# cptq/SignNet-BasisNet

Hardware: AMD Instinct MI355X
Metric: graphs/sec SignNet+GINE forward, ZINC batch=128 k=16 (higher is better)
Workload: dtype f32

## Files before the change

include/signnet_hip.h:

```cpp
#ifndef SIGNNET_HIP_H
#define SIGNNET_HIP_H

#include <stdint.h>

#ifdef __cplusplus
extern "C" {
#endif

#define SN_OK 0
#define SN_ERR_ARG (-1)
#define SN_ERR_LAUNCH (-2)
#define SN_ERR_UNSUPPORTED (-3)

#define SN_ABI_VERSION 3

int sn_version(void);
const char* sn_last_error(void);
int sn_device_info(int* cu_count, int* lds_bytes_per_cu, int* clock_khz);
int sn_clock_probe(int64_t cycles, int64_t* out_cycles, void* stream);

typedef struct {
  int32_t* phi_bin_col;
  int64_t phi_max_bins;
  int32_t* phi_col_bin0;
// ... 344 lines not shown
                     const int32_t* rowptr, const int32_t* col, const sn_plan_bins* bins,
                     int kmax , int K ,
                     float* out, void* stream);
int sn_phi_fused_prec_f32(const sn_phi_params* params, const float* eigen_vectors, const int32_t* graph_ptr, const int64_t* evoff,
                          const int32_t* rowptr, const int32_t* col, const sn_plan_bins* bins, int kmax, int K, float* out,
                          int precision, void* stream);

int sn_deepsigns_phi_f32(const sn_phi_params* params, const float* x, int ldx, const int32_t* graph_ptr, const int32_t* rowptr,
                         const int32_t* col, const sn_plan_bins* bins, int K, float* out, void* stream);
int sn_deepsigns_phi_prec_f32(const sn_phi_params* params, const float* x, int ldx, const int32_t* graph_ptr, const int32_t* rowptr,
                              const int32_t* col, const sn_plan_bins* bins, int K, float* out, int precision, void* stream);

#define SN_MLP_MAX_LAYERS 16
int sn_mlp_chain_f32(const float* x, int ldx, int64_t R, int d_in, const int32_t* nvalid, int K, const void* const* weights,
                     int n_layers, int d_pad, float* y, int ldy, int d_out, void* stream);
int sn_mlp_chain_prec_f32(const float* x, int ldx, int64_t R, int d_in, const int32_t* nvalid, int K, const void* const* weights,
                          int n_layers, int d_pad, float* y, int ldy, int d_out, int precision, void* stream);

typedef struct {
  const void *wq, *wk, *wv, *wfc;
  const float *ln1_g, *ln1_b;
  const void *w1, *w2;
  const float *ln2_g, *ln2_b;
} sn_rho_layer;

#define SN_RHO_MAX_LAYERS 8
#define SN_RHO_BIN_ROWS 64
typedef struct {
  int d, n_layers, heads, has_pos;
  float ln_eps;
  int head_pad;
  const float* pe_w1;
  const float* pe_bn0_scale;
  const float* pe_bn0_shift;
  const float* pe_w2;
  const float* pe_bn1_scale;
  const float* pe_bn1_shift;
  sn_rho_layer layers[SN_RHO_MAX_LAYERS];
} sn_rho_params;

int sn_rho_fused_f32(const sn_rho_params* params, const float* x, const float* eigen_values,
                     const int32_t* graph_ptr, int64_t B, int64_t N, const sn_plan_bins* bins, int kmax, int K,
                     float* out_sum, void* stream);
int sn_rho_fused_prec_f32(const sn_rho_params* params, const float* x, const float* eigen_values, const int32_t* graph_ptr, int64_t B,
                          int64_t N, const sn_plan_bins* bins, int kmax, int K, float* out_sum, int precision, void* stream);

typedef struct {
  const float* etab[10];
  const float* ew;
  const float* e_scale;
  const float* e_shift;
  const void* w1s;
  const void* w2s;
  const float* eps;
} sn_gnn_layer;

#define SN_GNN_MAX_LAYERS 16
#define SN_GNN_MAX_NODES 64
typedef struct {
  int d, n_layers, n_out, reserved;
  int node_discrete, node_nf;
  int edge_discrete, edge_nf;
  int node_vocab, edge_vocab;
  const float* ntab[10];
  const float* nw;
  const float* n_scale;
  const float* n_shift;
  const void* rho_out_w;
  const void* lin_a;
  const void* lin_b;
  const void* head_w1;
  const void* head_w2;
  sn_gnn_layer layers[SN_GNN_MAX_LAYERS];
} sn_gnn_params;

int sn_gnn_fused_f32(const sn_gnn_params* params, const void* x, int ldx, const void* edge_attr, int lde,
                     const float* rho_sum, const int32_t* graph_ptr, int64_t B, const int32_t* rowptr,
                     const int32_t* col, const int32_t* eperm, int32_t* status ,
                     float* y ,
                     const int32_t* flags_src, int n_flags, int32_t* flags_host ,
                     void* stream);


int sn_gin_net_fused_f32(const sn_gnn_params* params, const void* head_mid, int pool_mean, const int64_t* atom, const float* p, int ldp,
                         int kp, const int32_t* graph_ptr, int64_t B, const int32_t* rowptr, const int32_t* col, const int32_t* eperm,
                         int32_t* status, float* y, const int32_t* flags_src, int n_flags, void* stream);

int sn_transformer_net_fused_f32(const sn_gnn_params* params, const void* head_mid, int pool_mean, const int64_t* atom, const float* p,
                                 int ldp, int kp, const float* e_proj, int lde, const int32_t* graph_ptr, int64_t B, const int32_t* rowptr,
                                 const int32_t* col, const int32_t* eperm, int32_t* status, float* y, const int32_t* flags_src, int n_flags,
                                 void* stream);

typedef struct {
  const float* x; int ldx;
  int64_t R; int G;
  int d_in, d_out;
  const float* W; int ldw;
  const float* bias;
  const int32_t* nvalid; int K;
  const float* in_scale; const float* in_shift;
  int in_relu, out_relu;
  float* y; int ldy;
  float* stat_part;
} sn_train_linear_args;

typedef struct {
  int64_t R; int G;
  const int32_t* nvalid; int K;
  int d_in, d_out;
  const float* dy; int lddy;
  const float* zo; int ldzo;
  const float* coef_a; const float* coef_b; const float* coef_c;
  const float* mask_scale; const float* mask_shift;
  const float* x; int ldx;
  const float* x_scale; const float* x_shift;
  int x_relu;
  const float* x_mean;
  const float* W; int ldw;
  float* gx; int ldgx;
  float* sums_part;
  float* dw_part;
  int want_db;
  int gx_accumulate;
  const float* dot_x; int lddot;
  double* dot_part;
  const float* merge_sums; int merge_nblk;
  const float* merge_state; const float* merge_count; const float* merge_gamma;
  float* merge_dgamma; float* merge_dbeta; int merge_accumulate;
} sn_train_linear_bwd_args;

typedef struct sn_train_post_args {
  const float* dw_part; int nparts; int64_t stride; int64_t n_w; float* dw_out; int64_t n_b; float* db_out;
  const float* sums_part; int nblk; int G; int C; const float* state; const float* count; const float* gamma; float* coef;
  float* dgamma; float* dbeta; int accumulate_bn;
  const double* dot_part; int dot_n; float* dot_out;
} sn_train_post_args;
int sn_train_post_link_f32(const sn_train_post_args* args, void* stream);
int sn_train_linear_blocks(int64_t R, int G);
int sn_train_linear_bwd_blocks(int64_t R, int G);
int sn_train_bn_bwd_blocks(int64_t R, int G);
int64_t sn_train_linear_bwd_part_floats(int64_t R, int G, int d_in, int d_out);
int sn_train_linear_f32(const sn_train_linear_args* args, void* stream);
int sn_train_bn_finish_f32(const float* stat_part, int nblk, int G, int C, const float* gamma, const float* beta, float eps,
                           float momentum, float* running_mean, float* running_var, float* state, float* count, void* stream);
int sn_train_linear_bwd_f32(const sn_train_linear_bwd_args* args, void* stream);
int sn_train_bn_bwd_sums_f32(const float* dy, int lddy, const float* z, int ldz, int64_t R, int G, int C, const int32_t* nvalid,
                             int K, const float* state, int relu, float* sums_part, void* stream);
int sn_train_bn_bwd_finish_f32(const float* sums_part, int nblk, int G, int C, const float* state, const float* count,
                               const float* gamma, float* coef, float* dgamma, float* dbeta, int accumulate, void* stream);
int sn_train_bn_apply_f32(const float* z, int ldz, int64_t R, int G, int C, const int32_t* nvalid, int K, const float* state,
                          int relu, const float* residual, int ldr, float* y, int ldy, void* stream);
int sn_train_reduce_parts_f32(const float* part, int nparts, int64_t stride, int64_t n, float* out, int accumulate, void* stream);
#define SN_TRAIN_MAX_REDUCE_JOBS 64
typedef struct { const float* part; int nparts; int64_t stride; int64_t n; float* out; int accumulate; } sn_train_reduce_job;
int sn_train_reduce_jobs_f32(const sn_train_reduce_job* jobs, int njobs, void* stream);
typedef struct { const double* part; int n; float* out; } sn_train_dot_job;
int sn_train_dot_jobs_f64(const sn_train_dot_job* jobs, int njobs, void* stream);
int sn_train_dot_finish_f64(const double* part, int n, float* out, int accumulate, void* stream);

int sn_gin_aggregate_add_f32(const float* x, const float* plus, float* out, int64_t N, int F, const int32_t* rowptr, const int32_t* col,
                             const float* eps, void* stream);
int sn_gine_aggregate_bwd_add_f32(const float* h, const float* ee, const float* g, const float* plus, int64_t N, int C,
                                  const int32_t* rev_rowptr, const int32_t* rev_col, const int32_t* rev_eperm, const float* eps,
                                  float* dh, float* dee, void* stream);

typedef struct {
// ... 42 lines not shown
```

signnet_basisnet_amd/_lib.py:

```python
from __future__ import annotations

import ctypes as C
import os

import torch

_HERE = os.path.dirname(os.path.abspath(__file__))
LIB_PATH = os.path.join(_HERE, "libsignnet_hip.so")

EPI_BIAS, EPI_RELU_PRE, EPI_AFFINE, EPI_RELU, EPI_RESIDUAL = 1, 2, 4, 8, 16
EPI_RESIDUAL_PRE = 64
EPI_LEAKY = 128

_p, _i, _l, _f = C.c_void_p, C.c_int, C.c_int64, C.c_float
ABI_VERSION = 3

SIGNATURES = {
    "sn_version": [],
    "sn_device_info": [C.POINTER(_i), C.POINTER(_i), C.POINTER(_i)],
    "sn_clock_probe": [_l, _p, _p],
    "sn_batch_plan": [_p, _l, _l, _p, _l, _i, _p, _p, _p, _p, _p, _p, _p, _p, _p, _p, _p],
    "sn_batch_plan_ex": [_p, _l, _l, _p, _l, _i, _p, _p, _p, _p, _p, _p, _p, _p, _p, _p, _p, _p],
    "sn_batch_plan_early_supported": [_l, _l, _l],
    "sn_pack_eig_f32": [_p, _p, _p, _p, _p, _p, _l, _i, _p, _p, _p],
    "sn_bucket_pack": [_p, _p],
    "sn_bucket_pack_dgl": [_p, _p],
    "sn_store_gather": [_p, _p],
    "sn_store_gather_max_graphs": [],
    "sn_batch_plan_padded": [_p, _l, _l, _p, _l, _i, _p, _p, _p, _p, _p, _p, _p, _p, _p, _p, _p, _p, _p],
    "sn_masked_l1_f32": [_p, _p, _l, _i, _p, _p, _p, _p],
    "sn_masked_l1_bwd_f32": [_p, _p, _l, _i, _p, _p, _p, _p, _p],
    "sn_lap_pe_transform_f32": [_p, _i, _p, _i, _i, _i, _i, _p, _p, _i, _p],
    "sn_pack_weight_f32": [_p, _i, _i, _i, _p, _p],
    "sn_pack_weight_t_f32": [_p, _i, _i, _i, _p, _p],
    "sn_pack_split_f32": [_p, _i, _i, _i, _p, _p, _p, _p, _p],
    "sn_gin_aggregate_f32": [_p, _p, _l, _i, _p, _p, _p, _i, _p],
    "sn_gin_aggregate_slab_f32": [_p, _p, _l, _i, _l, _p, _p, _p, _p, _i, _p],
    "sn_gine_aggregate_f32": [_p, _p, _p, _l, _i, _p, _p, _p, _p, _p],
    "sn_masked_linear_f32": [_p, _i, _l, _i, _p, _i, _p, _p, _i, _i, _p, _p, _p, _i, _p, _i, _p],
    "sn_ign_mlp_f32": [_p, _l, _i, _i, _i, _p, _p, _p],
    "sn_deepsets_tail_f32": [_p, _i, _p, _p, _p],
    "sn_masked_linear_blockbias_f32": [_p, _i, _l, _i, _p, _i, _p, _p, _l, _i, _i, _p, _p, _p, _i, _p],
    "sn_bn_fold_f32": [_p, _p, _p, _p, _f, _i, _i, _p, _p, _p],
    "sn_bn_running_update_f32": [_p, _p, _p, _f, _i, _p, _p, _p],
    "sn_colstats_blocks": [_l],
    "sn_phi_fused_f32": [_p, _p, _p, _p, _p, _p, _p, _i, _i, _p, _p],
    "sn_rho_fused_f32": [_p, _p, _p, _p, _l, _l, _p, _i, _i, _p, _p],
    "sn_phi_fused_prec_f32": [_p, _p, _p, _p, _p, _p, _p, _i, _i, _p, _i, _p],
    "sn_rho_fused_prec_f32": [_p, _p, _p, _p, _l, _l, _p, _i, _i, _p, _i, _p],
    "sn_gnn_fused_f32": [_p, _p, _i, _p, _i, _p, _p, _l, _p, _p, _p, _p, _p, _p, _i, _p, _p],
    "sn_gin_net_fused_f32": [_p, _p, _i, _p, _p, _i, _i, _p, _l, _p, _p, _p, _p, _p, _p, _i, _p],
    "sn_transformer_net_fused_f32": [_p, _p, _i, _p, _p, _i, _i, _p, _i, _p, _l, _p, _p, _p, _p, _p, _p, _i, _p],
    "sn_masked_colstats_f32": [_p, _i, _l, _i, _p, _i, _p, _p, _p, _p, _p],
    "sn_masked_affine_f32": [_p, _i, _l, _i, _p, _i, _i, _p, _p, _p, _i, _p, _i, _p],
    "sn_masked_layernorm_f32": [_p, _p, _l, _i, _p, _p, _f, _p, _i, _p, _p],
    "sn_set_attention_f32": [_p, _p, _p, _l, _i, _i, _i, _p, _p, _p, _p],
    "sn_slot_sum_f32": [_p, _l, _i, _i, _p, _p],
    "sn_plan_double_i32": [_p, _p, _l, _l, _p, _p, _p],
    "sn_keep_mask_f32": [_p, _l, _f, _f, _p],
    "sn_embedding_sum_f32": [_p, _i, _i, _l, C.POINTER(_p), C.POINTER(C.c_int64), _i, _p, _p, _p],
    "sn_segment_pool_f32": [_p, _l, _i, _p, _i, _p, _p],
    "sn_ign_contract_2to1_f32": [_p, _l, _i, _p, _p, _p],
    "sn_laplacian_evd_f32": [_p, _l, _p, _l, _l, _i, _p, _p, _p, _l, _p, _i, _i, _p, _p, _p],
    "sn_laplacian_evd_large_f32": [_p, _l, _p, _l, _l, _i, _p, _p, _p, _l, _p, _i, _i, _p, _p, _p],
    "sn_evd_large_max_nodes": [],
    "sn_evd_large_work_ints": [_l],
    "sn_linear_bn_scratch_floats": [_l, _i, _i],
    "sn_linear_bn_train_f32": [_p, _i, _l, _i, _p, _i, _p, _p, _i, _p, _i, _p, _p, _f, _f, _p, _p, _p, _p, _p, _p, _p, _p, _p, _p],
    "sn_bn_train_stats_f32": [_p, _i, _l, _i, _p, _i, _p, _p, _f, _f, _p, _p, _p, _p, _p, _p, _p, _p, _p, _p],
    "sn_linear_wgrad_f32": [_p, _i, _p, _i, _l, _i, _i, _p, _i, _p, _p, _p, _p],
    "sn_bn_act_bwd_f32": [_p, _i, _p, _i, _l, _i, _p, _i, _p, _p, _p, _p, _i, _p, _p, _p, _i, _p, _p],
    "sn_relu_bwd_f32": [_p, _p, _l, _i, _p, _i, _p, _p],
    "sn_masked_layernorm_bwd_f32": [_p, _p, _p, _l, _i, _p, _f, _p, _i, _p, _p, _p, _p, _p],
    "sn_set_attention_bwd_f32": [_p, _p, _p, _p, _l, _i, _i, _i, _p, _p, _p, _p, _p, _p],
    "sn_gine_aggregate_bwd_f32": [_p, _p, _p, _l, _i, _p, _p, _p, _p, _p, _p, _p],
    "sn_slot_broadcast_f32": [_p, _l, _i, _i, _p, _p, _p],
    "sn_segment_broadcast_f32": [_p, _l, _i, _p, _i, _p, _p],
    "sn_embedding_sum_bwd_f32": [_p, _i, _i, _l, _p, C.POINTER(C.c_int64), _i, _p, _p, _p, _p],
    "sn_embedding_sum_layers_f32": [_p, _i, _i, _l, _i, _p, C.POINTER(C.c_int64), _i, _p, _p, _p],
    "sn_embedding_sum_bwd_layers_f32": [_p, _i, _i, _l, _i, _p, C.POINTER(C.c_int64), _i, _p, _p, _p, _p],
    "sn_dot_f32": [_p, _p, _l, _p, _p, _p],
    "sn_pna_aggregate_f32": [_p, _i, _p, _i, _i, _l, _p, _p, _f, _p, _i, _p],
    "sn_pna_aggregate_gather_f32": [_p, _i, _p, _i, _p, _i, _p, _i, _i, _l, _p, _p, _p, _f, _p, _i, _i, _p],
    "sn_grouped_linear_f32": [_p, _i, _l, _i, _i, _i, _p, _p, _p, _p, _p, _p, _i, _p],
    "sn_edge_attention_f32": [_p, _p, _p, _p, _l, _i, _i, _p, _p, _p, _p, _p],
    "sn_edge_attention_strided_f32": [_p, _p, _p, _i, _p, _i, _l, _i, _i, _p, _p, _p, _p, _p],
    "sn_pointwise_f32": [_p, _i, _l, _i, _p, _p, _p, _i, _f, _p, _i, _p, _i, _p],
    "sn_deepsigns_phi_f32": [_p, _p, _i, _p, _p, _p, _p, _i, _p, _p],
    "sn_mlp_chain_f32": [_p, _i, _l, _i, _p, _i, _p, _i, _i, _p, _i, _i, _p],
    "sn_deepsigns_phi_prec_f32": [_p, _p, _i, _p, _p, _p, _p, _i, _p, _i, _p],
    "sn_mlp_chain_prec_f32": [_p, _i, _l, _i, _p, _i, _p, _i, _i, _p, _i, _i, _i, _p],
    "sn_gat_aggregate_f32": [_p, _p, _p, _p, _l, _i, _i, _f, _i, _p, _p, _p, _p, _p],
    "sn_gat_aggregate_bwd_f32": [_p, _p, _p, _p, _p, _p, _p, _l, _l, _i, _i, _f, _i, _p, _p, _p, _p, _p, _p, _p, _p, _p, _p, _p, _p],
    "sn_edge_rows_sum_f32": [_p, _i, _i, _l, _p, _p, _p, _i, _p],
    "sn_pna_aggregate_bwd_f32": [_p, _i, _i, _l, _p, _p, _f, _p, _i, _p, _p, _p],
    "sn_edge_attention_bwd_f32": [_p, _p, _p, _p, _p, _p, _l, _l, _i, _i, _p, _p, _p, _p, _p, _p, _p, _p, _p, _p, _p, _p],
    "sn_act_bwd_f32": [_p, _p, _l, _i, _p, _i, _f, _p, _p],
    "sn_gatedgcn_fused_f32": [_p, _p, _p, _p, _l, _p, _p, _p, _p, _p, _p],
    "sn_dense_attention_f32": [_p, _p, _p, _l, _i, _i, _i, _p, _p, _p],
    "sn_dense_attention_bwd_f32": [_p, _p, _p, _p, _p, _p, _l, _i, _i, _i, _p, _p, _p, _p, _p],
    "sn_eigenspace_group": [_p, _i, _i, _p, _p, _p, _p, _p, _p, _p, _p],
    "sn_eigenspace_projectors_f32": [_p, _i, _i, _p, _p, _i, _p, _p],
    "sn_ign_contract_eigvecs_f32": [_p, _i, _i, _p, _p, _i, _i, _p, _p],
    "sn_gated_aggregate_f32": [_p, _p, _p, _p, _i, _p, _l, _i, _p, _p, _p, _p, _p, _p, _p, _p, _p, _p, _p, _p, _p],
    "sn_gated_aggregate_bwd_f32": [_p, _p, _p, _p, _p, _p, _p, _l, _i, _p, _p, _p, _p, _p, _p, _p, _p, _p, _p, _p, _p],
    "sn_adam_step_f32": [_p, _p, _p, _p, _l, _f, _f, _f, _f, _f, _i, _f, _p],
    "sn_train_post_link_f32": [_p, _p],
    "sn_train_linear_blocks": [_l, _i],
    "sn_train_linear_bwd_blocks": [_l, _i],
    "sn_train_bn_bwd_blocks": [_l, _i],
    "sn_train_linear_f32": [_p, _p],
    "sn_train_bn_finish_f32": [_p, _i, _i, _i, _p, _p, _f, _f, _p, _p, _p, _p, _p],
    "sn_train_linear_bwd_f32": [_p, _p],
    "sn_train_bn_bwd_sums_f32": [_p, _i, _p, _i, _l, _i, _i, _p, _i, _p, _i, _p, _p],
    "sn_train_bn_bwd_finish_f32": [_p, _i, _i, _i, _p, _p, _p, _p, _p, _p, _i, _p],
    "sn_train_bn_apply_f32": [_p, _i, _l, _i, _i, _p, _i, _p, _i, _p, _i, _p, _i, _p],
    "sn_train_reduce_parts_f32": [_p, _i, _l, _l, _p, _i, _p],
    "sn_train_dot_finish_f64": [_p, _i, _p, _i, _p],
    "sn_train_reduce_jobs_f32": [_p, _i, _p],
    "sn_train_dot_jobs_f64": [_p, _i, _p],
    "sn_masked_layernorm_bwd_acc_f32": [_p, _p, _p, _l, _i, _p, _f, _p, _i, _p, _p, _p, _p, _p],
    "sn_gin_aggregate_add_f32": [_p, _p, _p, _l, _i, _p, _p, _p, _p],
    "sn_gine_aggregate_bwd_add_f32": [_p, _p, _p, _p, _l, _i, _p, _p, _p, _p, _p, _p, _p],
    "sn_train_scalar_mlp_stats_f32": [_p, _f, _p, _p, _f, _p, _p, _p, _p],
    "sn_train_scalar_mlp_apply_f32": [_p, _p, _p],
    "sn_train_scalar_mlp_bwd_f32": [_p, _p, _p, _p, _p, _p, _p, _p, _p, _p, _p, _i, _p, _p],
}
_SPECIAL_RESTYPE = {"sn_last_error": C.c_char_p, "sn_packed_weight_floats": C.c_int64, "sn_evd_large_work_ints": C.c_int64}

_lib = None


def lib():
# ... 110 lines not shown
```

signnet_basisnet_amd/csrc/fused_gnn.hip:

```cpp
#include "fused_common.hpp"

namespace sn {

#ifdef SN_PROFILE
static __device__ int g_prof_block = 0;
#undef SN_STAMP
#undef SN_ACCUM
#define SN_STAMP(i) do { if ((int)blockIdx.x == g_prof_block && threadIdx.x == 0) g_prof[i] = clock64(); } while (0)
#define SN_ACCUM(i, t0) do { if ((int)blockIdx.x == g_prof_block && threadIdx.x == 0) g_prof[i] += clock64() - (t0); } while (0)
#endif

constexpr int GNN_ROWS = SN_GNN_MAX_NODES;
constexpr int GNN_WAVES = 8;
constexpr int GNN_EMAX = 192;
constexpr int GNN_CLS = 16;
constexpr int GNN_EEMAX = 96;
constexpr int GNN_EEPF = (GNN_EEMAX * 32 + GNN_WAVES * 64 - 1) / (GNN_WAVES * 64);

constexpr int SP_STRIDE = 256;
constexpr int SP_PLANE = GNN_ROWS * SP_STRIDE;
constexpr int SP_IMAGE = 52224;
static_assert(SP_IMAGE >= 3 * SP_PLANE && SP_IMAGE % 16 == 0, "three planes fit an image");
__device__ __forceinline__ int sp_chunk(int row, int c) { return ((c ^ row) & 15) << 4; }

struct GnnStruct {
  const void* x;
  int ldx;
  const void* edge_attr;
  int lde;
  const float* rho_sum;
  const int32_t* graph_ptr;
  const int32_t* rowptr;
  const int32_t* col;
  const int32_t* eperm;
  int32_t* status;
  float* y;
  int ee_rows;
  const int32_t* flags_src;
  int n_flags;
  int32_t* flags_host;
  int rho_ld, rho_w;
  const void* head_mid;
  int pool_mean;
};

__device__ __forceinline__ void sp_store4(unsigned char* img, int row, int ot, int g, f32x4 v) {
  float h[4], m[4], l[4];
#pragma unroll
  for (int i = 0; i < 4; ++i) {
    h[i] = __uint_as_float(__float_as_uint(v[i]) & 0xffff0000u);
    const float r = v[i] - h[i];
    m[i] = __uint_as_float(__float_as_uint(r) & 0xffff0000u);
    l[i] = r - m[i];
  }
  unsigned char* p = img + row * SP_STRIDE + sp_chunk(row, (ot >> 1) * 4 + g) + (ot & 1) * 8;
  *reinterpret_cast<uint2*>(p) = make_uint2(pack_hi16(h[0], h[1]), pack_hi16(h[2], h[3]));
  *reinterpret_cast<uint2*>(p + SP_PLANE) = make_uint2(pack_hi16(m[0], m[1]), pack_hi16(m[2], m[3]));
  *reinterpret_cast<uint2*>(p + 2 * SP_PLANE) = make_uint2(pack_hi16(l[0], l[1]), pack_hi16(l[2], l[3]));
}

template <int NKB>
struct WSplit { u32x4 f[NKB * 3]; f32x4 e[SPLIT_EPI]; };

template <int NKB>
__device__ __forceinline__ void wload(WSplit<NKB>& p, const void* wsp, int ot, int lane) {
  constexpr int NFE = 3 * NKB + SPLIT_EPI;
  const __amdgpu_buffer_rsrc_t rs = weight_rsrc(reinterpret_cast<const float*>(wsp), 0x7fffffff);
  const int voff = lane * 16;
  const int base = __builtin_amdgcn_readfirstlane(ot * NFE * 1024);
#pragma unroll
  for (int i = 0; i < 3 * NKB; ++i) p.f[i] = __builtin_amdgcn_raw_buffer_load_b128(rs, voff, base + i * 1024, 0);
#pragma unroll
  for (int j = 0; j < SPLIT_EPI; ++j) {
    const u32x4 v = __builtin_amdgcn_raw_buffer_load_b128(rs, voff, base + (3 * NKB + j) * 1024, 0);
    p.e[j] = f32x4{__uint_as_float(v[0]), __uint_as_float(v[1]), __uint_as_float(v[2]), __uint_as_float(v[3])};
  }
}

struct TileRange {
  int t_lo, t_hi, T;
  __device__ __forceinline__ bool empty() const { return t_lo >= t_hi; }
  __device__ __forceinline__ void decode(int t, int& ot, int& rt) const { ot = t / T; rt = t - ot * T; }
  __device__ __forceinline__ int first_ot() const { return t_lo / T; }
};

template <int NKB>
__device__ __forceinline__ f32x4 mfma_split_tile(const WSplit<NKB>& w, const Split8 (&x)[NKB]) {
  f32x4 a0 = {0.f, 0.f, 0.f, 0.f}, a1 = {0.f, 0.f, 0.f, 0.f};
#pragma unroll
  for (int kb = 0; kb < NKB; ++kb) {
    const u32x4 wh = w.f[3 * kb], wm = w.f[3 * kb + 1], wl = w.f[3 * kb + 2];
    a1 = mfma_bf(wl, x[kb].h, a1);
    a0 = mfma_bf(wm, x[kb].h, a0);
    a1 = mfma_bf(wh, x[kb].l, a1);
    a0 = mfma_bf(wh, x[kb].m, a0);
    a1 = mfma_bf(wm, x[kb].m, a1);
    a0 = mfma_bf(wh, x[kb].h, a0);
  }
  return a0 + a1;
}

template <int NKB, typename Epi>
__device__ __forceinline__ void coop_gemm(WSplit<NKB>& pre, WSplit<NKB>& alt, const void* wsp, const unsigned char* img,
                                          TileRange tr, int lane, Epi epi, const void* next_wsp, TileRange next_tr) {
  if (tr.empty()) {
    if (next_wsp && !next_tr.empty()) wload<NKB>(pre, next_wsp, next_tr.first_ot(), lane);
    return;
  }
  asm volatile("" : "+v"(tr.t_lo), "+v"(tr.t_hi), "+v"(tr.T));
  int ot0, rt0;
  tr.decode(tr.t_lo, ot0, rt0);
  int otl, rtl;
  tr.decode(tr.t_hi - 1, otl, rtl);
  const bool two_ots = otl != ot0;
  const unsigned char* rowbase = img + (lane & 15) * SP_STRIDE;
  auto load_rows = [&](int rt, Split8 (&x)[NKB]) {
    const unsigned char* p = rowbase + rt * 16 * SP_STRIDE;
#pragma unroll
    for (int kb = 0; kb < NKB; ++kb) {
      const unsigned char* pc = p + sp_chunk(lane & 15, kb * 4 + (lane >> 4));
      x[kb].h = *reinterpret_cast<const u32x4*>(pc);
      x[kb].m = *reinterpret_cast<const u32x4*>(pc + SP_PLANE);
      x[kb].l = *reinterpret_cast<const u32x4*>(pc + 2 * SP_PLANE);
    }
  };
#ifdef SN_PROFILE
// ... 53 lines not shown
}

template <int NKB, typename Epi>
__device__ __forceinline__ void coop_gemm_roll(WSplit<NKB>& cur, const unsigned char* img, TileRange tr, int lane, Epi epi,
                                               const void* nn_wsp, TileRange nn_tr, int kb0 = 0) {
  if (!tr.empty()) {
    asm volatile("" : "+v"(tr.t_lo), "+v"(tr.t_hi), "+v"(tr.T));
    const unsigned char* rowbase = img + (lane & 15) * SP_STRIDE;
#pragma unroll
    for (int i = 0; i < 4; ++i) {
      const int t = tr.t_lo + i;
      if (t < tr.t_hi) {
        int ot, rt;
        tr.decode(t, ot, rt);
        Split8 in[NKB];
        const unsigned char* p = rowbase + rt * 16 * SP_STRIDE;
        int cx = (lane & 15) ^ (lane >> 4) ^ (kb0 << 2);
        asm volatile("" : "+v"(cx));
#pragma unroll
        for (int kb = 0; kb < NKB; ++kb) {
          const unsigned char* pc = p + (((4 * kb) ^ cx) << 4);
          in[kb].h = *reinterpret_cast<const u32x4*>(pc);
          in[kb].m = *reinterpret_cast<const u32x4*>(pc + SP_PLANE);
          in[kb].l = *reinterpret_cast<const u32x4*>(pc + 2 * SP_PLANE);
        }
        epi(rt, ot, mfma_split_tile<NKB>(cur, in), cur.e[0], cur.e[1], cur.e[2]);
      }
    }
  }
  if (nn_wsp != nullptr && !nn_tr.empty()) wload<NKB>(cur, nn_wsp, nn_tr.first_ot(), lane);
}

template <int NKB, int PAIRS, typename Epi>
__device__ __forceinline__ void coop_gemm_weave(WSplit<NKB>& cur, const unsigned char* img, int ot, int lane, Epi epi,
                                                const void* nn_wsp, int nn_ot) {
  constexpr int NFE = 3 * NKB + SPLIT_EPI;
  const __amdgpu_buffer_rsrc_t rs = weight_rsrc(reinterpret_cast<const float*>(nn_wsp), 0x7fffffff);
  const int voff = lane * 16;
  const int base = __builtin_amdgcn_readfirstlane(nn_ot * NFE * 1024);
  const unsigned char* rowbase = img + (lane & 15) * SP_STRIDE;
#pragma unroll
  for (int rt = 0; rt < PAIRS; ++rt) {
    Split8 in[NKB];
    const unsigned char* p = rowbase + rt * 16 * SP_STRIDE;
    int cx = (lane & 15) ^ (lane >> 4);
    asm volatile("" : "+v"(cx));
#pragma unroll
    for (int kb = 0; kb < NKB; ++kb) {
      const unsigned char* pc = p + (((4 * kb) ^ cx) << 4);
      in[kb].h = *reinterpret_cast<const u32x4*>(pc);
      in[kb].m = *reinterpret_cast<const u32x4*>(pc + SP_PLANE);
      in[kb].l = *reinterpret_cast<const u32x4*>(pc + 2 * SP_PLANE);
    }
    if (rt + 1 < PAIRS) {
      epi(rt, ot, mfma_split_tile<NKB>(cur, in), cur.e[0], cur.e[1], cur.e[2]);
      __builtin_amdgcn_sched_barrier(0);
    } else {
      f32x4 a0 = {0.f, 0.f, 0.f, 0.f}, a1 = {0.f, 0.f, 0.f, 0.f};
#pragma unroll
      for (int kb = 0; kb < NKB; ++kb) {
        const u32x4 wh = cur.f[3 * kb], wm = cur.f[3 * kb + 1], wl = cur.f[3 * kb + 2];
        a1 = mfma_bf(wl, in[kb].h, a1);
        a0 = mfma_bf(wm, in[kb].h, a0);
        a1 = mfma_bf(wh, in[kb].l, a1);
        a0 = mfma_bf(wh, in[kb].m, a0);
        a1 = mfma_bf(wm, in[kb].m, a1);
        a0 = mfma_bf(wh, in[kb].h, a0);
        __builtin_amdgcn_sched_barrier(0);
#pragma unroll
        for (int j = 0; j < 3; ++j) cur.f[3 * kb + j] = __builtin_amdgcn_raw_buffer_load_b128(rs, voff, base + (3 * kb + j) * 1024, 0);
        __builtin_amdgcn_sched_barrier(0);
      }
      epi(rt, ot, a0 + a1, cur.e[0], cur.e[1], cur.e[2]);
      __builtin_amdgcn_sched_barrier(0);
#pragma unroll
      for (int j = 0; j < SPLIT_EPI; ++j) {
        const u32x4 v = __builtin_amdgcn_raw_buffer_load_b128(rs, voff, base + (3 * NKB + j) * 1024, 0);
        cur.e[j] = f32x4{__uint_as_float(v[0]), __uint_as_float(v[1]), __uint_as_float(v[2]), __uint_as_float(v[3])};
      }
    }
  }
}

template <int NT, int MODE = 0, int TC = 0>
__device__ __forceinline__ void gnn_graph(const GnnStruct& S, const sn_gnn_params& P) {
  constexpr bool DGL = MODE != 0, TF = MODE == 2;
  static_assert(TC == 0 || (NT == 8 && MODE == 0), "compile-time row tiles: the GINE net at NT = 8");
  static_assert(!TF || NT == 4, "the Transformer mode is written for d = 64");
  constexpr int D = 16 * NT;
  constexpr int LD = D + 4;
  constexpr int NKB = (NT + 1) / 2;
  extern __shared__ __align__(16) unsigned char lds_raw[];
  unsigned char* SA = lds_raw;
  unsigned char* SB = lds_raw + SP_IMAGE;
  float* X1 = reinterpret_cast<float*>(lds_raw + 2 * SP_IMAGE);
  int* erow = reinterpret_cast<int*>(X1 + (GNN_ROWS + 1) * LD);
  int* esrc = erow + GNN_ROWS + 4;
  int* efeat = esrc + GNN_EMAX;
  int* ecls = efeat + GNN_EMAX * (P.n_layers > 0 ? P.edge_nf : 0);
  int* elead = ecls + GNN_EMAX;
  int* cedge = elead + GNN_EMAX;
  float* EE = reinterpret_cast<float*>(cedge + GNN_CLS);
  float* PART = EE;
  const int lane = threadIdx.x & 63, wave = threadIdx.x >> 6, g = lane >> 4, li = lane & 15;
  const int gi = blockIdx.x;
  SN_STAMP(0);
#ifdef SN_PROFILE
  if ((int)blockIdx.x == g_prof_block && threadIdx.x == 0) for (int i = 8; i < 20; ++i) g_prof[i] = 0;
  long long pt = 0;
#endif
  WSplit<NKB> pre, alt;
  const int gs = S.graph_ptr[gi], n = S.graph_ptr[gi + 1] - gs;
  auto give_up = [&](int bit) {
    if (threadIdx.x == 0 && bit) atomicOr(&S.status[3], bit);
    if ((int)threadIdx.x < P.n_out) S.y[(int64_t)gi * P.n_out + threadIdx.x] = __uint_as_float(0x7fc00000u);
  };
  if (S.flags_src != nullptr && (S.flags_src[0] != 0 || (S.n_flags >= 16 && (S.flags_src[9] != 0 || S.flags_src[13] != 0)))) { give_up(0); return; }
  if (n <= 0) { give_up(8); return; }
  if (n > GNN_ROWS) { give_up(1); return; }
  const int e_base = S.rowptr[gs];
  const int ne = S.rowptr[gs + n] - e_base;
  const int d = P.d;
  __shared__ unsigned s_pro[3];
  if (threadIdx.x == 0) { s_pro[0] = 0u; s_pro[1] = 0u; s_pro[2] = 0u; }
  const int T = TC > 0 ? TC : (n + 15) >> 4;
  const int ntile = T * NT;
  TileRange tr;
  tr.T = T;
  if constexpr (GNN_WAVES % NT == 0) {
    constexpr int WPO = GNN_WAVES / NT;
    const int ot = wave / WPO, h = wave % WPO, per = (T + WPO - 1) / WPO;
    tr.t_lo = ot * T + (h * per < T ? h * per : T);
    tr.t_hi = ot * T + ((h + 1) * per < T ? (h + 1) * per : T);
  } else {
    const int q = (ntile + GNN_WAVES - 1) / GNN_WAVES;
    tr.t_lo = wave * q < ntile ? wave * q : ntile;
    tr.t_hi = tr.t_lo + q < ntile ? tr.t_lo + q : ntile;
  }
  TileRange hr;
  hr.T = 1;
  hr.t_lo = wave < NT ? wave : NT;
  hr.t_hi = wave < NT ? wave + 1 : NT;
  const f32x4 zero4 = {0.f, 0.f, 0.f, 0.f};
  bool use_tab = false;
  int ncls = 0;
  bool use_ee = !DGL && P.n_layers > 0 && ne <= S.ee_rows;
  auto edge_embed = [&](const sn_gnn_layer& Lq, int k, int c) -> f32x4 {
    const int EF = P.edge_nf;
    f32x4 ef = zero4;
    if (P.edge_discrete) {
      for (int f = 0; f < EF; ++f) {
        const float* trow = Lq.etab[f] + (int64_t)efeat[k * EF + f] * d;
        if ((d & 3) == 0) { if (c < d) ef += ld4(trow + c); }
        else {
#pragma unroll
          for (int qq = 0; qq < 4; ++qq) if (c + qq < d) ef[qq] += trow[c + qq];
        }
      }
    } else {
      f32x4 acc = zero4;
      for (int f = 0; f < EF; ++f) {
        const float a = __int_as_float(efeat[k * EF + f]);
#pragma unroll
        for (int qq = 0; qq < 4; ++qq) acc[qq] += a * Lq.ew[(c + qq) * EF + f];
      }
      ef = relu4(acc * ld4(Lq.e_scale + c) + ld4(Lq.e_shift + c));
    }
    return ef;
  };
  f32x4 eepf[GNN_EEPF];
  auto ee_fetch = [&](int l) {
    if (!use_ee || l >= P.n_layers) return;
    const sn_gnn_layer& Lq = P.layers[l];
    int t0 = threadIdx.x;
    asm volatile("" : "+v"(t0));
#pragma unroll
    for (int i = 0; i < GNN_EEPF; ++i) {
      const int idx = t0 + i * GNN_WAVES * 64;
      eepf[i] = zero4;
      if (idx < ne * (D / 4)) eepf[i] = edge_embed(Lq, idx / (D / 4), 4 * (idx % (D / 4)));
    }
  };
  bool tab_pending = false;
  auto ee_store = [&]() {
    if (tab_pending) {
      tab_pending = false;
      int t1 = threadIdx.x;
      asm volatile("" : "+v"(t1));
#pragma unroll
      for (int i = 0; i < GNN_EEPF; ++i) {
        const int idx = t1 + i * GNN_WAVES * 64;
        if (idx < P.n_layers * ncls * (D / 4)) lds_st4(EE + (idx / (D / 4)) * LD + 4 * (idx % (D / 4)), eepf[i]);
      }
      return;
    }
    if (!use_ee) return;
    int t0 = threadIdx.x;
    asm volatile("" : "+v"(t0));
#pragma unroll
    for (int i = 0; i < GNN_EEPF; ++i) {
      const int idx = t0 + i * GNN_WAVES * 64;
      if (idx < ne * (D / 4)) lds_st4(EE + (idx / (D / 4)) * LD + 4 * (idx % (D / 4)), eepf[i]);
    }
  };

  constexpr bool ROLL = NT >= 7 || GNN_WAVES % NT == 0;
  static_assert(GNN_WAVES == 8, "the ROLL condition assumes 8 waves");
  TileRange h2;
  h2.T = 1;
  h2.t_lo = 0;
  h2.t_hi = wave == 0 ? 1 : 0;
  static_assert(GNN_EMAX <= GNN_WAVES * 64 && GNN_ROWS < GNN_WAVES * 64 && GNN_ROWS * (D / 4) <= 4 * GNN_WAVES * 64, "one pass of the block covers the graph");
  const int tid = threadIdx.x;
  const int rp_v = tid <= n ? S.rowptr[gs + tid] : 0;
  const int rho_ld = S.rho_ld, rho_w = S.rho_w;
  const bool rs_vec = ((rho_ld | rho_w) & 3) == 0;
  f32x4 rs_v[4];
#pragma unroll
  for (int j = 0; j < 4; ++j) {
    rs_v[j] = zero4;
    const int i = tid + j * GNN_WAVES * 64;
    if (rs_vec && i < n * (D / 4)) {
      const int rr = i / (D / 4), c4 = i % (D / 4);
      if (4 * c4 < rho_w) rs_v[j] = ld4(S.rho_sum + (int64_t)(gs + rr) * rho_ld + 4 * c4);
    }
  }
  const bool xid_pref = P.node_discrete && P.node_nf == 1 && (d & 3) == 0;
  long long xid[4];
#pragma unroll
  for (int i = 0; i < 4; ++i) {
    xid[i] = -1;
    const int t = tr.t_lo + i;
    if (xid_pref && t < tr.t_hi) {
      int ot, rt;
      tr.decode(t, ot, rt);
      if (rt * 16 + li < n) xid[i] = reinterpret_cast<const int64_t*>(S.x)[(int64_t)(gs + rt * 16 + li) * S.ldx];
    }
  }
  if (ne > GNN_EMAX) { give_up(2); return; }
  const int src_v = tid < ne ? S.col[e_base + tid] : 0;
  const int eid_v = tid < ne ? S.eperm[e_base + tid] : 0;
  SN_STAMP(30);
  for (int i = threadIdx.x; i < 2 * SP_IMAGE / 16; i += GNN_WAVES * 64)
    reinterpret_cast<uint4*>(lds_raw)[i] = make_uint4(0u, 0u, 0u, 0u);
  if ((int)threadIdx.x < LD) { X1[GNN_ROWS * LD + threadIdx.x] = 0.f; EE[S.ee_rows * LD + threadIdx.x] = 0.f; }
  lds_barrier();
  SN_STAMP(31);
  const bool efast = !DGL && P.n_layers > 0 && P.edge_discrete && P.edge_nf == 1 && (d & 3) == 0;
  int my_ev = 0;
  {
    const int EF = P.edge_nf;
    if (tid <= n) erow[tid] = rp_v - e_base;
    if (tid < ne) {
      const int k = tid;
      esrc[k] = src_v - gs;
      const int eid = eid_v;
      if (TF) ecls[k] = eid;
      if (!DGL && P.n_layers > 0) {
        if (P.edge_discrete) {
          const int64_t* ei = reinterpret_cast<const int64_t*>(S.edge_attr) + (int64_t)eid * S.lde;
          for (int f = 0; f < EF; ++f) {
            const int64_t v = ei[f];
            const bool ok = (uint64_t)v < (uint64_t)P.edge_vocab;
            efeat[k * EF + f] = ok ? (int)v : 0;
            if (!ok) { atomicOr(&S.status[3], 4); atomicOr(&s_pro[0], 1u); }
            if (efast) {
              my_ev = ok ? (int)v : 0;
              if (my_ev < 32) atomicOr(&s_pro[2], 1u << my_ev); else atomicOr(&s_pro[1], 1u);
            }
          }
        } else {
          const float* ea = reinterpret_cast<const float*>(S.edge_attr) + (int64_t)eid * S.lde;
          for (int f = 0; f < EF; ++f) efeat[k * EF + f] = __float_as_int(ea[f]);
        }
      }
    }
  }
  f32x4 nrow[4];
#pragma unroll
  for (int i = 0; i < 4; ++i) {
    nrow[i] = zero4;
    const int t = tr.t_lo + i;
    if (xid_pref && t < tr.t_hi && xid[i] != -1) {
      int ot, rt;
      tr.decode(t, ot, rt);
      long long xv = xid[i];
      if ((uint64_t)xv >= (uint64_t)P.node_vocab) { xv = 0; atomicOr(&S.status[3], 4); atomicOr(&s_pro[0], 1u); }
      const int c = 16 * ot + 4 * g;
      if (c < d) nrow[i] = ld4(P.ntab[0] + xv * d + c);
    }
  }
  if (!tr.empty()) {
    wload<NKB>(pre, P.lin_a, tr.first_ot(), lane);
    if constexpr (ROLL) wload<NKB>(alt, P.lin_b, tr.first_ot(), lane);
  }
  lds_barrier();
  SN_STAMP(32);
  if (efast && s_pro[1] == 0u) {
    const unsigned present = s_pro[2];
    ncls = __popc(present);
    if (tid < ne) ecls[tid] = __popc(present & ((1u << my_ev) - 1u));
    use_tab = ncls <= GNN_CLS && P.n_layers * ncls <= S.ee_rows;
    if (use_tab) {
      use_ee = false;
      tab_pending = true;
      int t0 = threadIdx.x;
      asm volatile("" : "+v"(t0));
#pragma unroll
      for (int i = 0; i < GNN_EEPF; ++i) {
        const int idx = t0 + i * GNN_WAVES * 64;
        eepf[i] = zero4;
        if (idx < P.n_layers * ncls * (D / 4)) {
          const int rowi = idx / (D / 4), ch = 4 * (idx % (D / 4));
          const int l = rowi / ncls, c = rowi - l * ncls;
          unsigned m = present;
          for (int q = 0; q < c; ++q) m &= m - 1u;
          if (ch < d) eepf[i] = ld4(P.layers[l].etab[0] + (int64_t)__builtin_ctz(m) * d + ch);
        }
      }
    }
  }
  if (!DGL && P.n_layers > 0 && !tab_pending && !(efast && s_pro[1] == 0u)) {
    const int EF = P.edge_nf;
    __shared__ unsigned long long lmask[(GNN_EMAX + 63) / 64];
    int lead = -1;
    if (tid < GNN_EMAX) {
      if (tid < ne) {
        lead = tid;
        if (EF == 1) {
          const int mine = efeat[tid];
#pragma unroll 8
          for (int j = 0; j < ne; ++j) lead = (efeat[j] == mine && j < lead) ? j : lead;
        } else {
          for (int j = 0; j < ne; ++j) {
            bool same = true;
            for (int f = 0; f < EF; ++f) same = same && (efeat[j * EF + f] == efeat[tid * EF + f]);
            lead = (same && j < lead) ? j : lead;
          }
        }
        elead[tid] = lead;
      }
      const unsigned long long m = __ballot(tid < ne && lead == tid);
      if (lane == 0) lmask[tid >> 6] = m;
    }
    __syncthreads();
    ncls = 0;
#pragma unroll
    for (int w = 0; w < (GNN_EMAX + 63) / 64; ++w) ncls += __popcll(lmask[w]);
    if (tid < ne) {
      int c = 0;
#pragma unroll
      for (int w = 0; w < (GNN_EMAX + 63) / 64; ++w) {
        const int below = lead - 64 * w;
        const unsigned long long keep = below >= 64 ? ~0ull : (below > 0 ? (1ull << below) - 1 : 0ull);
        c += __popcll(lmask[w] & keep);
      }
      ecls[tid] = c;
      if (lead == tid && c < GNN_CLS) cedge[c] = lead;
    }
    use_tab = ncls <= GNN_CLS && P.n_layers * ncls <= S.ee_rows;
    if (use_tab) use_ee = false;
    __syncthreads();
    if (use_tab) {
      for (int i = threadIdx.x; i < P.n_layers * ncls * (D / 4); i += GNN_WAVES * 64) {
        const int rowi = i / (D / 4), ch = 4 * (i % (D / 4));
        const int l = rowi / ncls, c = rowi - l * ncls;
        lds_st4(EE + rowi * LD + ch, edge_embed(P.layers[l], cedge[c], ch));
      }
    }
  }
  SN_STAMP(33);
  if (rs_vec) {
#pragma unroll
    for (int j = 0; j < 4; ++j) {
      const int i = tid + j * GNN_WAVES * 64;
      if (i < n * (D / 4)) {
        const int rr = i / (D / 4), c4 = i % (D / 4);
        sp_store4(SA, rr, c4 >> 2, c4 & 3, rs_v[j]);
      }
    }
  } else {
    for (int i = threadIdx.x; i < n * (D / 4); i += GNN_WAVES * 64) {
      const int rr = i / (D / 4), c4 = i % (D / 4);
      f32x4 v = zero4;
#pragma unroll
      for (int qq = 0; qq < 4; ++qq) if (4 * c4 + qq < rho_w) v[qq] = S.rho_sum[(int64_t)(gs + rr) * rho_ld + 4 * c4 + qq];
      sp_store4(SA, rr, c4 >> 2, c4 & 3, v);
    }
  }
  SN_STAMP(34);
  if (xid_pref) {
#pragma unroll
    for (int i = 0; i < 4; ++i) {
      const int t = tr.t_lo + i;
      if (t < tr.t_hi && xid[i] != -1) {
        int ot, rt;
        tr.decode(t, ot, rt);
        sp_store4(SB, rt * 16 + li, ot, g, nrow[i]);
      }
    }
  } else if (P.node_discrete) {
    for (int t = tr.t_lo; t < tr.t_hi; ++t) {
      int ot, rt;
      tr.decode(t, ot, rt);
      const int row = rt * 16 + li, c = 16 * ot + 4 * g;
      if (row < n) {
        const int64_t* xi = reinterpret_cast<const int64_t*>(S.x) + (int64_t)(gs + row) * S.ldx;
        f32x4 s = zero4;
        for (int f = 0; f < P.node_nf; ++f) {
          int64_t xv = xi[f];
          if ((uint64_t)xv >= (uint64_t)P.node_vocab) { xv = 0; atomicOr(&S.status[3], 4); atomicOr(&s_pro[0], 1u); }
          const float* trow = P.ntab[f] + xv * d;
          if ((d & 3) == 0) { if (c < d) s += ld4(trow + c); }
          else {
#pragma unroll
            for (int qq = 0; qq < 4; ++qq) if (c + qq < d) s[qq] += trow[c + qq];
          }
        }
        sp_store4(SB, row, ot, g, s);
      }
    }
  } else {
    for (int t = tr.t_lo; t < tr.t_hi; ++t) {
      int ot, rt;
      tr.decode(t, ot, rt);
      const int row = rt * 16 + li, c = 16 * ot + 4 * g;
      if (row < n) {
        const float* xr = reinterpret_cast<const float*>(S.x) + (int64_t)(gs + row) * S.ldx;
        f32x4 acc = zero4;
        for (int f = 0; f < P.node_nf; ++f) {
          const float a = xr[f];
#pragma unroll
          for (int qq = 0; qq < 4; ++qq) acc[qq] += a * P.nw[(c + qq) * P.node_nf + f];
        }
        sp_store4(SB, row, ot, g, relu4(acc * ld4(P.n_scale + c) + ld4(P.n_shift + c)));
      }
    }
  }
  SN_STAMP(35);
  lds_barrier();
  const int graph_bad = (int)s_pro[0];
  SN_STAMP(1);
  int a_dg[4];
  unsigned a_sr[4], a_er[4];
#pragma unroll
  for (int i = 0; i < 4; ++i) {
    a_dg[i] = -1;
    a_sr[i] = 0u;
    a_er[i] = 0u;
    const int t = tr.t_lo + i;
    if (!TF && t < tr.t_hi && (DGL || use_tab || use_ee)) {
      int ot, rt;
      tr.decode(t, ot, rt);
      const int row = rt * 16 + li;
      if (row < n) {
        const int e_lo = erow[row], dg = erow[row + 1] - e_lo;
        a_dg[i] = dg;
#pragma unroll
        for (int k = 0; k < 4; ++k) {
          const int ei = k < dg ? e_lo + k : 0;
          a_sr[i] |= (unsigned)(k < dg ? esrc[ei] : GNN_ROWS) << (8 * k);
          if (!DGL) a_er[i] |= (unsigned)(k < dg ? (use_tab ? ecls[ei] : ei) : 255) << (8 * k);
        }
      }
    }
  }
  ee_fetch(0);
  const void* first_w = P.n_layers > 0 ? P.layers[0].w1s : P.head_w1;
  const TileRange first_tr = P.n_layers > 0 ? tr : hr;
  {
    auto epi_a = [&](int rt, int ot, f32x4 acc, f32x4, f32x4, f32x4) { lds_st4(X1 + (rt * 16 + li) * LD + 16 * ot + 4 * g, acc); };
    auto epi_b = [&](int rt, int ot, f32x4 acc, f32x4 bias, f32x4, f32x4) {
      float* o = X1 + (rt * 16 + li) * LD + 16 * ot + 4 * g;
      lds_st4(o, (lds_ld4(o) + acc) + bias);
    };
    const bool hasl = P.n_layers > 0;
    if constexpr (TC > 0) coop_gemm_weave<NKB, TC>(pre, SB, wave, lane, epi_a, first_w, first_tr.first_ot());
    else if constexpr (ROLL) coop_gemm_roll<NKB>(pre, SB, tr, lane, epi_a, first_w, first_tr);
    else coop_gemm<NKB>(pre, alt, P.lin_a, SB, tr, lane, epi_a, P.lin_b, tr);
    SN_STAMP(20);
    if constexpr (TC > 0) coop_gemm_weave<NKB, TC>(alt, SA, wave, lane, epi_b, hasl ? P.layers[0].w2s : P.head_w2, hasl ? wave : 0);
    else if constexpr (ROLL) coop_gemm_roll<NKB>(alt, SA, tr, lane, epi_b, hasl ? P.layers[0].w2s : P.head_w2, hasl ? tr : h2);
    else coop_gemm<NKB>(pre, alt, P.lin_b, SA, tr, lane, epi_b, first_w, first_tr);
  }
  ee_store();
  lds_barrier();
  SN_STAMP(2);
  if constexpr (TF) {
    static_assert(ROLL, "one output tile per wave and Linear");
    for (int t = tr.t_lo; t < tr.t_hi; ++t) {
      int ot, rt;
      tr.decode(t, ot, rt);
      const int row = rt * 16 + li, c = 16 * ot + 4 * g;
      sp_store4(SA, row, ot, g, lds_ld4(X1 + row * LD + c));
    }
    lds_barrier();
    unsigned char* A = SA;
    unsigned char* B = SB;
    const float* Eg = reinterpret_cast<const float*>(S.edge_attr);
    const int an = (int)threadIdx.x >> 3, ah = (int)threadIdx.x & 7;
    const float root = sqrtf(8.f);
    int at_lo = 0, at_dg = 0, at_sr[4] = {0, 0, 0, 0};
    const float* at_er[4] = {Eg, Eg, Eg, Eg};
    if (an < n) {
      at_lo = erow[an];
      at_dg = erow[an + 1] - at_lo;
#pragma unroll
      for (int k = 0; k < 4; ++k) {
        if (k < at_dg) {
          at_sr[k] = esrc[at_lo + k];
          at_er[k] = Eg + (int64_t)ecls[at_lo + k] * S.lde + 8 * ah;
        }
      }
    }
    for (int l = 0; l < P.n_layers; ++l) {
      f32x4 pe0[4], pe1[4];
#pragma unroll
      for (int k = 0; k < 4; ++k) {
        pe0[k] = zero4; pe1[k] = zero4;
        if (k < at_dg) { pe0[k] = ld4(at_er[k] + l * D); pe1[k] = ld4(at_er[k] + l * D + 4); }
      }
      const sn_gnn_layer& Lp = P.layers[l];
      const bool lastl = l + 1 == P.n_layers;
      auto seq = [&](int j) -> const void* {
        if (j < 8) return Lp.etab[j];
        if (!lastl) return P.layers[l + 1].etab[j - 8];
        return j == 8 ? P.head_w1 : S.head_mid;
      };
      auto seq_tr = [&](int j) { return (j < 8 || !lastl) ? tr : hr; };
      float* Qi = reinterpret_cast<float*>(B);
      float* Ki = Qi + GNN_ROWS * LD;
      float* Vi = Ki + GNN_ROWS * LD;
      static_assert((size_t)3 * GNN_ROWS * LD * sizeof(float) <= (size_t)SP_IMAGE, "Q | K | V fit one split image");
      auto epi_q = [&](int rt, int ot, f32x4 acc, f32x4, f32x4, f32x4) { lds_st4(Qi + (rt * 16 + li) * LD + 16 * ot + 4 * g, acc); };
      auto epi_k = [&](int rt, int ot, f32x4 acc, f32x4, f32x4, f32x4) { lds_st4(Ki + (rt * 16 + li) * LD + 16 * ot + 4 * g, acc); };
      auto epi_v = [&](int rt, int ot, f32x4 acc, f32x4, f32x4, f32x4) { lds_st4(Vi + (rt * 16 + li) * LD + 16 * ot + 4 * g, acc); };
      coop_gemm_roll<NKB>(pre, A, tr, lane, epi_q, seq(2), seq_tr(2));
      coop_gemm_roll<NKB>(alt, A, tr, lane, epi_k, seq(3), seq_tr(3));
      coop_gemm_roll<NKB>(pre, A, tr, lane, epi_v, seq(4), seq_tr(4));
      lds_barrier();
      if (an < n) {
        const f32x4 q0 = lds_ld4(Qi + an * LD + 8 * ah), q1 = lds_ld4(Qi + an * LD + 8 * ah + 4);
        f32x4 a0 = zero4, a1 = zero4;
        float z = 0.f;
        auto edge = [&](int sr, f32x4 e0, f32x4 e1) {
          const f32x4 k0 = lds_ld4(Ki + sr * LD + 8 * ah), k1 = lds_ld4(Ki + sr * LD + 8 * ah + 4);
          const f32x4 v0 = lds_ld4(Vi + sr * LD + 8 * ah), v1 = lds_ld4(Vi + sr * LD + 8 * ah + 4);
          float sc = 0.f;
#pragma unroll
          for (int c = 0; c < 4; ++c) sc += ((k0[c] * q0[c]) / root) * e0[c];
#pragma unroll
          for (int c = 0; c < 4; ++c) sc += ((k1[c] * q1[c]) / root) * e1[c];
          const float sw = expf(fminf(fmaxf(sc, -5.f), 5.f));
          z += sw;
#pragma unroll
          for (int c = 0; c < 4; ++c) { a0[c] += v0[c] * sw; a1[c] += v1[c] * sw; }
        };
#pragma unroll
        for (int k = 0; k < 4; ++k)
          if (k < at_dg) edge(at_sr[k], pe0[k], pe1[k]);
        for (int e = at_lo + 4; e < at_lo + at_dg; ++e) {
          const float* er = Eg + (int64_t)ecls[e] * S.lde + l * D + 8 * ah;
          edge(esrc[e], ld4(er), ld4(er + 4));
        }
        const float rz = 1.0f / (z + 1e-6f);
        sp_store4(A, an, ah >> 1, 2 * (ah & 1), a0 * rz);
        sp_store4(A, an, ah >> 1, 2 * (ah & 1) + 1, a1 * rz);
      }
      lds_barrier();
      auto epi_o = [&](int rt, int ot, f32x4 acc, f32x4 bias, f32x4 sc, f32x4 sh) {
        float* o = X1 + (rt * 16 + li) * LD + 16 * ot + 4 * g;
        f32x4 v = acc + bias;
        v = v + lds_ld4(o);
        v = v * sc + sh;
        lds_st4(o, v);
        sp_store4(B, rt * 16 + li, ot, g, v);
      };
      coop_gemm_roll<NKB>(alt, A, tr, lane, epi_o, seq(5), seq_tr(5));
      lds_barrier();
      auto epi_f1a = [&](int rt, int ot, f32x4 acc, f32x4 bias, f32x4, f32x4) { sp_store4(A, rt * 16 + li, ot, g, relu4(acc + bias)); };
      auto epi_f1b = [&](int rt, int ot, f32x4 acc, f32x4 bias, f32x4, f32x4) { sp_store4(A, rt * 16 + li, ot + NT, g, relu4(acc + bias)); };
      coop_gemm_roll<NKB>(pre, B, tr, lane, epi_f1a, seq(6), seq_tr(6));
      coop_gemm_roll<NKB>(alt, B, tr, lane, epi_f1b, seq(7), seq_tr(7));
      lds_barrier();
      auto epi_f2a = [&](int rt, int ot, f32x4 acc, f32x4, f32x4, f32x4) { lds_st4(PART + (rt * 16 + li) * LD + 16 * ot + 4 * g, acc); };
      auto epi_f2b = [&](int rt, int ot, f32x4 acc, f32x4 bias, f32x4 sc, f32x4 sh) {
        const int off = (rt * 16 + li) * LD + 16 * ot + 4 * g;
        f32x4 v = (lds_ld4(PART + off) + acc) + bias;
        v = v + lds_ld4(X1 + off);
        v = v * sc + sh;
        lds_st4(X1 + off, v);
        sp_store4(B, rt * 16 + li, ot, g, v);
      };
      coop_gemm_roll<NKB>(pre, A, tr, lane, epi_f2a, seq(8), seq_tr(8));
      coop_gemm_roll<NKB>(alt, A, tr, lane, epi_f2b, seq(9), seq_tr(9), 2);
      lds_barrier();
      unsigned char* tsw = A; A = B; B = tsw;
    }
  } else {
  for (int l = 0; l < P.n_layers; ++l) {
    const sn_gnn_layer& Lp = P.layers[l];
#ifdef SN_PROFILE
    pt = clock64();
#endif
    ee_fetch(l + 1);
    {
      const float sc = 1.f + *Lp.eps;
      if (DGL || use_tab || use_ee) {
        const int eoff = use_tab ? l * ncls : 0;
#pragma unroll
        for (int i = 0; i < 4; ++i) {
          if (a_dg[i] >= 0) {
            const int t = tr.t_lo + i;
            int ot, rt;
            tr.decode(t, ot, rt);
            const int row = rt * 16 + li, c = 16 * ot + 4 * g, dg = a_dg[i];
            f32x4 hv[4], ev[4];
#pragma unroll
            for (int k = 0; k < 4; ++k) {
              const int sr = (int)((a_sr[i] >> (8 * k)) & 255u), er = (int)((a_er[i] >> (8 * k)) & 255u);
              hv[k] = lds_ld4(X1 + sr * LD + c);
              if (!DGL) ev[k] = lds_ld4(EE + (er == 255 ? S.ee_rows : er + eoff) * LD + c);
            }
            f32x4 u = zero4;
#pragma unroll
            for (int k = 0; k < 4; ++k) u += DGL ? hv[k] : relu4(hv[k] + ev[k]);
            if (dg > 4) {
              const int e_lo = erow[row], e_hi = e_lo + dg;
              for (int e = e_lo + 4; e < e_hi; ++e) {
                if (DGL) { u += lds_ld4(X1 + esrc[e] * LD + c); continue; }
                const f32x4 ef = use_tab ? lds_ld4(EE + (l * ncls + ecls[e]) * LD + c) : lds_ld4(EE + e * LD + c);
                u += relu4(lds_ld4(X1 + esrc[e] * LD + c) + ef);
              }
            }
            {
#pragma clang fp contract(off)
              const f32x4 self = lds_ld4(X1 + row * LD + c) * sc;
              u = u + self;
            }
            sp_store4(SA, row, ot, g, u);
          }
          __builtin_amdgcn_sched_barrier(0);
        }
      } else {
#pragma unroll 1
        for (int t = tr.t_lo; t < tr.t_hi; ++t) {
          int ot, rt;
          tr.decode(t, ot, rt);
          const int row = rt * 16 + li, c = 16 * ot + 4 * g;
          if (row >= n) continue;
          f32x4 u = zero4;
          const int e_lo = erow[row], e_hi = erow[row + 1];
          for (int e = e_lo; e < e_hi; ++e) u += relu4(lds_ld4(X1 + esrc[e] * LD + c) + edge_embed(Lp, e, c));
          {
#pragma clang fp contract(off)
            const f32x4 self = lds_ld4(X1 + row * LD + c) * sc;
            u = u + self;
          }
          sp_store4(SA, row, ot, g, u);
        }
      }
    }
    lds_barrier();
    SN_ACCUM(9, pt);
#ifdef SN_PROFILE
    pt = clock64();
#endif
    ee_store();
    const bool lastl = l + 1 == P.n_layers;
    auto epi_1 = [&](int rt, int ot, f32x4 acc, f32x4 sc, f32x4 sh, f32x4) { sp_store4(SB, rt * 16 + li, ot, g, relu4(acc * sc + sh)); };
    if constexpr (TC > 0) coop_gemm_weave<NKB, TC>(pre, SA, wave, lane, epi_1, lastl ? P.head_w1 : P.layers[lastl ? l : l + 1].w1s, wave);
    else if constexpr (ROLL) coop_gemm_roll<NKB>(pre, SA, tr, lane, epi_1, lastl ? P.head_w1 : P.layers[lastl ? l : l + 1].w1s, lastl ? hr : tr);
    else coop_gemm<NKB>(pre, alt, Lp.w1s, SA, tr, lane, epi_1, Lp.w2s, tr);
    lds_barrier();
    SN_ACCUM(11, pt);
#ifdef SN_PROFILE
    pt = clock64();
#endif
    auto epi_2 = [&](int rt, int ot, f32x4 acc, f32x4 sc, f32x4 sh, f32x4) {
      float* o = X1 + (rt * 16 + li) * LD + 16 * ot + 4 * g;
      if (DGL) lds_st4(o, acc * sc + sh);
      else lds_st4(o, relu4(acc * sc + sh) + lds_ld4(o));
    };
    if constexpr (TC > 0) coop_gemm_weave<NKB, TC>(alt, SB, wave, lane, epi_2, lastl ? P.head_w2 : P.layers[lastl ? l : l + 1].w2s, lastl ? 0 : wave);
    else if constexpr (ROLL) coop_gemm_roll<NKB>(alt, SB, tr, lane, epi_2, lastl ? (DGL ? S.head_mid : P.head_w2) : P.layers[lastl ? l : l + 1].w2s,
                                            lastl ? (DGL ? hr : h2) : tr);
    else coop_gemm<NKB>(pre, alt, Lp.w2s, SB, tr, lane, epi_2, lastl ? P.head_w1 : P.layers[lastl ? l : l + 1].w1s, lastl ? hr : tr);
    if (TC > 0 && !lastl) asm volatile("" ::: "memory");
    else lds_barrier();
    SN_ACCUM(12, pt);
    SN_STAMP(24 + l);
  }
  }
  SN_STAMP(3);
  static_assert(16 * (D / 4) <= GNN_WAVES * 64 && (size_t)16 * D * sizeof(float) <= (size_t)(SP_PLANE - 16 * SP_STRIDE), "one pass; the partial sums fit");
  float* PS = reinterpret_cast<float*>(SA + 16 * SP_STRIDE);
  {
    const int pj = threadIdx.x / (D / 4), pc4 = threadIdx.x % (D / 4);
    if (pj < 16) {
      f32x4 s = zero4;
      for (int r = pj; r < n; r += 16) s += lds_ld4(X1 + r * LD + 4 * pc4);
      lds_st4(PS + pj * D + 4 * pc4, s);
    }
    lds_barrier();
    if (pj < 16) {
      f32x4 s = zero4;
      if (pj == 0) {
#pragma unroll
        for (int j = 0; j < 16; ++j) s += lds_ld4(PS + j * D + 4 * pc4);
        if (DGL && S.pool_mean) s = s / (float)n;
      }
      sp_store4(SA, pj, pc4 >> 2, pc4 & 3, s);
    }
  }
  lds_barrier();
  SN_STAMP(4);
  auto epi_h1 = [&](int rt, int ot, f32x4 acc, f32x4 sc, f32x4 sh, f32x4) { sp_store4(SB, li, ot, g, relu4(acc * sc + sh)); };
  auto epi_h2 = [&](int rt, int ot, f32x4 acc, f32x4 bias, f32x4, f32x4) {
    if (li == 0) {
#pragma unroll
      for (int qq = 0; qq < 4; ++qq) {
        const int c = 4 * g + qq;
        if (c < P.n_out) S.y[(int64_t)gi * P.n_out + c] = graph_bad ? __uint_as_float(0x7fc00000u) : acc[qq] + bias[qq];
      }
    }
  };
  if constexpr (DGL) {
    auto epi_hm = [&](int rt, int ot, f32x4 acc, f32x4 sc, f32x4 sh, f32x4) { sp_store4(SA, li, ot, g, relu4(acc * sc + sh)); };
    if constexpr (ROLL) coop_gemm_roll<NKB>(pre, SA, hr, lane, epi_h1, wave == 0 ? P.head_w2 : nullptr, h2);
    else coop_gemm<NKB>(pre, alt, P.head_w1, SA, hr, lane, epi_h1, S.head_mid, hr);
    lds_barrier();
    if constexpr (ROLL) coop_gemm_roll<NKB>(alt, SB, hr, lane, epi_hm, nullptr, h2);
    else coop_gemm<NKB>(pre, alt, S.head_mid, SB, hr, lane, epi_hm, wave == 0 ? P.head_w2 : nullptr, h2);
    lds_barrier();
    if constexpr (ROLL) coop_gemm_roll<NKB>(pre, SA, h2, lane, epi_h2, nullptr, h2);
    else coop_gemm<NKB>(pre, alt, P.head_w2, SA, h2, lane, epi_h2, nullptr, h2);
  } else {
  if constexpr (ROLL) coop_gemm_roll<NKB>(pre, SA, hr, lane, epi_h1, nullptr, h2);
  else coop_gemm<NKB>(pre, alt, P.head_w1, SA, hr, lane, epi_h1, wave == 0 ? P.head_w2 : nullptr, h2);
  lds_barrier();
  if constexpr (ROLL) coop_gemm_roll<NKB>(alt, SB, h2, lane, epi_h2, nullptr, h2);
  else coop_gemm<NKB>(pre, alt, P.head_w2, SB, h2, lane, epi_h2, nullptr, h2);
  }
  SN_STAMP(5);
#ifdef SN_PROFILE
  if ((int)blockIdx.x == g_prof_block && threadIdx.x == 0) { g_prof[6] = n; g_prof[7] = ne; }
#endif
}

template <int NT, int MODE = 0>
__global__ __launch_bounds__(GNN_WAVES * 64, 2) void k_gnn_coop(GnnStruct S, sn_gnn_params P) {
  if constexpr (NT == 8 && MODE == 0) {
    const int n = S.graph_ptr[blockIdx.x + 1] - S.graph_ptr[blockIdx.x];
    switch ((n + 15) >> 4) {
      case 1: gnn_graph<NT, MODE, 1>(S, P); break;
      case 2: gnn_graph<NT, MODE, 2>(S, P); break;
      case 3: gnn_graph<NT, MODE, 3>(S, P); break;
      case 4: gnn_graph<NT, MODE, 4>(S, P); break;
      default:
        if (threadIdx.x == 0) atomicOr(&S.status[3], n > GNN_ROWS ? 1 : 8);
        if ((int)threadIdx.x < P.n_out) S.y[(int64_t)blockIdx.x * P.n_out + threadIdx.x] = __uint_as_float(0x7fc00000u);
        break;
    }
  } else {
    gnn_graph<NT, MODE>(S, P);
  }
  if (S.flags_host != nullptr) {
    __syncthreads();
    if (threadIdx.x == 0) {
      __threadfence();
      if (atomicAdd(&S.status[4], 1) == (int)gridDim.x - 1) {
        __threadfence();
        for (int i = 0; i < S.n_flags; ++i)
          S.flags_host[i] = __hip_atomic_load(&S.flags_src[i], __ATOMIC_RELAXED, __HIP_MEMORY_SCOPE_AGENT);
        __threadfence_system();
        __hip_atomic_store(&S.flags_host[S.n_flags], 1, __ATOMIC_RELEASE, __HIP_MEMORY_SCOPE_SYSTEM);
        __threadfence_system();
      }
    }
  }
}

template <int NT, int MODE = 0>
static int launch_gnn(const GnnStruct& S, const sn_gnn_params& P, int64_t B, hipStream_t st) {
  constexpr bool DGL = MODE != 0;
  constexpr int LD = 16 * NT + 4;
  const size_t base = (size_t)2 * SP_IMAGE + (size_t)((GNN_ROWS + 1) * LD) * sizeof(float) +
                      (size_t)(GNN_ROWS + 4 + GNN_EMAX * (3 + (P.n_layers > 0 ? P.edge_nf : 0)) + GNN_CLS) * sizeof(int);
  const size_t lds_cap = 160 * 1024 - 512;
  const size_t room = base < lds_cap ? lds_cap - base : 0;
  int ee_rows = (int)(room / ((size_t)LD * sizeof(float))) - 1;
  if (ee_rows > GNN_EEMAX) ee_rows = GNN_EEMAX;
  if (ee_rows < 0) ee_rows = 0;
  GnnStruct S2 = S;
  S2.ee_rows = MODE == 2 ? GNN_ROWS : ((!DGL && P.n_layers > 0) ? ee_rows : 0);
  const size_t lds = base + (size_t)(S2.ee_rows + 1) * LD * sizeof(float);
  static bool init = false;
  if (!init) {
    const size_t lds_max = lds_cap;
    if (lds_max > 64 * 1024 &&
        hipFuncSetAttribute(reinterpret_cast<const void*>(k_gnn_coop<NT, MODE>), hipFuncAttributeMaxDynamicSharedMemorySize,
                            (int)lds_max) != hipSuccess)
      return fail(SN_ERR_LAUNCH, "sn_gnn_fused_f32: cannot raise the dynamic LDS limit to %zu", lds_max);
    init = true;
  }
  hipLaunchKernelGGL((k_gnn_coop<NT, MODE>), dim3((unsigned)B), dim3(GNN_WAVES * 64), lds, st, S2, P);
  return SN_OK;
}

}

using namespace sn;

#ifdef SN_PROFILE
extern "C" int sn_prof_read_gnn(long long* host) { return (int)hipMemcpyFromSymbol(host, HIP_SYMBOL(g_prof), sizeof(long long) * 64); }
extern "C" int sn_prof_set_block(int b) { return (int)hipMemcpyToSymbol(HIP_SYMBOL(g_prof_block), &b, sizeof(int)); }
#endif

extern "C" int sn_gnn_fused_f32(const sn_gnn_params* params, const void* x, int ldx, const void* edge_attr, int lde,
                                const float* rho_sum, const int32_t* graph_ptr, int64_t B, const int32_t* rowptr,
                                const int32_t* col, const int32_t* eperm, int32_t* status, float* y,
                                const int32_t* flags_src, int n_flags, int32_t* flags_host, void* stream) {
  SN_REQUIRE(params && x && rho_sum && graph_ptr && rowptr && status && y && B >= 0, "sn_gnn_fused_f32: null pointer");
  const sn_gnn_params& P = *params;
  SN_REQUIRE(P.d > 0 && P.d <= 128, "sn_gnn_fused_f32: hidden width %d not in (0, 128]", P.d);
  SN_REQUIRE(P.n_layers >= 0 && P.n_layers <= SN_GNN_MAX_LAYERS, "sn_gnn_fused_f32: %d layers unsupported", P.n_layers);
  SN_REQUIRE(P.n_out >= 1 && P.n_out <= 16, "sn_gnn_fused_f32: n_out=%d not in [1,16]", P.n_out);
  SN_REQUIRE(P.node_nf >= 1 && P.node_nf <= (P.node_discrete ? 10 : 16) && ldx >= P.node_nf,
             "sn_gnn_fused_f32: node feature count %d unsupported", P.node_nf);
  SN_REQUIRE(P.n_layers == 0 || (edge_attr && P.edge_nf >= 1 && P.edge_nf <= (P.edge_discrete ? 10 : 16) && lde >= P.edge_nf),
             "sn_gnn_fused_f32: edge feature count %d unsupported", P.edge_nf);
  SN_REQUIRE(P.lin_a && P.lin_b && P.head_w1 && P.head_w2, "sn_gnn_fused_f32: parameters missing");
  SN_REQUIRE(P.rho_out_w == nullptr, "sn_gnn_fused_f32: rho_out_w must be NULL — fold rho.out into lin_b (see signnet_hip.h)");
  if (P.node_discrete) { for (int f = 0; f < P.node_nf; ++f) SN_REQUIRE(P.ntab[f], "sn_gnn_fused_f32: node table %d missing", f); }
  else SN_REQUIRE(P.nw && P.n_scale && P.n_shift, "sn_gnn_fused_f32: node MLP parameters missing");
  for (int l = 0; l < P.n_layers; ++l) {
    const sn_gnn_layer& L = P.layers[l];
    SN_REQUIRE(L.w1s && L.w2s && L.eps, "sn_gnn_fused_f32: layer %d parameters missing", l);
    if (P.edge_discrete) { for (int f = 0; f < P.edge_nf; ++f) SN_REQUIRE(L.etab[f], "sn_gnn_fused_f32: layer %d edge table %d missing", l, f); }
    else SN_REQUIRE(L.ew && L.e_scale && L.e_shift, "sn_gnn_fused_f32: layer %d edge MLP parameters missing", l);
  }
  if (B == 0) return SN_OK;
  SN_REQUIRE(!flags_host || (flags_src && n_flags > 0 && n_flags <= 64), "sn_gnn_fused_f32: flag report needs flags_src and 0 < n_flags <= 64");
  SN_REQUIRE(!flags_src || n_flags >= 1, "sn_gnn_fused_f32: flags_src needs n_flags >= 1");
  SN_REQUIRE((!P.node_discrete || P.node_vocab > 0) && (P.n_layers == 0 || !P.edge_discrete || P.edge_vocab > 0),
             "sn_gnn_fused_f32: node_vocab / edge_vocab (rows of the embedding tables) missing");
  GnnStruct S{x, ldx, edge_attr, lde, rho_sum, graph_ptr, rowptr, col, eperm, status, y, 0, flags_src, n_flags, flags_host,
              P.d, P.d, nullptr, 0};
  hipStream_t st = (hipStream_t)stream;
  int rc = SN_OK;
  switch ((P.d + 15) / 16) {
    case 1: rc = launch_gnn<1>(S, P, B, st); break;
    case 2: rc = launch_gnn<2>(S, P, B, st); break;
    case 3: rc = launch_gnn<3>(S, P, B, st); break;
    case 4: rc = launch_gnn<4>(S, P, B, st); break;
    case 5: rc = launch_gnn<5>(S, P, B, st); break;
    case 6: rc = launch_gnn<6>(S, P, B, st); break;
    case 7: rc = launch_gnn<7>(S, P, B, st); break;
    default: rc = launch_gnn<8>(S, P, B, st); break;
  }
  if (rc != SN_OK) return rc;
  SN_CHECK_LAUNCH("sn_gnn_fused_f32");
  return SN_OK;
}

extern "C" int sn_gin_net_fused_f32(const sn_gnn_params* params, const void* head_mid, int pool_mean, const int64_t* atom, const float* p,
                                    int ldp, int kp, const int32_t* graph_ptr, int64_t B, const int32_t* rowptr, const int32_t* col,
                                    const int32_t* eperm, int32_t* status, float* y, const int32_t* flags_src, int n_flags, void* stream) {
  SN_REQUIRE(params && head_mid && atom && p && graph_ptr && rowptr && col && eperm && status && y && B >= 0, "sn_gin_net_fused_f32: null pointer");
  const sn_gnn_params& P = *params;
  SN_REQUIRE(P.d > 0 && P.d <= 128 && (P.d & 3) == 0, "sn_gin_net_fused_f32: padded hidden width %d must be a multiple of 4 in (0, 128]", P.d);
  SN_REQUIRE(P.n_layers >= 1 && P.n_layers <= SN_GNN_MAX_LAYERS, "sn_gin_net_fused_f32: %d layers unsupported", P.n_layers);
  SN_REQUIRE(P.n_out >= 1 && P.n_out <= 16, "sn_gin_net_fused_f32: n_out=%d not in [1,16]", P.n_out);
  SN_REQUIRE(P.node_discrete == 1 && P.node_nf == 1 && P.ntab[0] && P.node_vocab > 0, "sn_gin_net_fused_f32: one atom-type table expected");
  SN_REQUIRE(P.edge_nf == 0, "sn_gin_net_fused_f32: the GIN net has no edge term (edge_nf must be 0)");
  SN_REQUIRE(P.lin_a && P.lin_b && P.head_w1 && P.head_w2 && P.rho_out_w == nullptr, "sn_gin_net_fused_f32: parameters missing");
  SN_REQUIRE(kp >= 1 && kp <= P.d && ldp >= kp, "sn_gin_net_fused_f32: positional encoding width %d unsupported", kp);
  for (int l = 0; l < P.n_layers; ++l) {
    const sn_gnn_layer& L = P.layers[l];
    SN_REQUIRE(L.w1s && L.w2s && L.eps, "sn_gin_net_fused_f32: layer %d parameters missing", l);
  }
  SN_REQUIRE(!flags_src || n_flags >= 1, "sn_gin_net_fused_f32: flags_src needs n_flags >= 1");
  if (B == 0) return SN_OK;
  GnnStruct S{atom, 1, nullptr, 0, p, graph_ptr, rowptr, col, eperm, status, y, 0, flags_src, n_flags, nullptr, ldp, kp, head_mid, pool_mean};
  hipStream_t st = (hipStream_t)stream;
  int rc = SN_OK;
  switch ((P.d + 15) / 16) {
    case 1: case 2: case 3: case 4: rc = launch_gnn<4, 1>(S, P, B, st); break;
    case 5: case 6: rc = launch_gnn<6, 1>(S, P, B, st); break;
    default: rc = launch_gnn<8, 1>(S, P, B, st); break;
  }
  if (rc != SN_OK) return rc;
  SN_CHECK_LAUNCH("sn_gin_net_fused_f32");
  return SN_OK;
}

extern "C" int sn_transformer_net_fused_f32(const sn_gnn_params* params, const void* head_mid, int pool_mean, const int64_t* atom,
                                            const float* p, int ldp, int kp, const float* e_proj, int lde, const int32_t* graph_ptr, int64_t B,
                                            const int32_t* rowptr, const int32_t* col, const int32_t* eperm, int32_t* status, float* y,
                                            const int32_t* flags_src, int n_flags, void* stream) {
  SN_REQUIRE(params && head_mid && atom && p && e_proj && graph_ptr && rowptr && col && eperm && status && y && B >= 0,
             "sn_transformer_net_fused_f32: null pointer");
  const sn_gnn_params& P = *params;
  SN_REQUIRE(P.d == 64, "sn_transformer_net_fused_f32: hidden width %d (the stage kernel is written for 64 = 8 heads of 8)", P.d);
  SN_REQUIRE(P.n_layers >= 1 && P.n_layers <= SN_GNN_MAX_LAYERS, "sn_transformer_net_fused_f32: %d layers unsupported", P.n_layers);
  SN_REQUIRE(P.n_out >= 1 && P.n_out <= 16, "sn_transformer_net_fused_f32: n_out=%d not in [1,16]", P.n_out);
  SN_REQUIRE(P.node_discrete == 1 && P.node_nf == 1 && P.ntab[0] && P.node_vocab > 0, "sn_transformer_net_fused_f32: one atom-type table expected");
  SN_REQUIRE(P.edge_nf == 0, "sn_transformer_net_fused_f32: edge_nf must be 0 (the edge term is e_proj)");
  SN_REQUIRE(P.lin_a && P.lin_b && P.head_w1 && P.head_w2 && P.rho_out_w == nullptr, "sn_transformer_net_fused_f32: parameters missing");
  SN_REQUIRE(kp >= 1 && kp <= P.d && ldp >= kp && lde >= P.n_layers * P.d && (lde & 3) == 0 && (reinterpret_cast<uintptr_t>(e_proj) & 15) == 0,
             "sn_transformer_net_fused_f32: positional encoding / edge projection shapes");
  for (int l = 0; l < P.n_layers; ++l) {
    const sn_gnn_layer& L = P.layers[l];
    for (int j = 0; j < 8; ++j) SN_REQUIRE(L.etab[j], "sn_transformer_net_fused_f32: layer %d stage matrix %d missing", l, j);
    SN_REQUIRE(L.w1s == (const void*)L.etab[0] && L.w2s == (const void*)L.etab[1], "sn_transformer_net_fused_f32: w1s / w2s must repeat etab[0] / etab[1]");
  }
  SN_REQUIRE(!flags_src || n_flags >= 1, "sn_transformer_net_fused_f32: flags_src needs n_flags >= 1");
  if (B == 0) return SN_OK;
  GnnStruct S{atom, 1, e_proj, lde, p, graph_ptr, rowptr, col, eperm, status, y, 0, flags_src, n_flags, nullptr, ldp, kp, head_mid, pool_mean};
  const int rc = launch_gnn<4, 2>(S, P, B, (hipStream_t)stream);
  if (rc != SN_OK) return rc;
  SN_CHECK_LAUNCH("sn_transformer_net_fused_f32");
  return SN_OK;
}
```

signnet_basisnet_amd/csrc/plan.hip:

```cpp
#include "common.hpp"

namespace sn {

enum { ST_ERR = 0, ST_NMAX = 1, ST_DEGMAX = 2 };
enum { ERR_UNSORTED = 1, ERR_GRAPH_ID = 2, ERR_EDGE_RANGE = 4, ERR_EDGE_CROSS = 8 };

constexpr int PLAN_T = 1024;
constexpr int BINS_BMAX = 6144;

struct BinsDev {
  int32_t* phi_bin_col;
  long long phi_max_bins;
  int32_t* phi_col_bin0;
  int32_t* phi_col_mem;
  int32_t* phi_col_off;
  int32_t* rho_bin0;
  int32_t* meta;
  int32_t* phi_bin_mem;
};

struct EarlyDev {
  const int64_t* node_ids;
  long long n_node_ids, node_vocab;
  const int64_t* edge_ids;
// ... 343 lines not shown
          for (int k = 0; k < 4; ++k) dst[k] = make_int4(w[4 * k], w[4 * k + 1], w[4 * k + 2], w[4 * k + 3]);
        }
      } else {
        for (int b = t; b < nbins; b += PLAN_T) {
          int lo = 0, hi = ncol;
          while (hi - lo > 1) {
            const int mid = (lo + hi) >> 1;
            if (col_bin[mid] <= b) lo = mid; else hi = mid;
          }
          const int slot = b - col_bin[lo];
          const int cs = col_start[lo], ce = (lo + 1 < ncol) ? col_start[lo + 1] : nrec;
          int w[16];
#pragma unroll
          for (int k = 0; k < 8; ++k) {
            w[2 * k] = -1; w[2 * k + 1] = 0;
            if (cs + k < ce) {
              const int rw = rec[cs + k];
              const int cls = rw & 127, left = rw >> 8;
              if (slot < phi_slots_of(cls, kmax)) {
                const int g = bucket[bstart[cls] + hist[cls] - 1 - left];
                w[2 * k] = g | (slot << 13) | ((rec_pre[cs + k] - rec_pre[cs]) << 19) | ((cls - 1) << 25);
                w[2 * k + 1] = gp[g];
              }
            }
          }
          int4* dst = reinterpret_cast<int4*>(bd.phi_bin_mem + (size_t)b * 16);
#pragma unroll
          for (int k = 0; k < 4; ++k) dst[k] = make_int4(w[4 * k], w[4 * k + 1], w[4 * k + 2], w[4 * k + 3]);
        }
      }
    }
    PL_STAMP(7);
    if (bd.phi_bin_col == nullptr) return;
    for (int c = t; c <= ncol; c += PLAN_T) bd.phi_col_bin0[c] = col_bin[c];
    for (int r = t; r < nrec; r += PLAN_T) {
      const int w = rec[r];
      const int cls = w & 127, left = w >> 8;
      int lo = 0, hi = ncol;
      while (hi - lo > 1) {
        const int mid = (lo + hi) >> 1;
        if (col_start[mid] <= r) lo = mid; else hi = mid;
      }
      const int cs = col_start[lo];
      const int rank = hist[cls] - 1 - left;
      const int g = bucket[bstart[cls] + rank];
      const int mem = r - cs;
      const int slot = lo * 8 + mem;
      bd.phi_col_mem[slot] = g;
      bd.phi_col_off[slot] = rec_pre[r] - rec_pre[cs];
      if (r + 1 == nrec || ((rec[r + 1] >> 7) & 1)) {
        for (int m = mem + 1; m < 8; ++m) { bd.phi_col_mem[lo * 8 + m] = -1; bd.phi_col_off[lo * 8 + m] = 0; }
      }
    }
    if (!over) {
      for (int c = t; c < ncol; c += PLAN_T) {
        const int lo = col_bin[c], hi = col_bin[c + 1];
        for (int j = lo; j < hi; ++j) bd.phi_bin_col[j] = c;
      }
    }
  }
}

__device__ void lds_graph_ptr(const int64_t* __restrict__ batch, int N, int B, int* gp, int* err, int* ng = nullptr) {
  const int t = threadIdx.x;
  for (int i = t; i <= B; i += PLAN_T) gp[i] = N;
  __syncthreads();
  for (int i = t; i < N; i += PLAN_T) {
    const long long g = batch[i];
    const long long gprev = (i == 0) ? -1 : batch[i - 1];
    if (ng) ng[i] = (g < 0 || g >= B) ? -1 : (int)g;
    if (g < 0 || g >= B) { if (err) atomicOr(err, ERR_GRAPH_ID); continue; }
    if (gprev > g && err) atomicOr(err, ERR_UNSORTED);
    if (gprev < g) {
      const long long lo = gprev < -1 ? 0 : gprev + 1;
      for (long long k = lo; k <= g; ++k) gp[k] = i;
    }
  }
  __syncthreads();
}

constexpr int PS_NMAX = 4096, PS_EMAX = 12288, PS_BMAX = 1024;
constexpr int PS_BINS_INTS = 5 * PS_BMAX + 3 * 66 + 32 + 8;



__global__ __launch_bounds__(PLAN_T) void k_plan_small(const int64_t* __restrict__ batch, int N, int B,
                                                       const int64_t* __restrict__ ei, int E, int kmax,
                                                       int32_t* __restrict__ graph_ptr, int32_t* __restrict__ node_graph,
                                                       int32_t* __restrict__ nvalid, int64_t* __restrict__ evoff,
                                                       int32_t* __restrict__ rowptr, int32_t* __restrict__ col,
                                                       int32_t* __restrict__ eperm, int32_t* __restrict__ status, BinsDev bd,
                                                       int do_bins, EarlyDev early) {
  extern __shared__ int sm[];
  const int t = threadIdx.x;
  PL_STAMP(0);
  if (blockIdx.x == 1) {
    if (!do_bins) return;
    int* gp = sm;
    lds_graph_ptr(batch, N, B, gp, nullptr);
    PL_STAMP(1);
    plan_bins_block(gp, B, kmax, bd, sm + (PS_BMAX + 4), sm + (PS_BMAX + 4) + PS_BINS_INTS, early.host);
    PL_STAMP(2);
    return;
  }
  if (blockIdx.x == 3) {
    int bad = 0;
    for (long long i = t; i < early.n_node_ids; i += PLAN_T) bad |= ((unsigned long long)early.node_ids[i] >= (unsigned long long)early.node_vocab) ? 1 : 0;
    for (long long i = t; i < early.n_edge_ids; i += PLAN_T) bad |= ((unsigned long long)early.edge_ids[i] >= (unsigned long long)early.edge_vocab) ? 1 : 0;
    bad = __syncthreads_or(bad);
    if (t == 0) { early_put(early.host, EH_IDS, bad ? 1 : 0); early_done(early.host, 3); }
    return;
  }
  if (blockIdx.x == 2) {
    int* gp = sm;
    lds_graph_ptr(batch, N, B, gp, nullptr);
    plan_rho_block(gp, B, kmax, bd, sm + (PS_BMAX + 4), early.host);
    {
      int* wsum2 = sm + (PS_BMAX + 4) + B;
      __shared__ int s_nmax2;
      if (t == 0) s_nmax2 = 0;
      __syncthreads();
      const int perb = (B + PLAN_T - 1) / PLAN_T;
      const int blo = t * perb, bhi = (blo + perb < B) ? blo + perb : B;
      int q = 0, nmax = 0;
      for (int g = blo; g < bhi; ++g) { const int n = gp[g + 1] - gp[g]; q += n * n; nmax = nmax > n ? nmax : n; }
      for (int off = 32; off > 0; off >>= 1) nmax = max(nmax, __shfl_xor(nmax, off, 64));
      if ((t & 63) == 0) atomicMax(&s_nmax2, nmax);
      int qtot;
      int qrun = block_exscan(q, wsum2, t, &qtot);
      for (int g = blo; g < bhi; ++g) { const int n = gp[g + 1] - gp[g]; evoff[g] = qrun; qrun += n * n; }
      if (t == 0) {
        evoff[B] = qtot; status[ST_NMAX] = s_nmax2;
        if (early.host != nullptr) { early_put(early.host, EH_NMAX, s_nmax2); early_done(early.host, 2); }
      }
    }
    return;
  }
  int* gp = sm;
  int* deg = gp + (PS_BMAX + 4);
  int* rp = deg + PS_NMAX;
  int* lfill = rp + (PS_NMAX + 4);
  int* lperm = lfill + PS_EMAX;
  int* wsum = lperm + PS_EMAX;
  int* ng = wsum + 32;
  __shared__ int s_err, s_nmax, s_dmax, s_big;
  if (t == 0) { s_err = 0; s_nmax = 0; s_dmax = 0; s_big = 0; }
  constexpr int NPT = PS_NMAX / PLAN_T, EPT = PS_EMAX / PLAN_T;
  long long bcur[NPT], bprev[NPT];
#pragma unroll
  for (int k = 0; k < NPT; ++k) {
    const int i = t + k * PLAN_T;
    bcur[k] = i < N ? batch[i] : 0;
    bprev[k] = (i < N && i > 0) ? batch[i - 1] : -1;
  }
  int es[EPT], ed[EPT];
  {
    long long sv[EPT], dv[EPT];
#pragma unroll
    for (int k = 0; k < EPT; ++k) {
      const int e = t + k * PLAN_T;
      sv[k] = e < E ? ei[e] : 0;
      dv[k] = e < E ? ei[(long long)E + e] : 0;
    }
    for (int i = t; i < N; i += PLAN_T) deg[i] = 0;
    for (int i = t; i <= B; i += PLAN_T) gp[i] = N;
    __syncthreads();
#pragma unroll
    for (int k = 0; k < NPT; ++k) {
      const int i = t + k * PLAN_T;
      if (i < N) {
        const long long g = bcur[k], gprev = bprev[k];
        const bool ok = g >= 0 && g < B;
        ng[i] = ok ? (int)g : -1;
        if (!ok) atomicOr(&s_err, ERR_GRAPH_ID);
        else {
          if (gprev > g) atomicOr(&s_err, ERR_UNSORTED);
          if (gprev < g) {
            const long long lo = gprev < -1 ? 0 : gprev + 1;
            for (long long q = lo; q <= g; ++q) gp[q] = i;
          }
        }
      }
    }
#pragma unroll
    for (int k = 0; k < EPT; ++k) {
      const int e = t + k * PLAN_T;
      const bool bad = e < E && (sv[k] < 0 || sv[k] >= N || dv[k] < 0 || dv[k] >= N);
      if (bad) atomicOr(&s_err, ERR_EDGE_RANGE);
      es[k] = (e < E && !bad) ? (int)sv[k] : -1;
      ed[k] = (e < E && !bad) ? (int)dv[k] : -1;
    }
  }
  __syncthreads();
  PL_STAMP(1);
  int epos[EPT];
#pragma unroll
  for (int k = 0; k < EPT; ++k) {
    epos[k] = 0;
    if (ed[k] >= 0) {
      if (ng[es[k]] != ng[ed[k]]) atomicOr(&s_err, ERR_EDGE_CROSS);
      epos[k] = atomicAdd(&deg[ed[k]], 1);
    }
  }
  __syncthreads();
  PL_STAMP(2);
  {
    const int per = (N + PLAN_T - 1) / PLAN_T;
    const int lo = t * per, hi = (lo + per < N) ? lo + per : N;
    int s = 0, dmax = 0;
    for (int i = lo; i < hi; ++i) { s += deg[i]; dmax = dmax > deg[i] ? dmax : deg[i]; }
    for (int off = 32; off > 0; off >>= 1) dmax = max(dmax, __shfl_xor(dmax, off, 64));
    if ((t & 63) == 0) atomicMax(&s_dmax, dmax);
    int total;
    int run = block_exscan(s, wsum, t, &total);
    for (int i = lo; i < hi; ++i) { rp[i] = run; run += deg[i]; }
    if (t == 0) rp[N] = total;
    if (!do_bins) {
      const int perb = (B + PLAN_T - 1) / PLAN_T;
      const int blo = t * perb, bhi = (blo + perb < B) ? blo + perb : B;
      int q = 0, nmax = 0;
      for (int g = blo; g < bhi; ++g) { const int n = gp[g + 1] - gp[g]; q += n * n; nmax = nmax > n ? nmax : n; }
      for (int off = 32; off > 0; off >>= 1) nmax = max(nmax, __shfl_xor(nmax, off, 64));
      if ((t & 63) == 0) atomicMax(&s_nmax, nmax);
      int qtot;
      int qrun = block_exscan(q, wsum, t, &qtot);
      for (int g = blo; g < bhi; ++g) { const int n = gp[g + 1] - gp[g]; evoff[g] = qrun; qrun += n * n; }
      if (t == 0) evoff[B] = qtot;
    }
  }
  __syncthreads();
  PL_STAMP(3);
#pragma unroll
  for (int k = 0; k < EPT; ++k)
    if (ed[k] >= 0) lfill[rp[ed[k]] + epos[k]] = ((t + k * PLAN_T) << 12) | es[k];
  if (early.host != nullptr && early.max_graph_edges > 0) {
    for (int g = t; g < B; g += PLAN_T)
      if (rp[gp[g + 1]] - rp[gp[g]] > early.max_graph_edges) atomicOr(&s_big, 1);
  }
  __syncthreads();
  PL_STAMP(4);
#pragma unroll
  for (int k = 0; k < EPT; ++k) {
    if (ed[k] >= 0) {
      const int key = ((t + k * PLAN_T) << 12) | es[k];
      const int lo = rp[ed[k]], hi = rp[ed[k] + 1];
      int rank = 0;
      for (int q = lo; q < hi; ++q) rank += lfill[q] < key ? 1 : 0;
      lperm[lo + rank] = key;
    }
  }
  __syncthreads();
  PL_STAMP(5);
  for (int i = t; i <= N; i += PLAN_T) rowptr[i] = rp[i];
  for (int i = t; i < E; i += PLAN_T) { const int k = lperm[i]; col[i] = k & 4095; eperm[i] = k >> 12; }
  for (int i = t; i <= B; i += PLAN_T) graph_ptr[i] = gp[i];
  for (int i = t; i < N; i += PLAN_T) {
    const int g = ng[i];
    int nv = 0, gi = 0;
    if (g >= 0) { gi = g; nv = slots_of(gp[g + 1] - gp[g], kmax); }
    node_graph[i] = gi;
    nvalid[i] = nv;
  }
  if (t == 0) { status[ST_ERR] = s_err; if (!do_bins) status[ST_NMAX] = s_nmax; status[ST_DEGMAX] = s_dmax; status[3] = 0; }
  if (t >= 4 && t < 8) status[t] = 0;
  if (early.host != nullptr) {
    if (t == 0) {
      early_put(early.host, EH_ERR, s_err);
      early_put(early.host, EH_DEGMAX, s_dmax);
      early_put(early.host, EH_EDGES, s_big);
      if (!do_bins) { early_put(early.host, EH_NMAX, s_nmax); early_put(early.host, EH_PHI, 0); early_put(early.host, EH_RHO, 0); }
      early_done(early.host, 0);
      if (!do_bins) { early_done(early.host, 1); early_done(early.host, 2); }
      if (early.node_ids == nullptr && early.edge_ids == nullptr) { early_put(early.host, EH_IDS, 0); early_done(early.host, 3); }
    }
  }
  PL_STAMP(6);
}

__global__ void k_plan_nodes(const int64_t* __restrict__ batch, int64_t N, int64_t B,
                             int32_t* __restrict__ graph_ptr, int32_t* __restrict__ node_graph,
                             int32_t* __restrict__ deg, int32_t* __restrict__ status) {
  const int64_t i = (int64_t)blockIdx.x * blockDim.x + threadIdx.x;
  if (i < 8) status[i] = 0;
  if (i == 0) graph_ptr[B] = (int32_t)N;
  if (i >= N) return;
  int64_t g = batch[i];
  deg[i] = 0;
  if (g < 0 || g >= B) { node_graph[i] = 0; return; }
  node_graph[i] = (int32_t)g;
  int64_t gp = (i == 0) ? -1 : batch[i - 1];
  if (gp < -1) gp = -1;
  if (gp < g)
    for (int64_t t = gp + 1; t <= g; ++t) graph_ptr[t] = (int32_t)i;
  if (i == N - 1)
    for (int64_t t = g + 1; t < B; ++t) graph_ptr[t] = (int32_t)N;
}

__global__ void k_plan_degree(const int64_t* __restrict__ batch, const int64_t* __restrict__ ei, int64_t E,
                              int64_t N, int64_t B, int32_t* __restrict__ deg, int32_t* __restrict__ status) {
  const int64_t t = (int64_t)blockIdx.x * blockDim.x + threadIdx.x;
  if (t < N) {
    int64_t g = batch[t];
    if (g < 0 || g >= B) atomicOr(&status[ST_ERR], ERR_GRAPH_ID);
    if (t > 0 && batch[t - 1] > g) atomicOr(&status[ST_ERR], ERR_UNSORTED);
  }
  if (t >= E) return;
  int64_t s = ei[t], d = ei[E + t];
  if (s < 0 || s >= N || d < 0 || d >= N) {
    atomicOr(&status[ST_ERR], ERR_EDGE_RANGE);
    return;
  }
  if (batch[s] != batch[d]) atomicOr(&status[ST_ERR], ERR_EDGE_CROSS);
  atomicAdd(&deg[d], 1);
}

__global__ __launch_bounds__(PLAN_T) void k_plan_scan(int64_t N, int64_t B, int kmax,
                                                      const int32_t* __restrict__ graph_ptr,
                                                      const int32_t* __restrict__ node_graph,
                                                      int32_t* __restrict__ deg ,
                                                      int32_t* __restrict__ rowptr, int32_t* __restrict__ nvalid,
                                                      int64_t* __restrict__ evoff, int32_t* __restrict__ status, BinsDev bd) {
  extern __shared__ int sm[];
  const int T = blockDim.x, t = threadIdx.x;
  if (blockIdx.x == 1) {
    int* gp = sm;
    for (int64_t i = t; i <= B; i += T) gp[i] = graph_ptr[i];
    __syncthreads();
    plan_rho_block(gp, (int)B, kmax, bd, sm + B + 4);
    __syncthreads();
    plan_bins_block(gp, (int)B, kmax, bd, sm + B + 4, (kmax == 0 && B <= PLAN_SLAB_BMAX) ? sm + B + 4 + 5 * (int)B + 3 * 66 + 32 + 8 : nullptr);
    return;
  }
  __shared__ long long part[PLAN_T];
  __shared__ int maxs[2];
  if (t == 0) { maxs[0] = 0; maxs[1] = 0; }
  __syncthreads();
  {
    int64_t per = (N + T - 1) / T;
    int64_t lo = (int64_t)t * per, hi = lo + per < N ? lo + per : N;
    long long s = 0;
    int dmax = 0;
    for (int64_t i = lo; i < hi; ++i) { s += deg[i]; dmax = dmax > deg[i] ? dmax : deg[i]; }
    part[t] = s;
    atomicMax(&maxs[1], dmax);
    __syncthreads();
    for (int off = 1; off < T; off <<= 1) {
      long long v = (t >= off) ? part[t - off] : 0;
      __syncthreads();
      part[t] += v;
      __syncthreads();
    }
    long long run = part[t] - s;
    for (int64_t i = lo; i < hi; ++i) {
      int dgi = deg[i];
      rowptr[i] = (int32_t)run;
      deg[i] = (int32_t)run;
      run += dgi;
    }
    if (t == T - 1) rowptr[N] = (int32_t)part[T - 1];
    __syncthreads();
  }
  {
    int64_t per = (B + T - 1) / T;
    int64_t lo = (int64_t)t * per, hi = lo + per < B ? lo + per : B;
    long long s = 0;
    int nmax = 0;
    for (int64_t b = lo; b < hi; ++b) {
      long long n = graph_ptr[b + 1] - graph_ptr[b];
      s += n * n;
      nmax = nmax > (int)n ? nmax : (int)n;
    }
    part[t] = s;
    atomicMax(&maxs[0], nmax);
    __syncthreads();
    for (int off = 1; off < T; off <<= 1) {
      long long v = (t >= off) ? part[t - off] : 0;
      __syncthreads();
      part[t] += v;
      __syncthreads();
    }
    long long run = part[t] - s;
    for (int64_t b = lo; b < hi; ++b) {
      long long n = graph_ptr[b + 1] - graph_ptr[b];
      evoff[b] = run;
      run += n * n;
    }
    if (t == T - 1) evoff[B] = part[T - 1];
    __syncthreads();
  }
  for (int64_t i = t; i < N; i += T) {
    int g = node_graph[i];
    nvalid[i] = slots_of(graph_ptr[g + 1] - graph_ptr[g], kmax);
  }
  if (t == 0) { status[ST_NMAX] = maxs[0]; status[ST_DEGMAX] = maxs[1]; }
}

__global__ __launch_bounds__(256) void k_plan_fill(const int64_t* __restrict__ ei, int64_t E, int64_t N,
                                                   int32_t* __restrict__ cursor, int32_t* __restrict__ col,
                                                   int32_t* __restrict__ eperm) {
  int64_t e = (int64_t)blockIdx.x * blockDim.x + threadIdx.x;
  if (e >= E) return;
  int64_t s = ei[e], d = ei[E + e];
  if (s < 0 || s >= N || d < 0 || d >= N) return;
  int p = atomicAdd(&cursor[d], 1);
  col[p] = (int32_t)s;
  eperm[p] = (int32_t)e;
}

__global__ void k_plan_sort(int64_t N, const int32_t* __restrict__ rowptr, int32_t* __restrict__ col,
                            int32_t* __restrict__ eperm) {
  int64_t i = (int64_t)blockIdx.x * blockDim.x + threadIdx.x;
  if (i >= N) return;
  int lo = rowptr[i], hi = rowptr[i + 1];
  for (int a = lo + 1; a < hi; ++a) {
    int ke = eperm[a], kc = col[a];
    int b = a - 1;
    while (b >= lo && eperm[b] > ke) {
      eperm[b + 1] = eperm[b];
      col[b + 1] = col[b];
      --b;
    }
    eperm[b + 1] = ke;
    col[b + 1] = kc;
  }
}

__global__ void k_pack_eig(const float* __restrict__ ev, const float* __restrict__ es,
                           const int32_t* __restrict__ graph_ptr, const int32_t* __restrict__ node_graph,
                           const int32_t* __restrict__ nvalid, const int64_t* __restrict__ evoff,
                           int64_t N, int K, float* __restrict__ x0, float* __restrict__ s0) {
  int64_t idx = (int64_t)blockIdx.x * blockDim.x + threadIdx.x;
  if (idx >= N * K) return;
  int64_t i = idx / K;
  int j = (int)(idx - i * K);
  int g = node_graph[i];
  int gs = graph_ptr[g];
  int n = graph_ptr[g + 1] - gs;
  bool ok = j < nvalid[i];
  float v = 0.f, s = 0.f;
  if (ok) {
    v = ev[evoff[g] + (int64_t)(i - gs) * n + j];
    if (s0) s = es[gs + j];
  }
  x0[idx] = v;
  if (s0) s0[idx] = s;
}

}

using namespace sn;

static bool plan_one_launch(int64_t N, int64_t E, int64_t B) { return N > 0 && N <= PS_NMAX && E <= PS_EMAX && B <= PS_BMAX; }

extern "C" int sn_batch_plan_early_supported(int64_t N, int64_t E, int64_t B) { return plan_one_launch(N, E, B) ? 1 : 0; }

extern "C" int sn_batch_plan_ex(const int64_t* batch, int64_t N, int64_t B, const int64_t* edge_index,
                                int64_t E, int kmax, int32_t* graph_ptr, int32_t* node_graph,
                                int32_t* nvalid, int64_t* evoff, int32_t* rowptr, int32_t* col,
                                int32_t* eperm, int32_t* status, const sn_plan_bins* bins, int32_t* scratch,
                                const sn_plan_early* early, void* stream) {
  SN_REQUIRE(N >= 0 && B >= 0 && E >= 0, "sn_batch_plan: negative size");
  SN_REQUIRE(N < (1ll << 31) && E < (1ll << 31), "sn_batch_plan: N/E exceed int32");
  SN_REQUIRE(graph_ptr && node_graph && nvalid && evoff && rowptr && status && scratch,
             "sn_batch_plan: null output");
  SN_REQUIRE(N == 0 || batch, "sn_batch_plan: null batch");
  SN_REQUIRE(E == 0 || (edge_index && col && eperm), "sn_batch_plan: null edge arrays");
  BinsDev bd{};
  const bool do_bins = bins != nullptr;
  if (do_bins) {
    SN_REQUIRE(bins->rho_bin0 && bins->meta && bins->phi_max_bins >= 0, "sn_batch_plan: incomplete sn_plan_bins");
    const int ncolp = (bins->phi_bin_col != nullptr) + (bins->phi_col_bin0 != nullptr) + (bins->phi_col_mem != nullptr) + (bins->phi_col_off != nullptr);
    SN_REQUIRE(ncolp == 4 || (ncolp == 0 && bins->phi_bin_mem), "sn_batch_plan: give all four column arrays of sn_plan_bins, or none of them and phi_bin_mem");
    SN_REQUIRE(B <= BINS_BMAX, "sn_batch_plan: work bins support at most %d graphs per batch (got %lld)", BINS_BMAX, (long long)B);
    SN_REQUIRE(!bins->phi_bin_mem || (reinterpret_cast<uintptr_t>(bins->phi_bin_mem) & 15) == 0, "sn_batch_plan: phi_bin_mem must be 16-byte aligned");
    bd = BinsDev{bins->phi_bin_col, bins->phi_max_bins, bins->phi_col_bin0, bins->phi_col_mem, bins->phi_col_off,
                 bins->rho_bin0, bins->meta, bins->phi_bin_mem};
  }
  EarlyDev ed{};
  if (early != nullptr) {
    SN_REQUIRE(early->host, "sn_batch_plan_ex: sn_plan_early.host (pinned int32[16]) missing");
    SN_REQUIRE(plan_one_launch(N, E, B), "sn_batch_plan_ex: the early report needs the one-launch plan (N <= %d, E <= %d, B <= %d): ask "
               "sn_batch_plan_early_supported first", PS_NMAX, PS_EMAX, PS_BMAX);
    SN_REQUIRE((!early->node_ids && !early->edge_ids) || do_bins, "sn_batch_plan_ex: the feature-id check runs beside the bin planner (bins must be given)");
    SN_REQUIRE((!early->node_ids || (early->n_node_ids >= 0 && early->node_vocab > 0)) && (!early->edge_ids || (early->n_edge_ids >= 0 && early->edge_vocab > 0)),
               "sn_batch_plan_ex: feature-id counts / table rows");
    ed = EarlyDev{early->node_ids, early->node_ids ? early->n_node_ids : 0, early->node_vocab, early->edge_ids,
                  early->edge_ids ? early->n_edge_ids : 0, early->edge_vocab, early->max_graph_edges, early->host};
  }
  hipStream_t st = (hipStream_t)stream;
  if (plan_one_launch(N, E, B)) {
    const size_t lds0 = (size_t)((PS_BMAX + 4) + PS_NMAX + (PS_NMAX + 4) + 2 * PS_EMAX + 32 + PS_NMAX) * sizeof(int);
    const size_t lds1 = (size_t)((PS_BMAX + 4) + PS_BINS_INTS + PAT_INTS) * sizeof(int);
    const size_t lds = lds0 > lds1 ? lds0 : lds1;
    static bool init = false;
    if (!init) {
      if (hipFuncSetAttribute(reinterpret_cast<const void*>(k_plan_small), hipFuncAttributeMaxDynamicSharedMemorySize,
                              (int)lds) != hipSuccess)
        return fail(SN_ERR_LAUNCH, "sn_batch_plan: cannot raise the dynamic LDS limit to %zu", lds);
      init = true;
    }
    const bool ids = ed.host != nullptr && (ed.node_ids != nullptr || ed.edge_ids != nullptr);
    hipLaunchKernelGGL(k_plan_small, dim3(do_bins ? (ids ? 4 : 3) : 1), dim3(PLAN_T), lds, st, batch, (int)N, (int)B, edge_index, (int)E,
                       kmax, graph_ptr, node_graph, nvalid, evoff, rowptr, col, eperm, status, bd, do_bins ? 1 : 0, ed);
    SN_CHECK_LAUNCH("sn_batch_plan");
    return SN_OK;
  }
  int32_t* deg = scratch;
  const int T = 256;
  hipLaunchKernelGGL(k_plan_nodes, dim3((unsigned)cdiv(N > 0 ? N : 1, T)), dim3(T), 0, st, batch, N, B, graph_ptr, node_graph, deg,
                     status);
  const int64_t ne = N > E ? N : E;
  hipLaunchKernelGGL(k_plan_degree, dim3((unsigned)cdiv(ne > 0 ? ne : 1, T)), dim3(T), 0, st, batch, edge_index, E, N, B, deg,
                     status);
  const size_t lds3 = do_bins ? (size_t)((B + 4) + 5 * B + 3 * 66 + 32 + 8 + ((kmax == 0 && B <= PLAN_SLAB_BMAX) ? PAT_INTS : 0)) * sizeof(int) : 0;
  if (lds3 > 48 * 1024) {
    static bool init3 = false;
    if (!init3) {
      if (hipFuncSetAttribute(reinterpret_cast<const void*>(k_plan_scan), hipFuncAttributeMaxDynamicSharedMemorySize,
                              (int)((size_t)(6 * BINS_BMAX + 4 + 3 * 66 + 32 + 8) * sizeof(int))) != hipSuccess)
        return fail(SN_ERR_LAUNCH, "sn_batch_plan: cannot raise the dynamic LDS limit");
      init3 = true;
    }
  }
  hipLaunchKernelGGL(k_plan_scan, dim3(do_bins ? 2 : 1), dim3(PLAN_T), lds3, st, N, B, kmax, graph_ptr, node_graph, deg, rowptr,
                     nvalid, evoff, status, bd);
  if (E > 0) {
    hipLaunchKernelGGL(k_plan_fill, dim3((unsigned)cdiv(E, T)), dim3(T), 0, st, edge_index, E, N, deg, col, eperm);
    hipLaunchKernelGGL(k_plan_sort, dim3((unsigned)cdiv(N, T)), dim3(T), 0, st, N, rowptr, col, eperm);
  }
  SN_CHECK_LAUNCH("sn_batch_plan");
  return SN_OK;
}

extern "C" int sn_batch_plan(const int64_t* batch, int64_t N, int64_t B, const int64_t* edge_index,
                             int64_t E, int kmax, int32_t* graph_ptr, int32_t* node_graph,
                             int32_t* nvalid, int64_t* evoff, int32_t* rowptr, int32_t* col,
                             int32_t* eperm, int32_t* status, const sn_plan_bins* bins, int32_t* scratch,
                             void* stream) {
  return sn_batch_plan_ex(batch, N, B, edge_index, E, kmax, graph_ptr, node_graph, nvalid, evoff, rowptr, col, eperm, status, bins,
                          scratch, nullptr, stream);
}

#ifdef SN_PROFILE
extern "C" int sn_prof_read_plan(long long* host) { return (int)hipMemcpyFromSymbol(host, HIP_SYMBOL(g_pprof), sizeof(long long) * 64); }
#endif

extern "C" int64_t sn_phi_bins_bound(int64_t B, int kmax) {
  const int k = kmax < 0 ? -kmax : kmax;
  const int64_t h = kmax < 0 ? k : ((k > 0 && k < 64) ? k : 64);
  return B * h + 1;
}

extern "C" int sn_pack_eig_f32(const float* eigen_vectors, const float* eigen_values,
                               const int32_t* graph_ptr, const int32_t* node_graph,
                               const int32_t* nvalid, const int64_t* evoff, int64_t N, int K, float* x0,
                               float* s0, void* stream) {
  SN_REQUIRE(K > 0 && N >= 0, "sn_pack_eig_f32: bad sizes");
  SN_REQUIRE(x0 && graph_ptr && node_graph && nvalid && evoff, "sn_pack_eig_f32: null pointer");
  SN_REQUIRE(!s0 || eigen_values, "sn_pack_eig_f32: s0 requested without eigen_values");
  if (N == 0) return SN_OK;
  hipLaunchKernelGGL(k_pack_eig, dim3((unsigned)cdiv(N * K, 256)), dim3(256), 0, (hipStream_t)stream,
                     eigen_vectors, eigen_values, graph_ptr, node_graph, nvalid, evoff, N, K, x0, s0);
  SN_CHECK_LAUNCH("sn_pack_eig_f32");
  return SN_OK;
}

namespace sn {
__global__ __launch_bounds__(256) void k_plan_double(const int32_t* __restrict__ rowptr, const int32_t* __restrict__ col, int64_t N, int64_t E,
                                                     int32_t* __restrict__ rowptr2, int32_t* __restrict__ col2) {
  const int64_t i = (int64_t)blockIdx.x * 256 + threadIdx.x;
  if (i <= N) {
    const int32_t r = rowptr[i];
    rowptr2[i] = r;
    if (i > 0) rowptr2[N + i] = r + (int32_t)E;
  }
  if (i < E) {
    const int32_t c = col[i];
    col2[i] = c;
    col2[E + i] = c + (int32_t)N;
  }
}
}

extern "C" int sn_plan_double_i32(const int32_t* rowptr, const int32_t* col, int64_t N, int64_t E, int32_t* rowptr2, int32_t* col2, void* stream) {
  SN_REQUIRE(rowptr && rowptr2 && N >= 0 && E >= 0 && (E == 0 || (col && col2)), "sn_plan_double_i32: bad arguments");
  SN_REQUIRE(2 * N < (1ll << 31) && 2 * E < (1ll << 31), "sn_plan_double_i32: the doubled graph does not fit 32-bit indices");
  const int64_t work = (N + 1 > E ? N + 1 : E);
  hipLaunchKernelGGL(sn::k_plan_double, dim3((unsigned)sn::cdiv(work, 256)), dim3(256), 0, (hipStream_t)stream, rowptr, col, N, E, rowptr2, col2);
  SN_CHECK_LAUNCH("sn_plan_double_i32");
  return SN_OK;
}
```

signnet_basisnet_amd/fused.py:

```python
from __future__ import annotations

import ctypes as C

import torch

from . import ops
from ._lib import check, lib, ptr, stream

PHI_MAX_LAYERS = 16

PRECISIONS = ops.PRECISIONS
REDUCED_TILES = (4, 7, 8)
REDUCED_TILES_DGL = (4, 5, 6)


def precision_code(name, tiles=None, allowed=REDUCED_TILES, what="this model"):
    if not isinstance(name, str) or name not in PRECISIONS:
        raise ValueError(f"matmul_precision must be one of {sorted(PRECISIONS)} (got {name!r})")
    code = PRECISIONS[name]
    if code and tiles not in allowed:
        raise ValueError(f"matmul_precision={name!r}: the reduced modes of the fused stages are built for widths of "
                         f"{', '.join(str(t) for t in allowed)} 16-channel tiles; {what} has {tiles}. 'highest' serves every width")
    return code


class _PhiLayer(C.Structure):
    _fields_ = [(n, C.c_void_p) for n in ("w1s", "w2s", "eps")]


class _PhiParams(C.Structure):
    _fields_ = [("d", C.c_int), ("n_layers", C.c_int), ("hid0", C.c_int), ("reserved", C.c_int)] + \
               [(n, C.c_void_p) for n in ("l0_w1", "l0_bn0_scale", "l0_bn0_shift", "l0_w2", "l0_bias2", "l0_bn_scale",
                                          "l0_bn_shift", "l0_eps")] + \
               [("layers", _PhiLayer * (PHI_MAX_LAYERS - 1))]


class PhiPlan:

    def __init__(self, phi_module):
        convs, norms = phi_module.convs, phi_module.norms
        L = len(convs)
        d = convs[0].nn.layers[1].weight.shape[0]
        if not (0 < d <= 128 and d % 4 == 0 and 1 <= L <= PHI_MAX_LAYERS):
            raise ValueError("fused phi supports hidden width <= 128 (a multiple of 4) and <= 16 layers")
        dp = 16 * ((d + 15) // 16)
        self.d, self.L, self.dp = d, L, dp
        keep = self._keep = []

        def hold(t):
            keep.append(t)
            return t.data_ptr()

        P = _PhiParams()
        P.d, P.n_layers = d, L
        c0 = convs[0]
        w1 = c0.nn.layers[0].weight.detach()
        hid0 = w1.shape[0]
        if hid0 not in (1, d):
            raise ValueError("fused phi: first hidden width must be 1 or d")
        P.hid0 = hid0
        hp = 16 * ((hid0 + 15) // 16)
        P.l0_w1 = hold(ops.pad_vec(w1[:, 0], hp))
        s, h = ops.bn_fold(c0.nn.norms[0].bn, hp)
        P.l0_bn0_scale, P.l0_bn0_shift = hold(s), hold(h)
        w2 = c0.nn.layers[1].weight.detach()
        b2 = c0.nn.layers[1].bias
        s, h = ops.bn_fold(norms[0].bn, dp)
        if hid0 == 1:
            P.l0_w2 = hold(ops.pad_vec(w2[:, 0], dp))
            P.l0_bias2 = hold(ops.pad_vec(b2, dp)) if b2 is not None else None
            P.l0_bn_scale, P.l0_bn_shift = hold(s), hold(h)
        else:
            P.l0_w2 = hold(ops.pack_split(w2, None if b2 is None else b2.detach(), s, h))
        P.l0_eps = hold(c0.layer.eps.detach())
        for l in range(1, L):
            c, Lp = convs[l], P.layers[l - 1]
            s, h = ops.bn_fold(c.nn.norms[0].bn, dp)
            Lp.w1s = hold(ops.pack_split(c.nn.layers[0].weight.detach(), s, h, None))
            b2 = c.nn.layers[1].bias
            s, h = ops.bn_fold(norms[l].bn, dp)
            Lp.w2s = hold(ops.pack_split(c.nn.layers[1].weight.detach(), None if b2 is None else b2.detach(), s, h))
            Lp.eps = hold(c.layer.eps.detach())
        self.params = P

    def run(self, plan: ops.GraphPlan, eigen_vectors, K: int, out=None, zero_invalid=True, precision=0):
# ... 46 lines not shown
    def _build(self, rho_module, eigen_encoder, heads, ln_eps, hp):
        tls = rho_module.transformer_layers
        d = self.d
        dk = d // heads
        dp = heads * hp if hp else 16 * ((d + 15) // 16)
        keep = self._keep

        def hold(t):
            keep.append(t)
            return t.data_ptr()

        dev = rho_module.out[0].weight.device
        if hp:
            hidx = torch.tensor([h * hp + j for h in range(heads) for j in range(dk)], device=dev)

        def wpad(W, head_rows=False, head_cols=False):
            W = W.detach()
            if not hp:
                return W
            out = torch.zeros(dp, dp, dtype=torch.float32, device=dev)
            rows = hidx if head_rows else torch.arange(W.shape[0], device=dev)
            cols = hidx if head_cols else torch.arange(W.shape[1], device=dev)
            out[rows[:, None], cols[None, :]] = W
            return out

        def vpad(v):
            return ops.pad_vec(v.detach(), dp)

        P = _RhoParams()
        P.d, P.n_layers, P.heads, P.ln_eps, P.head_pad = d, len(tls), heads, float(ln_eps), hp
        P.has_pos = 1 if eigen_encoder is not None else 0
        if eigen_encoder is not None:
            ee = eigen_encoder
            P.pe_w1 = hold(ops.pad_vec(ee.layers[0].weight.detach(), 4))
            s, h = ops.bn_fold(ee.norms[0].bn, 4)
            P.pe_bn0_scale, P.pe_bn0_shift = hold(s), hold(h)
            P.pe_w2 = hold(ops.pad_vec(ee.layers[1].weight.detach()[:, 0], dp))
            s, h = ops.bn_fold(ee.norms[1].bn, dp)
            P.pe_bn1_scale, P.pe_bn1_shift = hold(s), hold(h)
        for l, tl in enumerate(tls):
            a, f, Lp = tl.slf_attn, tl.pos_ffn, P.layers[l]
            Lp.wq = hold(ops.pack_split(wpad(a.w_qs.weight, head_rows=True)))
            Lp.wk = hold(ops.pack_split(wpad(a.w_ks.weight, head_rows=True)))
            Lp.wv = hold(ops.pack_split(wpad(a.w_vs.weight, head_rows=True)))
            Lp.wfc = hold(ops.pack_split(wpad(a.fc.weight, head_cols=True)))
            Lp.ln1_g, Lp.ln1_b = hold(vpad(a.norm.ln.weight)), hold(vpad(a.norm.ln.bias))
            Lp.w1 = hold(ops.pack_split(wpad(f.w_1.weight), vpad(f.w_1.bias) if hp else f.w_1.bias.detach()))
            Lp.w2 = hold(ops.pack_split(wpad(f.w_2.weight), vpad(f.w_2.bias) if hp else f.w_2.bias.detach()))
            Lp.ln2_g, Lp.ln2_b = hold(vpad(f.norm.ln.weight)), hold(vpad(f.norm.ln.bias))
        return P

    def run(self, plan: ops.GraphPlan, x, eigen_values, K: int, precision=0):
        out = torch.empty(plan.N, self.d, dtype=torch.float32, device=x.device)
        kcap = min(plan.kmax, K) if plan.kmax > 0 else K
        params = self.params_hp if (self.params_hp is not None and kcap <= 16) else self.params
        with ops._span("sn_rho_fused_f32"):
            if precision:
                check(lib().sn_rho_fused_prec_f32(C.byref(params), ptr(x), ptr(eigen_values), ptr(plan.graph_ptr), plan.B,
                                                  plan.N, C.byref(plan.bins.cstruct), plan.kmax, K, ptr(out), int(precision), stream()),
                      "sn_rho_fused_prec_f32")
                return out
            check(lib().sn_rho_fused_f32(C.byref(params), ptr(x), ptr(eigen_values), ptr(plan.graph_ptr), plan.B,
                                         plan.N, C.byref(plan.bins.cstruct), plan.kmax, K, ptr(out), stream()),
                  "sn_rho_fused_f32")
        return out


GNN_MAX_LAYERS = 16
GNN_MAX_NODES = 64
GNN_MAX_EDGES = 192


class _GnnLayer(C.Structure):
    _fields_ = [("etab", C.c_void_p * 10)] + \
               [(n, C.c_void_p) for n in ("ew", "e_scale", "e_shift", "w1s", "w2s", "eps")]


class _GnnParams(C.Structure):
    _fields_ = [(n, C.c_int) for n in ("d", "n_layers", "n_out", "reserved", "node_discrete", "node_nf", "edge_discrete",
                                       "edge_nf", "node_vocab", "edge_vocab")] + \
               [("ntab", C.c_void_p * 10)] + \
               [(n, C.c_void_p) for n in ("nw", "n_scale", "n_shift", "rho_out_w", "lin_a", "lin_b", "head_w1", "head_w2")] + \
               [("layers", _GnnLayer * GNN_MAX_LAYERS)]


class GnnPlan:

    def __init__(self, rho_out, gnn, node_feat, edge_feat):
        d = gnn.linear.weight.shape[0]
        L = len(gnn.convs)
        n_out = gnn.output_encoder.layers[1].weight.shape[0]
        if not (0 < d <= 128 and L <= GNN_MAX_LAYERS and 1 <= n_out <= 16 and gnn.pooling == "add"):
            raise ValueError("fused gnn supports hidden width <= 128, <= 16 layers, n_out <= 16, add pooling")
        if (node_feat is not None and node_feat > 16) or (edge_feat is not None and edge_feat > 16):
            raise ValueError("fused gnn supports at most 16 continuous node/edge features")
        dp = 16 * ((d + 15) // 16)
        self.d, self.n_out = d, n_out
        self.node_discrete, self.edge_discrete = node_feat is None, edge_feat is None
        keep = self._keep = []

        def hold(t):
            keep.append(t)
            return t.data_ptr()

        P = _GnnParams()
        P.d, P.n_layers, P.n_out = d, L, n_out
        P.node_discrete, P.edge_discrete = int(self.node_discrete), int(self.edge_discrete)
        P.node_nf = 1 if self.node_discrete else int(node_feat)
        P.edge_nf = 1 if self.edge_discrete else int(edge_feat)
        P.node_vocab = P.edge_vocab = 0
        if self.node_discrete:
            P.node_vocab = gnn.input_encoder.embeddings[0].weight.shape[0]
            for f, e in enumerate(gnn.input_encoder.embeddings):
                P.ntab[f] = hold(e.weight.detach())
        else:
            w = gnn.input_encoder.layers[0].weight.detach()
            wp = torch.zeros(dp, w.shape[1], dtype=torch.float32, device=w.device)
            wp[:d].copy_(w)
            P.nw = hold(wp)
            s, h = ops.bn_fold(gnn.input_encoder.norms[0], dp)
            P.n_scale, P.n_shift = hold(s), hold(h)
        W = gnn.linear.weight.detach()
        Wp = W[:, d:].contiguous()
        s, h = ops.bn_fold(rho_out[1], d)
        A = ops.masked_affine(Wp, scale=s, shift=torch.zeros_like(s))
        Wt = rho_out[0].weight.detach().t().contiguous()
        Wf = ops.masked_linear(A, ops.PackedLinear(ops.pack_weight(Wt), d, d, None))
        bf = ops.masked_linear(h.view(1, d).contiguous(), ops.PackedLinear(ops.pack_weight(Wp), d, d, gnn.linear.bias.detach().contiguous()))
        P.rho_out_w = None
        P.lin_a = hold(ops.pack_split(W[:, :d]))
        P.lin_b = hold(ops.pack_split(Wf, bf.view(-1)))
        oe = gnn.output_encoder
        s, h = ops.bn_fold(oe.norms[0], dp)
        P.head_w1 = hold(ops.pack_split(oe.layers[0].weight.detach(), s, h))
        P.head_w2 = hold(ops.pack_split(oe.layers[1].weight.detach(), oe.layers[1].bias.detach()))
        for l, (enc, conv, norm) in enumerate(zip(gnn.edge_encoders, gnn.convs, gnn.norms)):
            Lp = P.layers[l]
            if self.edge_discrete:
                P.edge_vocab = enc.embeddings[0].weight.shape[0]
                for f, e in enumerate(enc.embeddings):
                    Lp.etab[f] = hold(e.weight.detach())
            else:
                w = enc.layers[0].weight.detach()
                wp = torch.zeros(dp, w.shape[1], dtype=torch.float32, device=w.device)
                wp[:d].copy_(w)
                Lp.ew = hold(wp)
                s, h = ops.bn_fold(enc.norms[0], dp)
                Lp.e_scale, Lp.e_shift = hold(s), hold(h)
            s, h = ops.bn_fold(conv.nn.norms[0], dp)
            Lp.w1s = hold(ops.pack_split(conv.nn.layers[0].weight.detach(), s, h))
            s, h = ops.bn_fold(norm, dp)
            Lp.w2s = hold(ops.pack_split(conv.nn.layers[1].weight.detach(), s, h))
            Lp.eps = hold(conv.layer.eps.detach())
        self.params = P

    def run(self, plan: ops.GraphPlan, x, edge_attr, rho_sum, flags_host=None):
        P = self.params
        if self.node_discrete:
            if x.dtype != torch.int64:
                raise ValueError("discrete node features must be int64")
            x = x.reshape(plan.N, -1).contiguous()
            P.node_nf = x.shape[1]
        else:
            if x.dtype != torch.float32:
                raise ValueError("continuous node features must be float32")
            x = x.reshape(plan.N, -1).contiguous()
        if self.edge_discrete:
            if edge_attr.dtype != torch.int64:
                raise ValueError("discrete edge features must be int64")
            edge_attr = (edge_attr.reshape(plan.E, -1) if plan.E else edge_attr.reshape(0, 1)).contiguous()
            P.edge_nf = edge_attr.shape[1] if plan.E else 1
        else:
            edge_attr = (edge_attr.reshape(plan.E, -1) if plan.E else edge_attr.reshape(0, max(1, int(P.edge_nf)))).contiguous()
        if plan.E == 0:
            edge_attr = torch.zeros(1, max(1, int(P.edge_nf)), dtype=edge_attr.dtype, device=rho_sum.device)
        if P.node_nf > (10 if self.node_discrete else 16) or P.edge_nf > (10 if self.edge_discrete else 16):
            raise ValueError("too many feature columns for the fused gnn kernel")
        y = torch.empty(plan.B, self.n_out, dtype=torch.float32, device=rho_sum.device)
        with ops._span("sn_gnn_fused_f32"):
            check(lib().sn_gnn_fused_f32(C.byref(P), ptr(x), x.shape[1], ptr(edge_attr),
                                         edge_attr.shape[1] if edge_attr.dim() > 1 else 1, ptr(rho_sum),
                                         ptr(plan.graph_ptr), plan.B, ptr(plan.rowptr), ptr(plan.col),
                                         ptr(plan.eperm), ptr(plan.status), ptr(y),
                                         ptr(plan.flags), plan.flags.numel(), ptr(flags_host), stream()),
                  "sn_gnn_fused_f32")
        return y
```

signnet_basisnet_amd/ops.py:

```python
from __future__ import annotations

import ctypes as C
from dataclasses import dataclass

import torch

from . import _lib
from ._lib import (EPI_AFFINE, EPI_BIAS, EPI_LEAKY, EPI_RELU, EPI_RELU_PRE, EPI_RESIDUAL, EPI_RESIDUAL_PRE, check, lib, ptr,
                   require_cuda, stream)

__all__ = ["KernelTimer", "KERNEL_ROOFLINE", "GraphPlan", "PlanBins", "build_plan", "pack_eig", "pack_weight", "gin_aggregate", "gine_aggregate",
           "masked_linear", "masked_colstats", "masked_affine", "masked_layernorm", "set_attention",
           "slot_sum", "embedding_sum", "segment_pool", "PackedLinear",
           "EPI_BIAS", "EPI_RELU_PRE", "EPI_AFFINE", "EPI_RELU", "EPI_RESIDUAL"]


class _NoSpan:
    def __enter__(self):
        return self

    def __exit__(self, *a):
        return False


# ... 13 lines not shown
        return self

    def __exit__(self, *a):
        e1 = torch.cuda.Event(enable_timing=True)
        e1.record()
        self.timer.spans.append((self.name, self.e0, e1))
        return False


class KernelTimer:

    def __init__(self, only=None, stride=1):
        self.only = set(only) if only else None
        self.stride = max(1, int(stride))
        self.seen = {}
        self.spans = []

    def __enter__(self):
        global _active_timer
        _active_timer = self
        return self

    def __exit__(self, *a):
        global _active_timer
        _active_timer = None
        return False

    def summary(self):
        torch.cuda.synchronize()
        acc = {}
        for name, e0, e1 in self.spans:
            n, t = acc.get(name, (0, 0.0))
            acc[name] = (n + 1, t + e0.elapsed_time(e1))
        return {k: (n, t / n) for k, (n, t) in acc.items()}


def _span(name):
    t = _active_timer
    if t is None or (t.only is not None and name not in t.only):
        return _NOSPAN
    if t.stride > 1:
        k = t.seen.get(name, 0)
        t.seen[name] = k + 1
        if k % t.stride:
            return _NOSPAN
    return _Span(t, name)


def _f32c(t, name):
    if t.dtype != torch.float32 or not t.is_contiguous():
        raise ValueError(f"{name}: expected a contiguous float32 tensor, got {t.dtype} contiguous={t.is_contiguous()}")
    return t


@dataclass
class PlanBins:
    phi_bin_col: torch.Tensor
    phi_max_bins: int
    phi_col_bin0: torch.Tensor
    phi_col_mem: torch.Tensor
    phi_col_off: torch.Tensor
    rho_bin0: torch.Tensor
    meta: torch.Tensor
    cstruct: object
    phi_bin_mem: torch.Tensor = None


@dataclass
class GraphPlan:
    N: int
    B: int
    E: int
    kmax: int
    graph_ptr: torch.Tensor
    node_graph: torch.Tensor
    nvalid: torch.Tensor
    evoff: torch.Tensor
    rowptr: torch.Tensor
    col: torch.Tensor
    eperm: torch.Tensor
    status: torch.Tensor
    bins: PlanBins | None
    flags: torch.Tensor = None

    def check(self):
        st = self.status.tolist()
        if st[0]:
            bits = [n for b, n in ((1, "batch not sorted"), (2, "graph id out of range"),
                                   (4, "edge endpoint out of range"), (8, "edge crosses graphs")) if st[0] & b]
            raise ValueError("malformed graph batch: " + ", ".join(bits))
        if st[5] or (st[3] & 4):
            raise IndexError(EMBEDDING_INDEX_ERROR)
        return st


class _PlanBinsC(C.Structure):
    _fields_ = [("phi_bin_col", C.c_void_p), ("phi_max_bins", C.c_int64), ("phi_col_bin0", C.c_void_p),
                ("phi_col_mem", C.c_void_p), ("phi_col_off", C.c_void_p), ("rho_bin0", C.c_void_p), ("meta", C.c_void_p),
                ("node_graph", C.c_void_p), ("phi_bin_mem", C.c_void_p)]


class _PlanEarlyC(C.Structure):
    _fields_ = [("node_ids", C.c_void_p), ("n_node_ids", C.c_int64), ("node_vocab", C.c_int64),
                ("edge_ids", C.c_void_p), ("n_edge_ids", C.c_int64), ("edge_vocab", C.c_int64),
                ("max_graph_edges", C.c_int), ("reserved", C.c_int), ("host", C.c_void_p)]


class EarlyReport:
    ERR, NMAX, DEGMAX, EDGES, PHI, RHO, IDS, DONE = 0, 1, 2, 3, 4, 5, 6, 8
    _pool = []

    def __init__(self):
        if EarlyReport._pool:
            self.t, self.v = EarlyReport._pool.pop()
        else:
            self.t = torch.zeros(16, dtype=torch.int32, pin_memory=True)
            self.v = self.t.numpy()
        self.v[:] = 0
        self.cstruct = None
        self._keep = None

    def arm(self, node_ids=None, node_vocab=0, edge_ids=None, edge_vocab=0, max_graph_edges=0):
        self._keep = (node_ids, edge_ids)
        self.cstruct = _PlanEarlyC(ptr(node_ids), 0 if node_ids is None else node_ids.numel(), int(node_vocab),
                                   ptr(edge_ids), 0 if edge_ids is None else edge_ids.numel(), int(edge_vocab),
                                   int(max_graph_edges), 0, self.t.data_ptr())
        return self

    def wait(self, timeout_s=5.0):
        v = self.v
        if not (v[8] and v[9] and v[10] and v[11]):
            import time
            t_end = time.perf_counter() + timeout_s
            while not (v[8] and v[9] and v[10] and v[11]):
                if time.perf_counter() > t_end:
                    torch.cuda.synchronize()
                    if not (v[8] and v[9] and v[10] and v[11]):
                        raise RuntimeError("sn_batch_plan_ex did not report its flags")
        return v[:8].tolist()

    def wait_nmax(self):
        v = self.v
        if not v[10]:
            import time
            t_end = time.perf_counter() + 5.0
            while not v[10]:
                if time.perf_counter() > t_end:
                    torch.cuda.synchronize()
                    if not v[10]:
                        raise RuntimeError("sn_batch_plan_ex did not report the largest graph")
        return int(v[1])

    def release(self):
        self._keep = self.cstruct = None
        EarlyReport._pool.append((self.t, self.v))


def early_supported(N: int, E: int, B: int) -> bool:
    return bool(lib().sn_batch_plan_early_supported(int(N), int(E), int(B)))


def build_plan(batch: torch.Tensor, edge_index: torch.Tensor, num_graphs: int, kmax: int = 0, bins: bool = False,
               early: "EarlyReport | None" = None, columns: bool = False, counts: torch.Tensor = None) -> GraphPlan:
    require_cuda(batch, edge_index)
    if batch.dtype != torch.int64 or edge_index.dtype != torch.int64:
        raise ValueError("build_plan: batch and edge_index must be int64 (the reference's index dtype)")
    batch = batch.contiguous()
    edge_index = edge_index.contiguous()
    N, E, B = batch.numel(), edge_index.shape[1] if edge_index.numel() else 0, int(num_graphs)
    dev = batch.device
    sizes = [B + 1, N, N, N + 1, E, E, N + 8, 8]
    mb = 0
    if bins:
        mb = int(lib().sn_phi_bins_bound(B, int(kmax)))
        sizes += [8, mb if columns else 0, (B + 1) if columns else 0, (8 * B) if columns else 0, (8 * B) if columns else 0, B + 1, 16 * mb]
    offs = [0]
    for s in sizes:
        offs.append(offs[-1] + ((s + 3) // 4) * 4)
    arena = torch.empty(offs[-1], dtype=torch.int32, device=dev)
    parts = [arena[offs[i]:offs[i] + sizes[i]] for i in range(len(sizes))]
    graph_ptr, node_graph, nvalid, rowptr, col, eperm, scratch, status = parts[:8]
    evoff = torch.empty(B + 1, dtype=torch.int64, device=dev)
    pb = None
    if bins:
        meta, bc, cb0, mem, off, rb0, bmem = parts[8:15]
        if columns:
            cs = _PlanBinsC(bc.data_ptr(), mb, cb0.data_ptr(), mem.data_ptr(), off.data_ptr(), rb0.data_ptr(), meta.data_ptr(),
                            node_graph.data_ptr(), bmem.data_ptr())
        else:
            bc = cb0 = mem = off = None
            cs = _PlanBinsC(None, mb, None, None, None, rb0.data_ptr(), meta.data_ptr(), node_graph.data_ptr(), bmem.data_ptr())
        pb = PlanBins(bc, mb, cb0, mem, off, rb0, meta, cs, bmem)
    if counts is not None:
        with _span("sn_batch_plan_padded"):
            check(lib().sn_batch_plan_padded(ptr(batch), N, B, ptr(edge_index), E, int(kmax), ptr(graph_ptr), ptr(node_graph),
                                             ptr(nvalid), ptr(evoff), ptr(rowptr), ptr(col), ptr(eperm), ptr(status),
                                             C.byref(pb.cstruct) if pb is not None else None, ptr(scratch),
                                             C.byref(early.cstruct) if early is not None else None, ptr(counts), stream()),
                  "sn_batch_plan_padded")
    else:
        with _span("sn_batch_plan"):
            check(lib().sn_batch_plan_ex(ptr(batch), N, B, ptr(edge_index), E, int(kmax), ptr(graph_ptr), ptr(node_graph),
                                         ptr(nvalid), ptr(evoff), ptr(rowptr), ptr(col), ptr(eperm), ptr(status),
                                         C.byref(pb.cstruct) if pb is not None else None, ptr(scratch),
                                         C.byref(early.cstruct) if early is not None else None, stream()), "sn_batch_plan")
    plan = GraphPlan(N, B, E, int(kmax), graph_ptr, node_graph, nvalid, evoff, rowptr, col, eperm, status, pb)
    plan.flags = arena[offs[7]:offs[7] + 16] if bins else status
    return plan


def pack_eig(plan: GraphPlan, eigen_vectors, eigen_values, K: int, want_values: bool):
    require_cuda(eigen_vectors)
    ev = _f32c(eigen_vectors, "eigen_vectors")
    x0 = torch.empty(plan.N, K, dtype=torch.float32, device=ev.device)
    s0 = torch.empty_like(x0) if want_values else None
    es = _f32c(eigen_values, "eigen_values") if want_values else None
    with _span("sn_pack_eig_f32"):
        check(lib().sn_pack_eig_f32(ptr(ev), ptr(es), ptr(plan.graph_ptr), ptr(plan.node_graph), ptr(plan.nvalid),
                                    ptr(plan.evoff), plan.N, K, ptr(x0), ptr(s0), stream()), "sn_pack_eig_f32")
    return x0, s0


PHI_BIN_ROWS = 64


def bn_fold(bn, c_pad=None):
    Cc = bn.num_features
    cp = Cc if c_pad is None else int(c_pad)
    dev = bn.running_mean.device
    require_cuda(bn.running_mean)
    scale = torch.empty(cp, dtype=torch.float32, device=dev)
    shift = torch.empty(cp, dtype=torch.float32, device=dev)
    w = bn.weight.detach() if bn.affine else None
    b = bn.bias.detach() if bn.affine else None
    check(lib().sn_bn_fold_f32(ptr(w), ptr(b), ptr(bn.running_mean), ptr(bn.running_var), float(bn.eps), Cc, cp,
                               ptr(scale), ptr(shift), stream()), "sn_bn_fold_f32")
    return scale, shift


def pad_vec(v, c_pad):
    v = v.detach().reshape(-1)
    out = torch.zeros(c_pad, dtype=torch.float32, device=v.device)
    out[:v.numel()].copy_(v)
    return out


def packed_floats(d_out: int, d_in: int) -> int:
    return int(lib().sn_packed_weight_floats(d_out, d_in))


def pack_weight(W: torch.Tensor, out: torch.Tensor | None = None) -> torch.Tensor:
    require_cuda(W)
    if W.dtype != torch.float32 or W.dim() != 2 or W.stride(1) != 1:
        raise ValueError("pack_weight: expected a float32 [d_out, d_in] matrix with unit inner stride")
    d_out, d_in = W.shape
    n = packed_floats(d_out, d_in)
    if out is None:
        out = torch.empty(n, dtype=torch.float32, device=W.device)
    check(lib().sn_pack_weight_f32(ptr(W), d_out, d_in, W.stride(0), ptr(out), stream()), "sn_pack_weight_f32")
    return out


def pack_weight_t(W: torch.Tensor) -> torch.Tensor:
    require_cuda(W)
    if W.dtype != torch.float32 or W.dim() != 2 or W.stride(1) != 1:
        raise ValueError("pack_weight_t: expected a float32 matrix with unit inner stride")
    rows, cols = W.shape
    out = torch.empty(packed_floats(cols, rows), dtype=torch.float32, device=W.device)
    check(lib().sn_pack_weight_t_f32(ptr(W), rows, cols, W.stride(0), ptr(out), stream()), "sn_pack_weight_t_f32")
    return out


def pack_split(W: torch.Tensor, e0=None, e1=None, e2=None) -> torch.Tensor:
    require_cuda(W)
    if W.dtype != torch.float32 or W.dim() != 2 or W.stride(1) != 1:
        raise ValueError("pack_split: expected a float32 [d_out, d_in] matrix with unit inner stride")
    d_out, d_in = W.shape
    vecs = []
    for e in (e0, e1, e2):
        if e is not None:
            e = e.detach().to(device=W.device, dtype=torch.float32).contiguous()
            if e.numel() < d_out:
                raise ValueError("pack_split: epilogue vector shorter than d_out")
        vecs.append(e)
    out = torch.empty(int(lib().sn_split_packed_bytes(d_out, d_in)), dtype=torch.uint8, device=W.device)
    check(lib().sn_pack_split_f32(ptr(W), d_out, d_in, W.stride(0), ptr(vecs[0]), ptr(vecs[1]), ptr(vecs[2]), ptr(out),
                                  stream()), "sn_pack_split_f32")
    return out


# ... 913 lines not shown
```

signnet_basisnet_amd/pyg.py:

```python
from __future__ import annotations

import time

import torch
import torch.nn as nn

from . import _lib as _lib_mod
from . import fused, ops

import os as _os
MAX_FUSED_GRAPHS = 6144
_NO_KERNEL_FLAGS = bool(_os.environ.get("SN_NO_KERNEL_FLAGS"))
N_HEAD = 4
LN_EPS = 1e-6


class MaskedBN(nn.Module):
    def __init__(self, c):
        super().__init__()
        self.bn = nn.BatchNorm1d(c)

    def reset_parameters(self):
        self.bn.reset_parameters()

# ... 634 lines not shown
        def lin(x_, m, relu=False):
            return T.linear_module(x_, m, nv, K, relu) if stage else AG.linear(x_, m.weight, m.bias, nv, K, relu=relu)
        static_masks = getattr(self, "_attn_masks", None)
        for li, tl in enumerate(sn.rho.transformer_layers):
            a, f = tl.slf_attn, tl.pos_ffn
            q, k, v = T.qkv(x, a.w_qs, a.w_ks, a.w_vs, nv, K) if stage else (lin(x, a.w_qs), lin(x, a.w_ks), lin(x, a.w_vs))
            pm = static_masks[li] if static_masks is not None else None
            if pm is not None and tuple(pm.shape) != (N, N_HEAD, K, K):
                pm = None
            if pm is None:
                pm = ops.attention_dropout_mask(N, K, N_HEAD, self.attn_dropout, x.device)
            o = AG.set_attention(q, k, v, N, K, N_HEAD, nv, pm)
            o = lin(o, a.fc)
            y = AG.masked_layernorm(o, x, a.norm.ln.weight, a.norm.ln.bias, LN_EPS, nv, K)
            z = lin(y, f.w_1, relu=True)
            z = lin(z, f.w_2)
            x = AG.masked_layernorm(z, y, f.norm.ln.weight, f.norm.ln.bias, LN_EPS, nv, K)
        s = AG.slot_sum(x, N, K, nv)
        pe = lin_bn(s, sn.rho.out[0], sn.rho.out[1], vN, k1, relu=False)
        xin = data.x.squeeze() if data.x.dim() > 1 and data.x.shape[-1] == 1 else data.x
        if isinstance(g.input_encoder, DiscreteEncoder):
            h = AG.embedding_sum(xin, [e.weight for e in g.input_encoder.embeddings], plan.status[5:6])
        else:
            h = lin_bn(xin.contiguous(), g.input_encoder.layers[0], g.input_encoder.norms[0], vN, k1)
        h = AG.linear(torch.cat([h, pe], dim=-1), g.linear.weight, g.linear.bias, vN, k1)
        staged = [stage and isinstance(conv.nn.norms[0], nn.BatchNorm1d) and isinstance(norm, nn.BatchNorm1d)
                  for conv, norm in zip(g.convs, g.norms)]
        e_all = None
        if all(staged) and all(isinstance(enc, DiscreteEncoder) for enc in g.edge_encoders) and 1 < len(g.edge_encoders) <= 16:
            e_all = AG.embedding_sum_layers(data.edge_attr, [[t.weight for t in enc.embeddings] for enc in g.edge_encoders], plan.status[5:6])
        for li, (enc, conv, norm) in enumerate(zip(g.edge_encoders, g.convs, g.norms)):
            if e_all is not None:
                h = T.gine_layer(h, e_all, conv.layer.eps, conv.nn.layers[0], conv.nn.norms[0], conv.nn.layers[1], norm, plan, rplan, layer=li,
                                 nvalid=vN, K=k1)
                continue
            if isinstance(enc, DiscreteEncoder):
                e = AG.embedding_sum(data.edge_attr, [t.weight for t in enc.embeddings], plan.status[5:6])
            else:
                e = lin_bn(data.edge_attr.contiguous(), enc.layers[0], enc.norms[0], vE, k1)
            if staged[li]:
                h = T.gine_layer(h, e, conv.layer.eps, conv.nn.layers[0], conv.nn.norms[0], conv.nn.layers[1], norm, plan, rplan,
                                 nvalid=vN, K=k1)
            else:
                u = AG.gine_aggregate(h, e, conv.layer.eps, plan, rplan)
                u = lin_bn(u, conv.nn.layers[0], conv.nn.norms[0], vN, k1)
                h = lin_bn(u, conv.nn.layers[1], norm, vN, k1, residual=h)
        pooled = AG.segment_pool(h, plan, g.pooling)
        oe = g.output_encoder
        y = lin_bn(pooled, oe.layers[0], oe.norms[0], vB, k1)
        y = AG.linear(y, oe.layers[1].weight, oe.layers[1].bias, vB, k1)
        discrete = isinstance(g.input_encoder, DiscreteEncoder) or any(isinstance(e, DiscreteEncoder) for e in g.edge_encoders)
        self._train_status = plan.status if discrete else None
        if not getattr(self, "_defer_status", False):
            self.check_train()
        return y

    def check_train(self):
        st, self._train_status = getattr(self, "_train_status", None), None
        if st is not None and int(st[5]):
            raise IndexError(ops.EMBEDDING_INDEX_ERROR)

    @staticmethod
    def _arm_early(gplan, data):
        xi = ei = None
        nv = ev = 0
        if gplan.node_discrete and data.x.dtype == torch.int64 and data.x.is_cuda:
            xi, nv = data.x.contiguous(), int(gplan.params.node_vocab)
        if gplan.edge_discrete and int(gplan.params.n_layers) > 0 and data.edge_attr.dtype == torch.int64 and data.edge_attr.is_cuda \
                and data.edge_attr.numel() > 0:
            ei, ev = data.edge_attr.contiguous(), int(gplan.params.edge_vocab)
        return ops.EarlyReport().arm(xi, nv, ei, ev, fused.GNN_MAX_EDGES)

    def _forward_overlapped(self, data, P, B):
        d = self.cfg["n_hid"]
        dev = data.batch.device
        cur = torch.cuda.current_stream(dev)
        if self._side_streams is None:
            self._side_streams = (torch.cuda.Stream(device=dev), torch.cuda.Stream(device=dev))
        side_a, side_b = self._side_streams
        if not self.overlap_inputs_ready:
            side_a.wait_stream(cur)
        want_vals = "eig" in P or "eig2" in P
        with torch.cuda.stream(side_a), _lib_mod.stream_scope():
            plan = ops.build_plan(data.batch, data.edge_index, B, self.max_k or 0, bins=True)
            K_host = None if self.max_k else host_max_nodes(data)
            K = int(self.max_k) if self.max_k else (int(K_host) if K_host is not None else plan.check()[1])
            x = P["phi_fused"].run(plan, data.eigen_vectors, K, zero_invalid=False, precision=self._prec).view(plan.N * K, d)
            ev_a = torch.cuda.Event()
            ev_a.record(side_a)
        side_b.wait_event(ev_a)
        with torch.cuda.stream(side_b), _lib_mod.stream_scope():
            s = P["rho_fused"].run(plan, x, data.eigen_values if want_vals else None, K, precision=self._prec)
            ev_b = torch.cuda.Event()
            ev_b.record(side_b)
        cur.wait_event(ev_b)
        for t in (data.batch, data.edge_index, data.eigen_vectors):
            t.record_stream(side_a)
        if want_vals:
            data.eigen_values.record_stream(side_b)
        for t in (plan.graph_ptr, plan.evoff):
            t.record_stream(side_b)
            t.record_stream(cur)
        x.record_stream(side_b)
        s.record_stream(cur)
        self._last_plan, self._used_fused, self._last_K = plan, True, K
        with _lib_mod.stream_scope():
            self._flags_host = self._host_flags() if (plan.bins is not None and not _NO_KERNEL_FLAGS) else None
            if self._flags_host is not None:
                self._flags_host[1][:] = 0
            return P["gnn_fused"].run(plan, data.x, data.edge_attr, s, None if self._flags_host is None else self._flags_host[0])

    def _forward(self, data, return_stages=False, train=False, force_layer=False):
        ops.require_cuda(data.edge_index, data.batch, data.eigen_vectors)
        if self._prep is None:
            self._prep = self._prepare(train)
        P = self._prep
        B = int(data.num_graphs)
        use_phi_fused = P["phi_fused"] is not None and not force_layer
        use_rho_fused = P["rho_fused"] is not None and not force_layer
        use_gnn_fused = P["gnn_fused"] is not None and not force_layer
        if (self.overlap_front and use_phi_fused and use_rho_fused and use_gnn_fused and not return_stages and not train
                and not self.strict):
            return self._forward_overlapped(data, P, B)
        all_fused = use_phi_fused and use_rho_fused and use_gnn_fused and not return_stages and not train
        early = None
        N_, E_n = int(data.batch.numel()), (int(data.edge_index.shape[1]) if data.edge_index.numel() else 0)
        capturing = torch.cuda.is_current_stream_capturing()
        if all_fused and self.strict and not capturing and ops.early_supported(N_, E_n, B):
            early = self._arm_early(P["gnn_fused"], data)
        K_host = None if self.max_k else host_max_nodes(data)
        if not self.max_k and K_host is None and early is None and not return_stages and not capturing and ops.early_supported(N_, E_n, B):
            early = ops.EarlyReport().arm()
        plan = ops.build_plan(data.batch, data.edge_index, B, self.max_k or 0, bins=use_phi_fused or use_rho_fused, early=early)
        self._last_plan, self._used_fused = plan, (use_phi_fused or use_rho_fused or use_gnn_fused)
        if self.max_k:
            K = int(self.max_k)
            plan.check() if return_stages else None
        elif K_host is not None:
            K = int(K_host)
            plan.check() if return_stages else None
        elif early is not None:
            K = early.wait_nmax()
        else:
            K = plan.check()[1]
        if early is not None and not (all_fused and self.strict):
            early.wait()
            early.release()
            early = None
        self._early, self._last_K = early, K
        N, d = plan.N, self.cfg["n_hid"]
        nv = plan.nvalid
        want_vals = "eig" in P or "eig2" in P
        x0 = s0 = None
        if return_stages or not (use_phi_fused and use_rho_fused):
            x0, s0 = ops.pack_eig(plan, data.eigen_vectors, data.eigen_values if want_vals else None, K, want_vals)
        stages = {}

        if "eig2" in P:
            E2 = P["eig2"]
            p2 = _lin_bn(s0.view(N * K, 1), E2["l0"], E2["bn0"], True, nv, K, relu=True)
            _lin_bn(p2, E2["l1"], E2["bn1"], True, nv, K, relu=True)
        phis = None
        if use_phi_fused and not return_stages:
            x = P["phi_fused"].run(plan, data.eigen_vectors, K, zero_invalid=not use_rho_fused, precision=self._prec).view(N * K, d)
        else:
            phis = []
            for sign in (0, 1):
                x, prev = x0, None
                for l, L in enumerate(P["phi"]):
                    a = ops.gin_aggregate(x.view(N, -1), plan, L["eps"], negate=(sign == 1 and l == 0))
                    h = _lin_bn(a.view(N * K, -1), L["l0"], L["bn0"], train, nv, K, relu=True)
                    x = _lin_bn(h, L["l1"], L["bn"], train, nv, K, relu=True, residual=prev)
                    prev = x
                phis.append(x)
            x = ops.masked_affine(phis[0], nv, K, residual=phis[1])
        if return_stages:
            stages.update(phi_plus=phis[0].view(N, K, d), phi_minus=phis[1].view(N, K, d), phi=x.view(N, K, d))
            if P["phi_fused"] is not None:
                stages["phi_fused"] = P["phi_fused"].run(plan, data.eigen_vectors, K, precision=self._prec)
                stages["bins_meta"] = plan.bins.meta
        x_phi = x
        if use_rho_fused and not return_stages:
            s = P["rho_fused"].run(plan, x_phi, data.eigen_values if want_vals else None, K, precision=self._prec)
        else:
            if "eig" in P:
                E_ = P["eig"]
                p = _lin_bn(s0.view(N * K, 1), E_["l0"], E_["bn0"], train, nv, K, relu=True)
                p = _lin_bn(p, E_["l1"], E_["bn1"], train, nv, K, relu=True)
                x = ops.masked_affine(x, nv, K, residual=p)
            given = getattr(self, "_attn_masks", None) if train else None
            for li, L in enumerate(P["rho"]):
                q = ops.masked_linear(x, L["q"], nv, K)
                k = ops.masked_linear(x, L["k"], nv, K)
                v = ops.masked_linear(x, L["v"], nv, K)
                pm = None
                if train:
                    pm = given[li] if given is not None else ops.attention_dropout_mask(N, K, N_HEAD, self.attn_dropout, x.device)
                o = ops.set_attention(q, k, v, N, K, N_HEAD, nv, pm)
                o = ops.masked_linear(o, L["fc"], nv, K)
                y = ops.masked_layernorm(o, x, L["ln1"][0], L["ln1"][1], LN_EPS, nv, K)
                z = ops.masked_linear(y, L["w1"], nv, K, relu=True)
                z = ops.masked_linear(z, L["w2"], nv, K)
                x = ops.masked_layernorm(z, y, L["ln2"][0], L["ln2"][1], LN_EPS, nv, K)
            s = ops.slot_sum(x, N, K)
        if use_gnn_fused and not return_stages:
            self._flags_host = self._host_flags() if (plan.bins is not None and not _NO_KERNEL_FLAGS and self._early is None) else None
            if self._flags_host is not None:
                self._flags_host[1][:] = 0
            return P["gnn_fused"].run(plan, data.x, data.edge_attr, s, None if self._flags_host is None else self._flags_host[0])
        pe = _lin_bn(s, P["rho_out"]["l"], P["rho_out"]["bn"], train, relu=False)
        if return_stages:
            stages["pos"] = pe
            stages["rho_sum"] = s
            if use_rho_fused:
                rho_in = stages["phi_fused"].view(N * K, d) if (self._prec and "phi_fused" in stages) else x_phi
                stages["rho_sum_fused"] = P["rho_fused"].run(plan, rho_in, data.eigen_values if want_vals else None, K, precision=self._prec)
# ... 28 lines not shown
```

Before: 536,300.

## Precompute GINE front tables and per-node edge records in the batch plan

New measurement: 512,900. -4.4%, worse.

```diff
diff --git a/include/signnet_hip.h b/include/signnet_hip.h
--- a/include/signnet_hip.h
+++ b/include/signnet_hip.h
@@ -450,6 +450,30 @@
                      void* stream);
 
 
+typedef struct {
+  const int64_t* edge_attr;
+  int64_t lde;
+  int classes, reserved;
+  int32_t* records;
+} sn_plan_gnn;
+int sn_batch_plan_gnn(const int64_t* batch, int64_t N, int64_t B, const int64_t* edge_index, int64_t E, int kmax, int32_t* graph_ptr,
+                      int32_t* node_graph, int32_t* nvalid, int64_t* evoff, int32_t* rowptr, int32_t* col, int32_t* eperm,
+                      int32_t* status, const sn_plan_bins* bins, int32_t* scratch, const sn_plan_early* early, const sn_plan_gnn* gnn,
+                      void* stream);
+
+typedef struct {
+  const float* node_tab;
+  const float* edge_tab;
+  const int32_t* records;
+  int64_t n_nodes;
+} sn_gnn_front;
+int sn_gnn_front_classes(const sn_gnn_params* params, int* classes);
+int sn_gnn_front_tables_f32(const sn_gnn_params* params, float* node_tab, float* edge_tab, void* stream);
+int sn_gnn_fused_front_f32(const sn_gnn_params* params, const sn_gnn_front* front, const void* x, int ldx, const void* edge_attr, int lde,
+                           const float* rho_sum, const int32_t* graph_ptr, int64_t B, const int32_t* rowptr, const int32_t* col,
+                           const int32_t* eperm, int32_t* status, float* y, const int32_t* flags_src, int n_flags, int32_t* flags_host,
+                           void* stream);
+
 int sn_gin_net_fused_f32(const sn_gnn_params* params, const void* head_mid, int pool_mean, const int64_t* atom, const float* p, int ldp,
                          int kp, const int32_t* graph_ptr, int64_t B, const int32_t* rowptr, const int32_t* col, const int32_t* eperm,
                          int32_t* status, float* y, const int32_t* flags_src, int n_flags, void* stream);
diff --git a/signnet_basisnet_amd/_lib.py b/signnet_basisnet_amd/_lib.py
--- a/signnet_basisnet_amd/_lib.py
+++ b/signnet_basisnet_amd/_lib.py
@@ -21,6 +21,7 @@
     "sn_clock_probe": [_l, _p, _p],
     "sn_batch_plan": [_p, _l, _l, _p, _l, _i, _p, _p, _p, _p, _p, _p, _p, _p, _p, _p, _p],
     "sn_batch_plan_ex": [_p, _l, _l, _p, _l, _i, _p, _p, _p, _p, _p, _p, _p, _p, _p, _p, _p, _p],
+    "sn_batch_plan_gnn": [_p, _l, _l, _p, _l, _i, _p, _p, _p, _p, _p, _p, _p, _p, _p, _p, _p, _p, _p],
     "sn_batch_plan_early_supported": [_l, _l, _l],
     "sn_pack_eig_f32": [_p, _p, _p, _p, _p, _p, _l, _i, _p, _p, _p],
     "sn_bucket_pack": [_p, _p],
@@ -49,6 +50,9 @@
     "sn_phi_fused_prec_f32": [_p, _p, _p, _p, _p, _p, _p, _i, _i, _p, _i, _p],
     "sn_rho_fused_prec_f32": [_p, _p, _p, _p, _l, _l, _p, _i, _i, _p, _i, _p],
     "sn_gnn_fused_f32": [_p, _p, _i, _p, _i, _p, _p, _l, _p, _p, _p, _p, _p, _p, _i, _p, _p],
+    "sn_gnn_front_classes": [_p, C.POINTER(_i)],
+    "sn_gnn_front_tables_f32": [_p, _p, _p, _p],
+    "sn_gnn_fused_front_f32": [_p, _p, _p, _i, _p, _i, _p, _p, _l, _p, _p, _p, _p, _p, _p, _i, _p, _p],
     "sn_gin_net_fused_f32": [_p, _p, _i, _p, _p, _i, _i, _p, _l, _p, _p, _p, _p, _p, _p, _i, _p],
     "sn_transformer_net_fused_f32": [_p, _p, _i, _p, _p, _i, _i, _p, _i, _p, _l, _p, _p, _p, _p, _p, _p, _i, _p],
     "sn_masked_colstats_f32": [_p, _i, _l, _i, _p, _i, _p, _p, _p, _p, _p],
diff --git a/signnet_basisnet_amd/csrc/fused_gnn.hip b/signnet_basisnet_amd/csrc/fused_gnn.hip
--- a/signnet_basisnet_amd/csrc/fused_gnn.hip
+++ b/signnet_basisnet_amd/csrc/fused_gnn.hip
@@ -42,6 +42,11 @@
   int rho_ld, rho_w;
   const void* head_mid;
   int pool_mean;
+  const float* node_tab;
+  const float* edge_tab;
+  int edge_cls;
+  const int32_t* gnn_rec;
+  int64_t n_nodes;
 };
 
 __device__ __forceinline__ void sp_store4(unsigned char* img, int row, int ot, int g, f32x4 v) {
@@ -261,10 +266,11 @@
   }
 }
 
-template <int NT, int MODE = 0, int TC = 0>
+template <int NT, int MODE = 0, int TC = 0, bool FAST = false>
 __device__ __forceinline__ void gnn_graph(const GnnStruct& S, const sn_gnn_params& P) {
   constexpr bool DGL = MODE != 0, TF = MODE == 2;
   static_assert(TC == 0 || (NT == 8 && MODE == 0), "compile-time row tiles: the GINE net at NT = 8");
+  static_assert(!FAST || MODE == 0, "the fast front is the GINE net's");
   static_assert(!TF || NT == 4, "the Transformer mode is written for d = 64");
   constexpr int D = 16 * NT;
   constexpr int LD = D + 4;
@@ -297,8 +303,8 @@
   if (S.flags_src != nullptr && (S.flags_src[0] != 0 || (S.n_flags >= 16 && (S.flags_src[9] != 0 || S.flags_src[13] != 0)))) { give_up(0); return; }
   if (n <= 0) { give_up(8); return; }
   if (n > GNN_ROWS) { give_up(1); return; }
-  const int e_base = S.rowptr[gs];
-  const int ne = S.rowptr[gs + n] - e_base;
+  const int e_base = FAST ? 0 : S.rowptr[gs];
+  const int ne = FAST ? 0 : S.rowptr[gs + n] - e_base;
   const int d = P.d;
   __shared__ unsigned s_pro[3];
   if (threadIdx.x == 0) { s_pro[0] = 0u; s_pro[1] = 0u; s_pro[2] = 0u; }
@@ -391,7 +397,20 @@
   h2.t_hi = wave == 0 ? 1 : 0;
   static_assert(GNN_EMAX <= GNN_WAVES * 64 && GNN_ROWS < GNN_WAVES * 64 && GNN_ROWS * (D / 4) <= 4 * GNN_WAVES * 64, "one pass of the block covers the graph");
   const int tid = threadIdx.x;
-  const int rp_v = tid <= n ? S.rowptr[gs + tid] : 0;
+  const int rp_v = (!FAST && tid <= n) ? S.rowptr[gs + tid] : 0;
+  int4 rec[4];
+#pragma unroll
+  for (int i = 0; i < 4; ++i) {
+    rec[i] = make_int4(-1, 0, 0, 0);
+    if constexpr (FAST) {
+      const int t = tr.t_lo + i;
+      if (t < tr.t_hi) {
+        int ot, rt;
+        tr.decode(t, ot, rt);
+        if (rt * 16 + li < n) rec[i] = reinterpret_cast<const int4*>(S.gnn_rec)[gs + rt * 16 + li];
+      }
+    }
+  }
   const int rho_ld = S.rho_ld, rho_w = S.rho_w;
   const bool rs_vec = ((rho_ld | rho_w) & 3) == 0;
   f32x4 rs_v[4];
@@ -404,7 +423,7 @@
       if (4 * c4 < rho_w) rs_v[j] = ld4(S.rho_sum + (int64_t)(gs + rr) * rho_ld + 4 * c4);
     }
   }
-  const bool xid_pref = P.node_discrete && P.node_nf == 1 && (d & 3) == 0;
+  const bool xid_pref = FAST || (P.node_discrete && P.node_nf == 1 && (d & 3) == 0);
   long long xid[4];
 #pragma unroll
   for (int i = 0; i < 4; ++i) {
@@ -416,9 +435,23 @@
       if (rt * 16 + li < n) xid[i] = reinterpret_cast<const int64_t*>(S.x)[(int64_t)(gs + rt * 16 + li) * S.ldx];
     }
   }
+  if constexpr (FAST) {
+    ncls = S.edge_cls;
+    use_tab = true;
+    use_ee = false;
+    tab_pending = true;
+    int t0 = threadIdx.x;
+    asm volatile("" : "+v"(t0));
+#pragma unroll
+    for (int i = 0; i < GNN_EEPF; ++i) {
+      const int idx = t0 + i * GNN_WAVES * 64;
+      eepf[i] = zero4;
+      if (idx < P.n_layers * ncls * (D / 4)) eepf[i] = ld4(S.edge_tab + 4 * idx);
+    }
+  }
   if (ne > GNN_EMAX) { give_up(2); return; }
-  const int src_v = tid < ne ? S.col[e_base + tid] : 0;
-  const int eid_v = tid < ne ? S.eperm[e_base + tid] : 0;
+  const int src_v = (!FAST && tid < ne) ? S.col[e_base + tid] : 0;
+  const int eid_v = (!FAST && tid < ne) ? S.eperm[e_base + tid] : 0;
   SN_STAMP(30);
   for (int i = threadIdx.x; i < 2 * SP_IMAGE / 16; i += GNN_WAVES * 64)
     reinterpret_cast<uint4*>(lds_raw)[i] = make_uint4(0u, 0u, 0u, 0u);
@@ -427,7 +460,7 @@
   SN_STAMP(31);
   const bool efast = !DGL && P.n_layers > 0 && P.edge_discrete && P.edge_nf == 1 && (d & 3) == 0;
   int my_ev = 0;
-  {
+  if constexpr (!FAST) {
     const int EF = P.edge_nf;
     if (tid <= n) erow[tid] = rp_v - e_base;
     if (tid < ne) {
@@ -466,16 +499,25 @@
       long long xv = xid[i];
       if ((uint64_t)xv >= (uint64_t)P.node_vocab) { xv = 0; atomicOr(&S.status[3], 4); atomicOr(&s_pro[0], 1u); }
       const int c = 16 * ot + 4 * g;
-      if (c < d) nrow[i] = ld4(P.ntab[0] + xv * d + c);
-    }
-  }
-  if (!tr.empty()) {
+      if constexpr (FAST) nrow[i] = ld4(S.node_tab + xv * D + c);
+      else if (c < d) nrow[i] = ld4(P.ntab[0] + xv * d + c);
+    }
+  }
+  const void* first_w = P.n_layers > 0 ? P.layers[0].w1s : P.head_w1;
+  const TileRange first_tr = P.n_layers > 0 ? tr : hr;
+  if constexpr (FAST) {
+    if constexpr (ROLL) {
+      if (!tr.empty()) wload<NKB>(alt, P.lin_b, tr.first_ot(), lane);
+      if (!first_tr.empty()) wload<NKB>(pre, first_w, first_tr.first_ot(), lane);
+    } else if (!tr.empty()) wload<NKB>(pre, P.lin_b, tr.first_ot(), lane);
+  } else if (!tr.empty()) {
     wload<NKB>(pre, P.lin_a, tr.first_ot(), lane);
     if constexpr (ROLL) wload<NKB>(alt, P.lin_b, tr.first_ot(), lane);
   }
-  lds_barrier();
+  if constexpr (!FAST) lds_barrier();
   SN_STAMP(32);
-  if (efast && s_pro[1] == 0u) {
+  if (FAST) {
+  } else if (efast && s_pro[1] == 0u) {
     const unsigned present = s_pro[2];
     ncls = __popc(present);
     if (tid < ne) ecls[tid] = __popc(present & ((1u << my_ev) - 1u));
@@ -499,7 +541,7 @@
       }
     }
   }
-  if (!DGL && P.n_layers > 0 && !tab_pending && !(efast && s_pro[1] == 0u)) {
+  if (!FAST && !DGL && P.n_layers > 0 && !tab_pending && !(efast && s_pro[1] == 0u)) {
     const int EF = P.edge_nf;
     __shared__ unsigned long long lmask[(GNN_EMAX + 63) / 64];
     int lead = -1;
@@ -568,7 +610,17 @@
     }
   }
   SN_STAMP(34);
-  if (xid_pref) {
+  if constexpr (FAST) {
+#pragma unroll
+    for (int i = 0; i < 4; ++i) {
+      const int t = tr.t_lo + i;
+      if (t < tr.t_hi) {
+        int ot, rt;
+        tr.decode(t, ot, rt);
+        lds_st4(X1 + (rt * 16 + li) * LD + 16 * ot + 4 * g, nrow[i]);
+      }
+    }
+  } else if (xid_pref) {
 #pragma unroll
     for (int i = 0; i < 4; ++i) {
       const int t = tr.t_lo + i;
@@ -632,7 +684,11 @@
       int ot, rt;
       tr.decode(t, ot, rt);
       const int row = rt * 16 + li;
-      if (row < n) {
+      if constexpr (FAST) {
+        a_dg[i] = rec[i].x;
+        a_sr[i] = (unsigned)rec[i].y;
+        a_er[i] = (unsigned)rec[i].z;
+      } else if (row < n) {
         const int e_lo = erow[row], dg = erow[row + 1] - e_lo;
         a_dg[i] = dg;
 #pragma unroll
@@ -645,8 +701,6 @@
     }
   }
   ee_fetch(0);
-  const void* first_w = P.n_layers > 0 ? P.layers[0].w1s : P.head_w1;
-  const TileRange first_tr = P.n_layers > 0 ? tr : hr;
   {
     auto epi_a = [&](int rt, int ot, f32x4 acc, f32x4, f32x4, f32x4) { lds_st4(X1 + (rt * 16 + li) * LD + 16 * ot + 4 * g, acc); };
     auto epi_b = [&](int rt, int ot, f32x4 acc, f32x4 bias, f32x4, f32x4) {
@@ -654,7 +708,8 @@
       lds_st4(o, (lds_ld4(o) + acc) + bias);
     };
     const bool hasl = P.n_layers > 0;
-    if constexpr (TC > 0) coop_gemm_weave<NKB, TC>(pre, SB, wave, lane, epi_a, first_w, first_tr.first_ot());
+    if constexpr (FAST) { }
+    else if constexpr (TC > 0) coop_gemm_weave<NKB, TC>(pre, SB, wave, lane, epi_a, first_w, first_tr.first_ot());
     else if constexpr (ROLL) coop_gemm_roll<NKB>(pre, SB, tr, lane, epi_a, first_w, first_tr);
     else coop_gemm<NKB>(pre, alt, P.lin_a, SB, tr, lane, epi_a, P.lin_b, tr);
     SN_STAMP(20);
@@ -804,7 +859,7 @@
             f32x4 u = zero4;
 #pragma unroll
             for (int k = 0; k < 4; ++k) u += DGL ? hv[k] : relu4(hv[k] + ev[k]);
-            if (dg > 4) {
+            if (!FAST && dg > 4) {
               const int e_lo = erow[row], e_hi = e_lo + dg;
               for (int e = e_lo + 4; e < e_hi; ++e) {
                 if (DGL) { u += lds_ld4(X1 + esrc[e] * LD + c); continue; }
@@ -927,22 +982,32 @@
 #endif
 }
 
-template <int NT, int MODE = 0>
-__global__ __launch_bounds__(GNN_WAVES * 64, 2) void k_gnn_coop(GnnStruct S, sn_gnn_params P) {
+template <int NT, int MODE, bool FAST>
+__device__ __forceinline__ void gnn_coop_graph(const GnnStruct& S, const sn_gnn_params& P) {
   if constexpr (NT == 8 && MODE == 0) {
     const int n = S.graph_ptr[blockIdx.x + 1] - S.graph_ptr[blockIdx.x];
     switch ((n + 15) >> 4) {
-      case 1: gnn_graph<NT, MODE, 1>(S, P); break;
-      case 2: gnn_graph<NT, MODE, 2>(S, P); break;
-      case 3: gnn_graph<NT, MODE, 3>(S, P); break;
-      case 4: gnn_graph<NT, MODE, 4>(S, P); break;
+      case 1: gnn_graph<NT, MODE, 1, FAST>(S, P); break;
+      case 2: gnn_graph<NT, MODE, 2, FAST>(S, P); break;
+      case 3: gnn_graph<NT, MODE, 3, FAST>(S, P); break;
+      case 4: gnn_graph<NT, MODE, 4, FAST>(S, P); break;
       default:
         if (threadIdx.x == 0) atomicOr(&S.status[3], n > GNN_ROWS ? 1 : 8);
         if ((int)threadIdx.x < P.n_out) S.y[(int64_t)blockIdx.x * P.n_out + threadIdx.x] = __uint_as_float(0x7fc00000u);
         break;
     }
   } else {
-    gnn_graph<NT, MODE>(S, P);
+    gnn_graph<NT, MODE, 0, FAST>(S, P);
+  }
+}
+
+template <int NT, int MODE = 0, bool FAST = false>
+__global__ __launch_bounds__(GNN_WAVES * 64, 2) void k_gnn_coop(GnnStruct S, sn_gnn_params P) {
+  if constexpr (FAST) {
+    if (S.gnn_rec[4 * (S.n_nodes + (int64_t)blockIdx.x) + 3] != 0) gnn_graph<NT, MODE, 0, false>(S, P);
+    else gnn_coop_graph<NT, MODE, true>(S, P);
+  } else {
+    gnn_coop_graph<NT, MODE, false>(S, P);
   }
   if (S.flags_host != nullptr) {
     __syncthreads();
@@ -959,18 +1024,32 @@
     }
   }
 }
-
-template <int NT, int MODE = 0>
-static int launch_gnn(const GnnStruct& S, const sn_gnn_params& P, int64_t B, hipStream_t st) {
-  constexpr bool DGL = MODE != 0;
+constexpr size_t GNN_LDS_CAP = 160 * 1024 - 512;
+template <int NT>
+static size_t gnn_lds_base(int edge_nf) {
   constexpr int LD = 16 * NT + 4;
-  const size_t base = (size_t)2 * SP_IMAGE + (size_t)((GNN_ROWS + 1) * LD) * sizeof(float) +
-                      (size_t)(GNN_ROWS + 4 + GNN_EMAX * (3 + (P.n_layers > 0 ? P.edge_nf : 0)) + GNN_CLS) * sizeof(int);
-  const size_t lds_cap = 160 * 1024 - 512;
+  return (size_t)2 * SP_IMAGE + (size_t)((GNN_ROWS + 1) * LD) * sizeof(float) +
+         (size_t)(GNN_ROWS + 4 + GNN_EMAX * (3 + edge_nf) + GNN_CLS) * sizeof(int);
+}
+template <int NT>
+static int gnn_ee_rows(int edge_nf) {
+  constexpr int LD = 16 * NT + 4;
+  const size_t base = gnn_lds_base<NT>(edge_nf);
+  const size_t lds_cap = GNN_LDS_CAP;
   const size_t room = base < lds_cap ? lds_cap - base : 0;
   int ee_rows = (int)(room / ((size_t)LD * sizeof(float))) - 1;
   if (ee_rows > GNN_EEMAX) ee_rows = GNN_EEMAX;
-  if (ee_rows < 0) ee_rows = 0;
+  return ee_rows < 0 ? 0 : ee_rows;
+}
+
+template <int NT, int MODE = 0, bool FAST = false>
+static int launch_gnn(const GnnStruct& S, const sn_gnn_params& P, int64_t B, hipStream_t st, const char* name = "sn_gnn_fused_f32") {
+  constexpr bool DGL = MODE != 0;
+  constexpr int LD = 16 * NT + 4;
+  const int edge_nf = P.n_layers > 0 ? P.edge_nf : 0;
+  const size_t base = gnn_lds_base<NT>(edge_nf);
+  const size_t lds_cap = GNN_LDS_CAP;
+  const int ee_rows = gnn_ee_rows<NT>(edge_nf);
   GnnStruct S2 = S;
   S2.ee_rows = MODE == 2 ? GNN_ROWS : ((!DGL && P.n_layers > 0) ? ee_rows : 0);
   const size_t lds = base + (size_t)(S2.ee_rows + 1) * LD * sizeof(float);
@@ -978,13 +1057,81 @@
   if (!init) {
     const size_t lds_max = lds_cap;
     if (lds_max > 64 * 1024 &&
-        hipFuncSetAttribute(reinterpret_cast<const void*>(k_gnn_coop<NT, MODE>), hipFuncAttributeMaxDynamicSharedMemorySize,
+        hipFuncSetAttribute(reinterpret_cast<const void*>(k_gnn_coop<NT, MODE, FAST>), hipFuncAttributeMaxDynamicSharedMemorySize,
                             (int)lds_max) != hipSuccess)
-      return fail(SN_ERR_LAUNCH, "sn_gnn_fused_f32: cannot raise the dynamic LDS limit to %zu", lds_max);
+      return fail(SN_ERR_LAUNCH, "%s: cannot raise the dynamic LDS limit to %zu", name, lds_max);
     init = true;
   }
-  hipLaunchKernelGGL((k_gnn_coop<NT, MODE>), dim3((unsigned)B), dim3(GNN_WAVES * 64), lds, st, S2, P);
+  hipLaunchKernelGGL((k_gnn_coop<NT, MODE, FAST>), dim3((unsigned)B), dim3(GNN_WAVES * 64), lds, st, S2, P);
   return SN_OK;
+}
+
+template <int NT>
+__global__ __launch_bounds__(GNN_WAVES * 64) void k_gnn_node_tab(sn_gnn_params P, float* __restrict__ out) {
+  constexpr int D = 16 * NT, NKB = (NT + 1) / 2;
+  extern __shared__ __align__(16) unsigned char lds_raw[];
+  unsigned char* SB = lds_raw;
+  const int lane = threadIdx.x & 63, wave = threadIdx.x >> 6, g = lane >> 4, li = lane & 15;
+  const int r0 = blockIdx.x * GNN_ROWS;
+  const int n = P.node_vocab - r0 < GNN_ROWS ? P.node_vocab - r0 : GNN_ROWS;
+  const int d = P.d;
+  for (int i = threadIdx.x; i < SP_IMAGE / 16; i += GNN_WAVES * 64) reinterpret_cast<uint4*>(lds_raw)[i] = make_uint4(0u, 0u, 0u, 0u);
+  __syncthreads();
+  for (int i = threadIdx.x; i < n * (D / 4); i += GNN_WAVES * 64) {
+    const int rr = i / (D / 4), c4 = i % (D / 4);
+    f32x4 v = {0.f, 0.f, 0.f, 0.f};
+    if (4 * c4 < d) v = ld4(P.ntab[0] + (int64_t)(r0 + rr) * d + 4 * c4);
+    sp_store4(SB, rr, c4 >> 2, c4 & 3, v);
+  }
+  __syncthreads();
+  const int T = (n + 15) >> 4;
+  auto epi = [&](int rt, int ot, f32x4 acc, f32x4, f32x4, f32x4) {
+    const int row = rt * 16 + li;
+    if (row < n) *reinterpret_cast<float4*>(out + (int64_t)(r0 + row) * D + 16 * ot + 4 * g) = make_float4(acc[0], acc[1], acc[2], acc[3]);
+  };
+  for (int t = wave; t < NT * T; t += GNN_WAVES) {
+    TileRange one;
+    one.T = T;
+    one.t_lo = t;
+    one.t_hi = t + 1;
+    WSplit<NKB> w;
+    wload<NKB>(w, P.lin_a, t / T, lane);
+    coop_gemm_roll<NKB>(w, SB, one, lane, epi, nullptr, one);
+  }
+}
+
+__global__ void k_gnn_edge_tab(sn_gnn_params P, int ncls, int D, float* __restrict__ out) {
+  const int row = blockIdx.x, l = row / ncls, v = row - l * ncls;
+  for (int c = threadIdx.x; c < D; c += blockDim.x) out[(int64_t)row * D + c] = c < P.d ? P.layers[l].etab[0][(int64_t)v * P.d + c] : 0.f;
+}
+
+template <int NT>
+static void launch_node_tab(const sn_gnn_params& P, float* out, hipStream_t st) {
+  hipLaunchKernelGGL((k_gnn_node_tab<NT>), dim3((unsigned)((P.node_vocab + GNN_ROWS - 1) / GNN_ROWS)), dim3(GNN_WAVES * 64), SP_IMAGE, st, P, out);
+}
+
+static int gnn_ee_rows_of(int d) {
+  switch ((d + 15) / 16) {
+    case 1: return gnn_ee_rows<1>(1);
+    case 2: return gnn_ee_rows<2>(1);
+    case 3: return gnn_ee_rows<3>(1);
+    case 4: return gnn_ee_rows<4>(1);
+    case 5: return gnn_ee_rows<5>(1);
+    case 6: return gnn_ee_rows<6>(1);
+    case 7: return gnn_ee_rows<7>(1);
+    default: return gnn_ee_rows<8>(1);
+  }
+}
+
+static int gnn_front_classes(const sn_gnn_params& P) {
+  int c = P.n_layers > 0 ? gnn_ee_rows_of(P.d) / P.n_layers : 0;
+  if (c > GNN_CLS) c = GNN_CLS;
+  return c < P.edge_vocab ? c : P.edge_vocab;
+}
+
+static bool gnn_front_params_ok(const sn_gnn_params& P) {
+  return P.d > 0 && P.d <= 128 && (P.d & 3) == 0 && P.n_layers >= 1 && P.n_layers <= SN_GNN_MAX_LAYERS && P.node_discrete == 1 &&
+         P.node_nf == 1 && P.edge_discrete == 1 && P.edge_nf == 1 && P.node_vocab > 0 && P.edge_vocab > 0 && gnn_front_classes(P) >= 1;
 }
 
 }
@@ -996,51 +1143,123 @@
 extern "C" int sn_prof_set_block(int b) { return (int)hipMemcpyToSymbol(HIP_SYMBOL(g_prof_block), &b, sizeof(int)); }
 #endif
 
+template <bool FAST>
+static int gnn_dispatch(const GnnStruct& S, const sn_gnn_params& P, int64_t B, hipStream_t st, const char* name) {
+  switch ((P.d + 15) / 16) {
+    case 1: return launch_gnn<1, 0, FAST>(S, P, B, st, name);
+    case 2: return launch_gnn<2, 0, FAST>(S, P, B, st, name);
+    case 3: return launch_gnn<3, 0, FAST>(S, P, B, st, name);
+    case 4: return launch_gnn<4, 0, FAST>(S, P, B, st, name);
+    case 5: return launch_gnn<5, 0, FAST>(S, P, B, st, name);
+    case 6: return launch_gnn<6, 0, FAST>(S, P, B, st, name);
+    case 7: return launch_gnn<7, 0, FAST>(S, P, B, st, name);
+    default: return launch_gnn<8, 0, FAST>(S, P, B, st, name);
+  }
+}
+
+static int gnn_fused(const char* name, const sn_gnn_params* params, const sn_gnn_front* front, const void* x, int ldx, const void* edge_attr, int lde,
+                     const float* rho_sum, const int32_t* graph_ptr, int64_t B, const int32_t* rowptr,
+                     const int32_t* col, const int32_t* eperm, int32_t* status, float* y,
+                     const int32_t* flags_src, int n_flags, int32_t* flags_host, void* stream) {
+  SN_REQUIRE(params && x && rho_sum && graph_ptr && rowptr && status && y && B >= 0, "%s: null pointer", name);
+  const sn_gnn_params& P = *params;
+  SN_REQUIRE(P.d > 0 && P.d <= 128, "%s: hidden width %d not in (0, 128]", name, P.d);
+  SN_REQUIRE(P.n_layers >= 0 && P.n_layers <= SN_GNN_MAX_LAYERS, "%s: %d layers unsupported", name, P.n_layers);
+  SN_REQUIRE(P.n_out >= 1 && P.n_out <= 16, "%s: n_out=%d not in [1,16]", name, P.n_out);
+  SN_REQUIRE(P.node_nf >= 1 && P.node_nf <= (P.node_discrete ? 10 : 16) && ldx >= P.node_nf,
+             "%s: node feature count %d unsupported", name, P.node_nf);
+  SN_REQUIRE(P.n_layers == 0 || (edge_attr && P.edge_nf >= 1 && P.edge_nf <= (P.edge_discrete ? 10 : 16) && lde >= P.edge_nf),
+             "%s: edge feature count %d unsupported", name, P.edge_nf);
+  SN_REQUIRE(P.lin_a && P.lin_b && P.head_w1 && P.head_w2, "%s: parameters missing", name);
+  SN_REQUIRE(P.rho_out_w == nullptr, "%s: rho_out_w must be NULL — fold rho.out into lin_b (see signnet_hip.h)", name);
+  if (P.node_discrete) { for (int f = 0; f < P.node_nf; ++f) SN_REQUIRE(P.ntab[f], "%s: node table %d missing", name, f); }
+  else SN_REQUIRE(P.nw && P.n_scale && P.n_shift, "%s: node MLP parameters missing", name);
+  for (int l = 0; l < P.n_layers; ++l) {
+    const sn_gnn_layer& L = P.layers[l];
+    SN_REQUIRE(L.w1s && L.w2s && L.eps, "%s: layer %d parameters missing", name, l);
+    if (P.edge_discrete) { for (int f = 0; f < P.edge_nf; ++f) SN_REQUIRE(L.etab[f], "%s: layer %d edge table %d missing", name, l, f); }
+    else SN_REQUIRE(L.ew && L.e_scale && L.e_shift, "%s: layer %d edge MLP parameters missing", name, l);
+  }
+  if (B == 0) return SN_OK;
+  SN_REQUIRE(!flags_host || (flags_src && n_flags > 0 && n_flags <= 64), "%s: flag report needs flags_src and 0 < n_flags <= 64", name);
+  SN_REQUIRE(!flags_src || n_flags >= 1, "%s: flags_src needs n_flags >= 1", name);
+  SN_REQUIRE((!P.node_discrete || P.node_vocab > 0) && (P.n_layers == 0 || !P.edge_discrete || P.edge_vocab > 0),
+             "%s: node_vocab / edge_vocab (rows of the embedding tables) missing", name);
+  GnnStruct S{x, ldx, edge_attr, lde, rho_sum, graph_ptr, rowptr, col, eperm, status, y, 0, flags_src, n_flags, flags_host,
+              P.d, P.d, nullptr, 0, nullptr, nullptr, 0, nullptr, 0};
+  hipStream_t st = (hipStream_t)stream;
+  int rc;
+  if (front != nullptr) {
+    S.node_tab = front->node_tab;
+    S.edge_tab = front->edge_tab;
+    S.edge_cls = gnn_front_classes(P);
+    S.gnn_rec = front->records;
+    S.n_nodes = front->n_nodes;
+    rc = gnn_dispatch<true>(S, P, B, st, name);
+  } else {
+    rc = gnn_dispatch<false>(S, P, B, st, name);
+  }
+  if (rc != SN_OK) return rc;
+  SN_CHECK_LAUNCH(name);
+  return SN_OK;
+}
+
 extern "C" int sn_gnn_fused_f32(const sn_gnn_params* params, const void* x, int ldx, const void* edge_attr, int lde,
                                 const float* rho_sum, const int32_t* graph_ptr, int64_t B, const int32_t* rowptr,
                                 const int32_t* col, const int32_t* eperm, int32_t* status, float* y,
                                 const int32_t* flags_src, int n_flags, int32_t* flags_host, void* stream) {
-  SN_REQUIRE(params && x && rho_sum && graph_ptr && rowptr && status && y && B >= 0, "sn_gnn_fused_f32: null pointer");
+  return gnn_fused("sn_gnn_fused_f32", params, nullptr, x, ldx, edge_attr, lde, rho_sum, graph_ptr, B, rowptr, col, eperm, status, y, flags_src, n_flags,
+                   flags_host, stream);
+}
+
+extern "C" int sn_gnn_front_classes(const sn_gnn_params* params, int* classes) {
+  SN_REQUIRE(params && classes, "sn_gnn_front_classes: null pointer");
+  SN_REQUIRE(params->d > 0 && params->d <= 128, "sn_gnn_front_classes: hidden width %d not in (0, 128]", params->d);
+  SN_REQUIRE(params->n_layers >= 0 && params->n_layers <= SN_GNN_MAX_LAYERS, "sn_gnn_front_classes: %d layers unsupported", params->n_layers);
+  *classes = gnn_front_params_ok(*params) ? gnn_front_classes(*params) : 0;
+  return SN_OK;
+}
+
+extern "C" int sn_gnn_front_tables_f32(const sn_gnn_params* params, float* node_tab, float* edge_tab, void* stream) {
+  SN_REQUIRE(params && node_tab && edge_tab, "sn_gnn_front_tables_f32: null pointer");
   const sn_gnn_params& P = *params;
-  SN_REQUIRE(P.d > 0 && P.d <= 128, "sn_gnn_fused_f32: hidden width %d not in (0, 128]", P.d);
-  SN_REQUIRE(P.n_layers >= 0 && P.n_layers <= SN_GNN_MAX_LAYERS, "sn_gnn_fused_f32: %d layers unsupported", P.n_layers);
-  SN_REQUIRE(P.n_out >= 1 && P.n_out <= 16, "sn_gnn_fused_f32: n_out=%d not in [1,16]", P.n_out);
-  SN_REQUIRE(P.node_nf >= 1 && P.node_nf <= (P.node_discrete ? 10 : 16) && ldx >= P.node_nf,
-             "sn_gnn_fused_f32: node feature count %d unsupported", P.node_nf);
-  SN_REQUIRE(P.n_layers == 0 || (edge_attr && P.edge_nf >= 1 && P.edge_nf <= (P.edge_discrete ? 10 : 16) && lde >= P.edge_nf),
-             "sn_gnn_fused_f32: edge feature count %d unsupported", P.edge_nf);
-  SN_REQUIRE(P.lin_a && P.lin_b && P.head_w1 && P.head_w2, "sn_gnn_fused_f32: parameters missing");
-  SN_REQUIRE(P.rho_out_w == nullptr, "sn_gnn_fused_f32: rho_out_w must be NULL — fold rho.out into lin_b (see signnet_hip.h)");
-  if (P.node_discrete) { for (int f = 0; f < P.node_nf; ++f) SN_REQUIRE(P.ntab[f], "sn_gnn_fused_f32: node table %d missing", f); }
-  else SN_REQUIRE(P.nw && P.n_scale && P.n_shift, "sn_gnn_fused_f32: node MLP parameters missing");
-  for (int l = 0; l < P.n_layers; ++l) {
-    const sn_gnn_layer& L = P.layers[l];
-    SN_REQUIRE(L.w1s && L.w2s && L.eps, "sn_gnn_fused_f32: layer %d parameters missing", l);
-    if (P.edge_discrete) { for (int f = 0; f < P.edge_nf; ++f) SN_REQUIRE(L.etab[f], "sn_gnn_fused_f32: layer %d edge table %d missing", l, f); }
-    else SN_REQUIRE(L.ew && L.e_scale && L.e_shift, "sn_gnn_fused_f32: layer %d edge MLP parameters missing", l);
-  }
-  if (B == 0) return SN_OK;
-  SN_REQUIRE(!flags_host || (flags_src && n_flags > 0 && n_flags <= 64), "sn_gnn_fused_f32: flag report needs flags_src and 0 < n_flags <= 64");
-  SN_REQUIRE(!flags_src || n_flags >= 1, "sn_gnn_fused_f32: flags_src needs n_flags >= 1");
-  SN_REQUIRE((!P.node_discrete || P.node_vocab > 0) && (P.n_layers == 0 || !P.edge_discrete || P.edge_vocab > 0),
-             "sn_gnn_fused_f32: node_vocab / edge_vocab (rows of the embedding tables) missing");
-  GnnStruct S{x, ldx, edge_attr, lde, rho_sum, graph_ptr, rowptr, col, eperm, status, y, 0, flags_src, n_flags, flags_host,
-              P.d, P.d, nullptr, 0};
+  SN_REQUIRE(gnn_front_params_ok(P), "sn_gnn_front_tables_f32: the fast front takes one discrete node feature and one discrete edge feature "
+             "(sn_gnn_front_classes > 0), d a multiple of 4 in (0, 128]");
+  SN_REQUIRE(P.lin_a && P.ntab[0], "sn_gnn_front_tables_f32: lin_a / ntab[0] missing");
+  for (int l = 0; l < P.n_layers; ++l) SN_REQUIRE(P.layers[l].etab[0], "sn_gnn_front_tables_f32: layer %d edge table missing", l);
+  SN_REQUIRE(((reinterpret_cast<uintptr_t>(node_tab) | reinterpret_cast<uintptr_t>(edge_tab)) & 15) == 0,
+             "sn_gnn_front_tables_f32: the tables must be 16-byte aligned");
   hipStream_t st = (hipStream_t)stream;
-  int rc = SN_OK;
-  switch ((P.d + 15) / 16) {
-    case 1: rc = launch_gnn<1>(S, P, B, st); break;
-    case 2: rc = launch_gnn<2>(S, P, B, st); break;
-    case 3: rc = launch_gnn<3>(S, P, B, st); break;
-    case 4: rc = launch_gnn<4>(S, P, B, st); break;
-    case 5: rc = launch_gnn<5>(S, P, B, st); break;
-    case 6: rc = launch_gnn<6>(S, P, B, st); break;
-    case 7: rc = launch_gnn<7>(S, P, B, st); break;
-    default: rc = launch_gnn<8>(S, P, B, st); break;
-  }
-  if (rc != SN_OK) return rc;
-  SN_CHECK_LAUNCH("sn_gnn_fused_f32");
+  const int NT = (P.d + 15) / 16;
+  switch (NT) {
+    case 1: launch_node_tab<1>(P, node_tab, st); break;
+    case 2: launch_node_tab<2>(P, node_tab, st); break;
+    case 3: launch_node_tab<3>(P, node_tab, st); break;
+    case 4: launch_node_tab<4>(P, node_tab, st); break;
+    case 5: launch_node_tab<5>(P, node_tab, st); break;
+    case 6: launch_node_tab<6>(P, node_tab, st); break;
+    case 7: launch_node_tab<7>(P, node_tab, st); break;
+    default: launch_node_tab<8>(P, node_tab, st); break;
+  }
+  const int ncls = gnn_front_classes(P);
+  hipLaunchKernelGGL(k_gnn_edge_tab, dim3((unsigned)(P.n_layers * ncls)), dim3(128), 0, st, P, ncls, 16 * NT, edge_tab);
+  SN_CHECK_LAUNCH("sn_gnn_front_tables_f32");
   return SN_OK;
+}
+
+extern "C" int sn_gnn_fused_front_f32(const sn_gnn_params* params, const sn_gnn_front* front, const void* x, int ldx, const void* edge_attr,
+                                      int lde, const float* rho_sum, const int32_t* graph_ptr, int64_t B, const int32_t* rowptr,
+                                      const int32_t* col, const int32_t* eperm, int32_t* status, float* y, const int32_t* flags_src,
+                                      int n_flags, int32_t* flags_host, void* stream) {
+  SN_REQUIRE(params && front && front->node_tab && front->edge_tab, "sn_gnn_fused_front_f32: null pointer");
+  SN_REQUIRE(gnn_front_params_ok(*params), "sn_gnn_fused_front_f32: these parameters take the full front (sn_gnn_fused_f32): one discrete "
+             "node feature, one discrete edge feature, sn_gnn_front_classes > 0");
+  SN_REQUIRE(((reinterpret_cast<uintptr_t>(front->node_tab) | reinterpret_cast<uintptr_t>(front->edge_tab)) & 15) == 0,
+             "sn_gnn_fused_front_f32: the tables must be 16-byte aligned");
+  SN_REQUIRE(front->records && front->n_nodes >= 0 && (reinterpret_cast<uintptr_t>(front->records) & 15) == 0,
+             "sn_gnn_fused_front_f32: the planner's records (sn_batch_plan_gnn) of this batch are missing or not 16-byte aligned");
+  return gnn_fused("sn_gnn_fused_front_f32", params, front, x, ldx, edge_attr, lde, rho_sum, graph_ptr, B, rowptr, col, eperm, status, y, flags_src, n_flags,
+                   flags_host, stream);
 }
 
 extern "C" int sn_gin_net_fused_f32(const sn_gnn_params* params, const void* head_mid, int pool_mean, const int64_t* atom, const float* p,
diff --git a/signnet_basisnet_amd/csrc/plan.hip b/signnet_basisnet_amd/csrc/plan.hip
--- a/signnet_basisnet_amd/csrc/plan.hip
+++ b/signnet_basisnet_amd/csrc/plan.hip
@@ -449,6 +449,12 @@
 constexpr int PS_NMAX = 4096, PS_EMAX = 12288, PS_BMAX = 1024;
 constexpr int PS_BINS_INTS = 5 * PS_BMAX + 3 * 66 + 32 + 8;
 
+struct GnnRec { const int64_t* ea; int32_t* row; int lde_cls; };
+__device__ __forceinline__ int32_t* gnn_graph_rec(const GnnRec& gr, long long N) { return gr.row + 4 * N; }
+constexpr int GR_NONE_SRC = 64, GR_NONE_CLS = 255, GR_MAX_NODES = 64, GR_MAX_EDGES = 255, GR_BAD = 16;
+__device__ __forceinline__ int gnn_edge_code(const GnnRec& gr, long long v) { return (v >= 0 && v < (gr.lde_cls & 31)) ? (int)v : GR_BAD; }
+__device__ __forceinline__ int gnn_graph_flag(int n, int ne) { return (n <= 0 || n > GR_MAX_NODES || ne > GR_MAX_EDGES) ? 1 : 0; }
+
 
 
 __global__ __launch_bounds__(PLAN_T) void k_plan_small(const int64_t* __restrict__ batch, int N, int B,
@@ -457,7 +463,7 @@
                                                        int32_t* __restrict__ nvalid, int64_t* __restrict__ evoff,
                                                        int32_t* __restrict__ rowptr, int32_t* __restrict__ col,
                                                        int32_t* __restrict__ eperm, int32_t* __restrict__ status, BinsDev bd,
-                                                       int do_bins, EarlyDev early) {
+                                                       int do_bins, EarlyDev early, GnnRec gr) {
   extern __shared__ int sm[];
   const int t = threadIdx.x;
   PL_STAMP(0);
@@ -521,6 +527,7 @@
     bprev[k] = (i < N && i > 0) ? batch[i - 1] : -1;
   }
   int es[EPT], ed[EPT];
+  int ecode[EPT];
   {
     long long sv[EPT], dv[EPT];
 #pragma unroll
@@ -560,6 +567,11 @@
   }
   __syncthreads();
   PL_STAMP(1);
+#pragma unroll
+  for (int k = 0; k < EPT; ++k) {
+    const int e = t + k * PLAN_T;
+    ecode[k] = (gr.row != nullptr && e < E) ? gnn_edge_code(gr, gr.ea[(long long)e * (gr.lde_cls >> 5)]) : 0;
+  }
   int epos[EPT];
 #pragma unroll
   for (int k = 0; k < EPT; ++k) {
@@ -600,6 +612,8 @@
 #pragma unroll
   for (int k = 0; k < EPT; ++k)
     if (ed[k] >= 0) lfill[rp[ed[k]] + epos[k]] = ((t + k * PLAN_T) << 12) | es[k];
+  if (gr.row != nullptr)
+    for (int g = t; g < B; g += PLAN_T) deg[g] = 0;
   if (early.host != nullptr && early.max_graph_edges > 0) {
     for (int g = t; g < B; g += PLAN_T)
       if (rp[gp[g + 1]] - rp[gp[g]] > early.max_graph_edges) atomicOr(&s_big, 1);
@@ -613,13 +627,52 @@
       const int lo = rp[ed[k]], hi = rp[ed[k] + 1];
       int rank = 0;
       for (int q = lo; q < hi; ++q) rank += lfill[q] < key ? 1 : 0;
-      lperm[lo + rank] = key;
+      lperm[lo + rank] = key | (ecode[k] << 26);
     }
   }
   __syncthreads();
   PL_STAMP(5);
+  auto node_record = [&](int i, unsigned& srw, unsigned& erw, int& dg) __attribute__((always_inline)) -> bool {
+    const int lo = rp[i], g = ng[i], gs = g >= 0 ? gp[g] : 0;
+    dg = rp[i + 1] - lo;
+    bool bad = dg > 4;
+    srw = 0u; erw = 0u;
+#pragma unroll
+    for (int q = 0; q < 4; ++q) {
+      int sr = GR_NONE_SRC, cl = GR_NONE_CLS;
+      if (q < dg) {
+        const int key = lperm[lo + q];
+        sr = (key & 4095) - gs;
+        cl = (key >> 26) & 31;
+        bad = bad || cl >= GR_BAD || sr < 0 || sr >= GR_MAX_NODES;
+      }
+      srw |= (unsigned)(sr & 255) << (8 * q);
+      erw |= (unsigned)(cl & 255) << (8 * q);
+    }
+    return bad;
+  };
+  if (gr.row != nullptr) {
+    for (int i = t; i < N; i += PLAN_T) {
+      unsigned srw, erw;
+      int dg;
+      if (node_record(i, srw, erw, dg) && ng[i] >= 0) atomicOr(&deg[ng[i]], 1);
+    }
+    __syncthreads();
+  }
   for (int i = t; i <= N; i += PLAN_T) rowptr[i] = rp[i];
-  for (int i = t; i < E; i += PLAN_T) { const int k = lperm[i]; col[i] = k & 4095; eperm[i] = k >> 12; }
+  for (int i = t; i < E; i += PLAN_T) { const int k = lperm[i]; col[i] = k & 4095; eperm[i] = (k >> 12) & 0x3fff; }
+  if (gr.row != nullptr) {
+    for (int i = t; i < N; i += PLAN_T) {
+      unsigned srw, erw;
+      int dg;
+      node_record(i, srw, erw, dg);
+      reinterpret_cast<int4*>(gr.row)[i] = make_int4(dg, (int)srw, (int)erw, 0);
+    }
+    for (int g = t; g < B; g += PLAN_T) {
+      const int gs = gp[g], n = gp[g + 1] - gs, e0 = rp[gs], ne = rp[gp[g + 1]] - e0;
+      reinterpret_cast<int4*>(gnn_graph_rec(gr, N))[g] = make_int4(gs, n, e0, deg[g] | gnn_graph_flag(n, ne));
+    }
+  }
   for (int i = t; i <= B; i += PLAN_T) graph_ptr[i] = gp[i];
   for (int i = t; i < N; i += PLAN_T) {
     const int g = ng[i];
@@ -646,8 +699,10 @@
 
 __global__ void k_plan_nodes(const int64_t* __restrict__ batch, int64_t N, int64_t B,
                              int32_t* __restrict__ graph_ptr, int32_t* __restrict__ node_graph,
-                             int32_t* __restrict__ deg, int32_t* __restrict__ status) {
+                             int32_t* __restrict__ deg, int32_t* __restrict__ status, int32_t* __restrict__ gnn_graph) {
   const int64_t i = (int64_t)blockIdx.x * blockDim.x + threadIdx.x;
+  if (gnn_graph != nullptr)
+    for (int64_t b = i; b < B; b += (int64_t)gridDim.x * blockDim.x) gnn_graph[4 * b + 3] = 0;
   if (i < 8) status[i] = 0;
   if (i == 0) graph_ptr[B] = (int32_t)N;
   if (i >= N) return;
@@ -775,8 +830,17 @@
 }
 
 __global__ void k_plan_sort(int64_t N, const int32_t* __restrict__ rowptr, int32_t* __restrict__ col,
-                            int32_t* __restrict__ eperm) {
+                            int32_t* __restrict__ eperm, int64_t B, const int32_t* __restrict__ graph_ptr,
+                            const int32_t* __restrict__ node_graph, GnnRec gr) {
   int64_t i = (int64_t)blockIdx.x * blockDim.x + threadIdx.x;
+  if (gr.row != nullptr && i < B) {
+    const int gs = graph_ptr[i], n = graph_ptr[i + 1] - gs, e0 = rowptr[gs], ne = rowptr[graph_ptr[i + 1]] - e0;
+    int32_t* grec = gnn_graph_rec(gr, N) + 4 * i;
+    grec[0] = gs;
+    grec[1] = n;
+    grec[2] = e0;
+    if (gnn_graph_flag(n, ne)) atomicOr(&grec[3], 1);
+  }
   if (i >= N) return;
   int lo = rowptr[i], hi = rowptr[i + 1];
   for (int a = lo + 1; a < hi; ++a) {
@@ -789,6 +853,23 @@
     }
     eperm[b + 1] = ke;
     col[b + 1] = kc;
+  }
+  if (gr.row != nullptr) {
+    const int g = node_graph[i], gs = graph_ptr[g], dg = hi - lo;
+    bool bad = dg > 4;
+    unsigned srw = 0u, erw = 0u;
+    for (int q = 0; q < 4; ++q) {
+      int sr = GR_NONE_SRC, cl = GR_NONE_CLS;
+      if (q < dg) {
+        sr = col[lo + q] - gs;
+        cl = gnn_edge_code(gr, gr.ea[(long long)eperm[lo + q] * (gr.lde_cls >> 5)]);
+        bad = bad || cl >= GR_BAD || sr < 0 || sr >= GR_MAX_NODES;
+      }
+      srw |= (unsigned)(sr & 255) << (8 * q);
+      erw |= (unsigned)(cl & 255) << (8 * q);
+    }
+    reinterpret_cast<int4*>(gr.row)[i] = make_int4(dg, (int)srw, (int)erw, 0);
+    if (bad) atomicOr(&gnn_graph_rec(gr, N)[4 * g + 3], 1);
   }
 }
 
@@ -821,11 +902,11 @@
 
 extern "C" int sn_batch_plan_early_supported(int64_t N, int64_t E, int64_t B) { return plan_one_launch(N, E, B) ? 1 : 0; }
 
-extern "C" int sn_batch_plan_ex(const int64_t* batch, int64_t N, int64_t B, const int64_t* edge_index,
-                                int64_t E, int kmax, int32_t* graph_ptr, int32_t* node_graph,
-                                int32_t* nvalid, int64_t* evoff, int32_t* rowptr, int32_t* col,
-                                int32_t* eperm, int32_t* status, const sn_plan_bins* bins, int32_t* scratch,
-                                const sn_plan_early* early, void* stream) {
+static int batch_plan(const int64_t* batch, int64_t N, int64_t B, const int64_t* edge_index,
+                      int64_t E, int kmax, int32_t* graph_ptr, int32_t* node_graph,
+                      int32_t* nvalid, int64_t* evoff, int32_t* rowptr, int32_t* col,
+                      int32_t* eperm, int32_t* status, const sn_plan_bins* bins, int32_t* scratch,
+                      const sn_plan_early* early, const sn_plan_gnn* gnn, void* stream) {
   SN_REQUIRE(N >= 0 && B >= 0 && E >= 0, "sn_batch_plan: negative size");
   SN_REQUIRE(N < (1ll << 31) && E < (1ll << 31), "sn_batch_plan: N/E exceed int32");
   SN_REQUIRE(graph_ptr && node_graph && nvalid && evoff && rowptr && status && scratch,
@@ -854,6 +935,13 @@
     ed = EarlyDev{early->node_ids, early->node_ids ? early->n_node_ids : 0, early->node_vocab, early->edge_ids,
                   early->edge_ids ? early->n_edge_ids : 0, early->edge_vocab, early->max_graph_edges, early->host};
   }
+  GnnRec gr{};
+  if (gnn != nullptr) {
+    SN_REQUIRE(gnn->records && (E == 0 || gnn->edge_attr) && gnn->lde >= 1 && gnn->lde < (1 << 26) && gnn->classes >= 1 && gnn->classes <= GR_BAD,
+               "sn_batch_plan_gnn: sn_plan_gnn needs the record array, the edge features with their row stride and 1 <= classes <= %d", GR_BAD);
+    SN_REQUIRE((reinterpret_cast<uintptr_t>(gnn->records) & 15) == 0, "sn_batch_plan_gnn: the record array must be 16-byte aligned");
+    gr = GnnRec{gnn->edge_attr, gnn->records, (int)(gnn->lde << 5) | gnn->classes};
+  }
   hipStream_t st = (hipStream_t)stream;
   if (plan_one_launch(N, E, B)) {
     const size_t lds0 = (size_t)((PS_BMAX + 4) + PS_NMAX + (PS_NMAX + 4) + 2 * PS_EMAX + 32 + PS_NMAX) * sizeof(int);
@@ -868,14 +956,14 @@
     }
     const bool ids = ed.host != nullptr && (ed.node_ids != nullptr || ed.edge_ids != nullptr);
     hipLaunchKernelGGL(k_plan_small, dim3(do_bins ? (ids ? 4 : 3) : 1), dim3(PLAN_T), lds, st, batch, (int)N, (int)B, edge_index, (int)E,
-                       kmax, graph_ptr, node_graph, nvalid, evoff, rowptr, col, eperm, status, bd, do_bins ? 1 : 0, ed);
+                       kmax, graph_ptr, node_graph, nvalid, evoff, rowptr, col, eperm, status, bd, do_bins ? 1 : 0, ed, gr);
     SN_CHECK_LAUNCH("sn_batch_plan");
     return SN_OK;
   }
   int32_t* deg = scratch;
   const int T = 256;
   hipLaunchKernelGGL(k_plan_nodes, dim3((unsigned)cdiv(N > 0 ? N : 1, T)), dim3(T), 0, st, batch, N, B, graph_ptr, node_graph, deg,
-                     status);
+                     status, gr.row != nullptr ? gr.row + 4 * N : nullptr);
   const int64_t ne = N > E ? N : E;
   hipLaunchKernelGGL(k_plan_degree, dim3((unsigned)cdiv(ne > 0 ? ne : 1, T)), dim3(T), 0, st, batch, edge_index, E, N, B, deg,
                      status);
@@ -891,12 +979,31 @@
   }
   hipLaunchKernelGGL(k_plan_scan, dim3(do_bins ? 2 : 1), dim3(PLAN_T), lds3, st, N, B, kmax, graph_ptr, node_graph, deg, rowptr,
                      nvalid, evoff, status, bd);
-  if (E > 0) {
-    hipLaunchKernelGGL(k_plan_fill, dim3((unsigned)cdiv(E, T)), dim3(T), 0, st, edge_index, E, N, deg, col, eperm);
-    hipLaunchKernelGGL(k_plan_sort, dim3((unsigned)cdiv(N, T)), dim3(T), 0, st, N, rowptr, col, eperm);
-  }
+  if (E > 0) hipLaunchKernelGGL(k_plan_fill, dim3((unsigned)cdiv(E, T)), dim3(T), 0, st, edge_index, E, N, deg, col, eperm);
+  const int64_t ns = gr.row != nullptr ? (N > B ? N : B) : N;
+  if ((E > 0 || gr.row != nullptr) && ns > 0)
+    hipLaunchKernelGGL(k_plan_sort, dim3((unsigned)cdiv(ns, T)), dim3(T), 0, st, N, rowptr, col, eperm, B, graph_ptr, node_graph, gr);
   SN_CHECK_LAUNCH("sn_batch_plan");
   return SN_OK;
+}
+
+extern "C" int sn_batch_plan_ex(const int64_t* batch, int64_t N, int64_t B, const int64_t* edge_index,
+                                int64_t E, int kmax, int32_t* graph_ptr, int32_t* node_graph,
+                                int32_t* nvalid, int64_t* evoff, int32_t* rowptr, int32_t* col,
+                                int32_t* eperm, int32_t* status, const sn_plan_bins* bins, int32_t* scratch,
+                                const sn_plan_early* early, void* stream) {
+  return batch_plan(batch, N, B, edge_index, E, kmax, graph_ptr, node_graph, nvalid, evoff, rowptr, col, eperm, status, bins, scratch,
+                    early, nullptr, stream);
+}
+
+extern "C" int sn_batch_plan_gnn(const int64_t* batch, int64_t N, int64_t B, const int64_t* edge_index,
+                                 int64_t E, int kmax, int32_t* graph_ptr, int32_t* node_graph,
+                                 int32_t* nvalid, int64_t* evoff, int32_t* rowptr, int32_t* col,
+                                 int32_t* eperm, int32_t* status, const sn_plan_bins* bins, int32_t* scratch,
+                                 const sn_plan_early* early, const sn_plan_gnn* gnn, void* stream) {
+  SN_REQUIRE(gnn, "sn_batch_plan_gnn: null sn_plan_gnn (sn_batch_plan_ex is the plan without records)");
+  return batch_plan(batch, N, B, edge_index, E, kmax, graph_ptr, node_graph, nvalid, evoff, rowptr, col, eperm, status, bins, scratch,
+                    early, gnn, stream);
 }
 
 extern "C" int sn_batch_plan(const int64_t* batch, int64_t N, int64_t B, const int64_t* edge_index,
diff --git a/signnet_basisnet_amd/fused.py b/signnet_basisnet_amd/fused.py
--- a/signnet_basisnet_amd/fused.py
+++ b/signnet_basisnet_amd/fused.py
@@ -1,6 +1,7 @@
 from __future__ import annotations
 
 import ctypes as C
+import os
 
 import torch
 
@@ -213,6 +214,13 @@
                [("ntab", C.c_void_p * 10)] + \
                [(n, C.c_void_p) for n in ("nw", "n_scale", "n_shift", "rho_out_w", "lin_a", "lin_b", "head_w1", "head_w2")] + \
                [("layers", _GnnLayer * GNN_MAX_LAYERS)]
+
+
+class _GnnFront(C.Structure):
+    _fields_ = [("node_tab", C.c_void_p), ("edge_tab", C.c_void_p), ("records", C.c_void_p), ("n_nodes", C.c_int64)]
+
+
+FAST_FRONT = os.environ.get("SN_GNN_FAST_FRONT", "1") != "0"
 
 
 class GnnPlan:
@@ -284,6 +292,36 @@
             Lp.w2s = hold(ops.pack_split(conv.nn.layers[1].weight.detach(), s, h))
             Lp.eps = hold(conv.layer.eps.detach())
         self.params = P
+        self.front = self._build_front(gnn, dp)
+
+    def _build_front(self, gnn, dp):
+        P = self.params
+        if not (self.node_discrete and self.edge_discrete):
+            return None
+        cls = C.c_int(0)
+        check(lib().sn_gnn_front_classes(C.byref(P), C.byref(cls)), "sn_gnn_front_classes")
+        if cls.value < 1:
+            return None
+        dev = gnn.linear.weight.device
+        node_tab = torch.empty(P.node_vocab, dp, dtype=torch.float32, device=dev)
+        edge_tab = torch.empty(P.n_layers * cls.value, dp, dtype=torch.float32, device=dev)
+        check(lib().sn_gnn_front_tables_f32(C.byref(P), ptr(node_tab), ptr(edge_tab), stream()), "sn_gnn_front_tables_f32")
+        self._keep += [node_tab, edge_tab]
+        self.front_classes = cls.value
+        F = _GnnFront()
+        F.node_tab, F.edge_tab = node_tab.data_ptr(), edge_tab.data_ptr()
+        return F
+
+    def plan_records(self, data):
+        if not FAST_FRONT or self.front is None:
+            return None
+        x, ea = data.x, data.edge_attr
+        if x.dtype != torch.int64 or ea.dtype != torch.int64 or x.numel() != data.batch.numel():
+            return None
+        E = int(data.edge_index.shape[1]) if data.edge_index.numel() else 0
+        if ea.numel() != E:
+            return None
+        return (ea.reshape(E, 1).contiguous() if E else ea.reshape(0, 1), self.front_classes)
 
     def run(self, plan: ops.GraphPlan, x, edge_attr, rho_sum, flags_host=None):
         P = self.params
@@ -308,6 +346,16 @@
         if P.node_nf > (10 if self.node_discrete else 16) or P.edge_nf > (10 if self.edge_discrete else 16):
             raise ValueError("too many feature columns for the fused gnn kernel")
         y = torch.empty(plan.B, self.n_out, dtype=torch.float32, device=rho_sum.device)
+        if self.front is not None and plan.gnn_rec is not None and P.node_nf == 1 and P.edge_nf == 1:
+            F = _GnnFront(self.front.node_tab, self.front.edge_tab, plan.gnn_rec.data_ptr(), plan.N)
+            with ops._span("sn_gnn_fused_f32"):
+                check(lib().sn_gnn_fused_front_f32(C.byref(P), C.byref(F), ptr(x), x.shape[1], ptr(edge_attr),
+                                                   edge_attr.shape[1] if edge_attr.dim() > 1 else 1, ptr(rho_sum),
+                                                   ptr(plan.graph_ptr), plan.B, ptr(plan.rowptr), ptr(plan.col),
+                                                   ptr(plan.eperm), ptr(plan.status), ptr(y),
+                                                   ptr(plan.flags), plan.flags.numel(), ptr(flags_host), stream()),
+                      "sn_gnn_fused_front_f32")
+            return y
         with ops._span("sn_gnn_fused_f32"):
             check(lib().sn_gnn_fused_f32(C.byref(P), ptr(x), x.shape[1], ptr(edge_attr),
                                          edge_attr.shape[1] if edge_attr.dim() > 1 else 1, ptr(rho_sum),
diff --git a/signnet_basisnet_amd/ops.py b/signnet_basisnet_amd/ops.py
--- a/signnet_basisnet_amd/ops.py
+++ b/signnet_basisnet_amd/ops.py
@@ -119,6 +119,7 @@
     status: torch.Tensor
     bins: PlanBins | None
     flags: torch.Tensor = None
+    gnn_rec: torch.Tensor = None
 
     def check(self):
         st = self.status.tolist()
@@ -141,6 +142,10 @@
     _fields_ = [("node_ids", C.c_void_p), ("n_node_ids", C.c_int64), ("node_vocab", C.c_int64),
                 ("edge_ids", C.c_void_p), ("n_edge_ids", C.c_int64), ("edge_vocab", C.c_int64),
                 ("max_graph_edges", C.c_int), ("reserved", C.c_int), ("host", C.c_void_p)]
+
+
+class _PlanGnnC(C.Structure):
+    _fields_ = [("edge_attr", C.c_void_p), ("lde", C.c_int64), ("classes", C.c_int), ("reserved", C.c_int), ("records", C.c_void_p)]
 
 
 class EarlyReport:
@@ -198,7 +203,7 @@
 
 
 def build_plan(batch: torch.Tensor, edge_index: torch.Tensor, num_graphs: int, kmax: int = 0, bins: bool = False,
-               early: "EarlyReport | None" = None, columns: bool = False, counts: torch.Tensor = None) -> GraphPlan:
+               early: "EarlyReport | None" = None, columns: bool = False, counts: torch.Tensor = None, gnn=None) -> GraphPlan:
     require_cuda(batch, edge_index)
     if batch.dtype != torch.int64 or edge_index.dtype != torch.int64:
         raise ValueError("build_plan: batch and edge_index must be int64 (the reference's index dtype)")
@@ -211,6 +216,11 @@
     if bins:
         mb = int(lib().sn_phi_bins_bound(B, int(kmax)))
         sizes += [8, mb if columns else 0, (B + 1) if columns else 0, (8 * B) if columns else 0, (8 * B) if columns else 0, B + 1, 16 * mb]
+    if gnn is not None and counts is not None:
+        raise ValueError("build_plan: the padded plan writes no GINE records")
+    own_rec = gnn is not None and len(gnn) < 3
+    if own_rec:
+        sizes.append(4 * (N + B))
     offs = [0]
     for s in sizes:
         offs.append(offs[-1] + ((s + 3) // 4) * 4)
@@ -235,6 +245,16 @@
                                              C.byref(pb.cstruct) if pb is not None else None, ptr(scratch),
                                              C.byref(early.cstruct) if early is not None else None, ptr(counts), stream()),
                   "sn_batch_plan_padded")
+    elif gnn is not None:
+        rec = parts[-1] if own_rec else gnn[2]
+        if rec.dtype != torch.int32 or rec.numel() < 4 * (N + B) or not rec.is_contiguous() or gnn[0].dtype != torch.int64:
+            raise ValueError("build_plan: GINE records need int64 edge features and an int32 tensor of (N + B) * 4 words")
+        gs = _PlanGnnC(ptr(gnn[0]), 1 if gnn[0].dim() < 2 else int(gnn[0].stride(0)) if E else 1, int(gnn[1]), 0, ptr(rec))
+        with _span("sn_batch_plan"):
+            check(lib().sn_batch_plan_gnn(ptr(batch), N, B, ptr(edge_index), E, int(kmax), ptr(graph_ptr), ptr(node_graph),
+                                          ptr(nvalid), ptr(evoff), ptr(rowptr), ptr(col), ptr(eperm), ptr(status),
+                                          C.byref(pb.cstruct) if pb is not None else None, ptr(scratch),
+                                          C.byref(early.cstruct) if early is not None else None, C.byref(gs), stream()), "sn_batch_plan_gnn")
     else:
         with _span("sn_batch_plan"):
             check(lib().sn_batch_plan_ex(ptr(batch), N, B, ptr(edge_index), E, int(kmax), ptr(graph_ptr), ptr(node_graph),
@@ -243,6 +263,8 @@
                                          C.byref(early.cstruct) if early is not None else None, stream()), "sn_batch_plan")
     plan = GraphPlan(N, B, E, int(kmax), graph_ptr, node_graph, nvalid, evoff, rowptr, col, eperm, status, pb)
     plan.flags = arena[offs[7]:offs[7] + 16] if bins else status
+    if gnn is not None:
+        plan.gnn_rec = parts[-1] if own_rec else gnn[2]
     return plan
 
 
diff --git a/signnet_basisnet_amd/pyg.py b/signnet_basisnet_amd/pyg.py
--- a/signnet_basisnet_amd/pyg.py
+++ b/signnet_basisnet_amd/pyg.py
@@ -740,7 +740,7 @@
             side_a.wait_stream(cur)
         want_vals = "eig" in P or "eig2" in P
         with torch.cuda.stream(side_a), _lib_mod.stream_scope():
-            plan = ops.build_plan(data.batch, data.edge_index, B, self.max_k or 0, bins=True)
+            plan = ops.build_plan(data.batch, data.edge_index, B, self.max_k or 0, bins=True, gnn=P["gnn_fused"].plan_records(data))
             K_host = None if self.max_k else host_max_nodes(data)
             K = int(self.max_k) if self.max_k else (int(K_host) if K_host is not None else plan.check()[1])
             x = P["phi_fused"].run(plan, data.eigen_vectors, K, zero_invalid=False, precision=self._prec).view(plan.N * K, d)
@@ -789,7 +789,8 @@
         K_host = None if self.max_k else host_max_nodes(data)
         if not self.max_k and K_host is None and early is None and not return_stages and not capturing and ops.early_supported(N_, E_n, B):
             early = ops.EarlyReport().arm()
-        plan = ops.build_plan(data.batch, data.edge_index, B, self.max_k or 0, bins=use_phi_fused or use_rho_fused, early=early)
+        plan = ops.build_plan(data.batch, data.edge_index, B, self.max_k or 0, bins=use_phi_fused or use_rho_fused, early=early,
+                              gnn=P["gnn_fused"].plan_records(data) if use_gnn_fused else None)
         self._last_plan, self._used_fused = plan, (use_phi_fused or use_rho_fused or use_gnn_fused)
         if self.max_k:
             K = int(self.max_k)
```
